# jby1993/SelfReconCode

Measured on NVIDIA H100. Metric: rays_per_sec, higher is better.
Workload: dtype f32

## Files before the change

include/selfrecon_b200.h:

```cpp
#ifndef SELFRECON_B200_H_
#define SELFRECON_B200_H_

#include <stdint.h>

#ifdef __cplusplus
extern "C" {
#endif

#ifndef __DRIVER_TYPES_H__
typedef struct CUstream_st* cudaStream_t;
#endif

enum {
  SR_OK = 0,
  SR_EINVAL = -1,
  SR_EUNSUPPORTED = -2,
  SR_ECAPACITY = -3
};

int sr_abi_version(void);
const char* sr_build_info(void);

int sr_minv3x3_f32(const float* ms, float* invs, uint8_t* checks, int64_t n, cudaStream_t s);
int sr_minv3x3_f64(const double* ms, double* invs, uint8_t* checks, int64_t n, cudaStream_t s);
int sr_minv3x3_bwd_f32(const float* grads, const float* invs, float* outs, int64_t n,
                       cudaStream_t s);
int sr_minv3x3_bwd_f64(const double* grads, const double* invs, double* outs, int64_t n,
                       cudaStream_t s);

int64_t sr_mc_work_bytes(int nx, int ny, int nz);
int sr_mc_count(const float* sdf, int nx, int ny, int nz, float iso, void* work, int32_t* counts,
                cudaStream_t s);
int sr_mc_emit(const float* sdf, int nx, int ny, int nz, float iso, float xstep, float ystep,
               float zstep, float xmin, float ymin, float zmin, int i_offset, const void* work,
               float* vertices, int64_t vcap, int64_t* faces, int64_t fcap, cudaStream_t s);

int sr_interp2x3d_fwd_f32(const float* in, float* out, uint8_t* is_boundary, int bc, int d, int h,
                          int w, float balance, cudaStream_t s);
int sr_interp2x3d_bwd_f32(const float* grad_out, float* grad_in, int bc, int d, int h, int w,
                          cudaStream_t s);
int sr_interp2x2d_fwd_f32(const float* in, float* out, uint8_t* is_boundary, int bc, int h, int w,
                          float balance, cudaStream_t s);
int sr_interp2x2d_bwd_f32(const float* grad_out, float* grad_in, int bc, int h, int w,
                          cudaStream_t s);

int sr_grid_sample3d_fwd_f32(const float* input, const int64_t* istr, const float* grid,
                             float* output, int32_t* corner_idx, int N, int C, int D, int H, int W,
                             int64_t P, cudaStream_t s);
int sr_grid_sample3d_bwd_f32(const float* input, const int64_t* istr, const float* grid,
                             const float* grad_output, float* grad_input, float* grad_grid, int N,
                             int C, int D, int H, int W, int64_t P, cudaStream_t s);
int sr_grid_sample3d_dbwd_f32(const float* gg_input ,
                              const float* gg_grid , const float* input,
                              const int64_t* istr, const float* grid, const float* grad_output,
                              float* grad_input , float* grad_grid,
                              float* grad_grad_output, int N, int C, int D, int H, int W,
                              int64_t P, cudaStream_t s);
int sr_grid_sample3d_fwd_f64(const double* input, const int64_t* istr, const double* grid,
                             double* output, int32_t* corner_idx, int N, int C, int D, int H,
                             int W, int64_t P, cudaStream_t s);
int sr_grid_sample3d_bwd_f64(const double* input, const int64_t* istr, const double* grid,
                             const double* grad_output, double* grad_input, double* grad_grid,
                             int N, int C, int D, int H, int W, int64_t P, cudaStream_t s);
int sr_grid_sample3d_dbwd_f64(const double* gg_input, const double* gg_grid, const double* input,
                              const int64_t* istr, const double* grid, const double* grad_output,
                              double* grad_input, double* grad_grid, double* grad_grad_output,
                              int N, int C, int D, int H, int W, int64_t P, cudaStream_t s);

#define SR_MLP_MAX_LAYERS 12
enum { SR_ACT_NONE = 0, SR_ACT_SOFTPLUS100 = 1, SR_ACT_RELU = 2, SR_ACT_TANH = 3 };

typedef struct sr_mlp_layer {
  const float* wt;
  const float* bias;
  int k;
  int n;
  int kpad;
  int npad;
  int act;
  int skip;
  const float* wb;
} sr_mlp_layer;

typedef struct sr_mlp_desc {
  int n_layers;
  int d_in;
  int multires;
  float pe_w[16];
  sr_mlp_layer layer[SR_MLP_MAX_LAYERS];
} sr_mlp_desc;

int sr_fold_linear(const float* v, const float* g, const float* b, int n, int k, int npad,
                   int kpad, float* wt, float* bias_out, float* wb ,
                   cudaStream_t s);

int sr_sdf_forward(const sr_mlp_desc* net, const float* pts, int64_t P, float* sdf, float* grad,
                   float* feat, int nfeat, cudaStream_t s);

int sr_lbs_bone_transforms(const float* poses, const float* Js, const int32_t* parents,
                           const float* init_pose_inv, int F, float* A, float* posedJ ,
                           cudaStream_t s);

typedef struct sr_lbs_params {
  const float* ws_cl;
  int D, H, W;
  float bmin[3], bmax[3];
  const float* A;
  const float* trans;
  int F;
} sr_lbs_params;

int sr_lbs_weights_to_channels_last(const float* ws_ncdhw, float* ws_cl, int D, int H, int W,
                                    cudaStream_t s);

int sr_deform_forward(const sr_mlp_desc* net, const sr_lbs_params* lbs, const float* pts,
                      const int64_t* batch_inds, int64_t pts_per_frame, const float* conds,
                      int condlen, int64_t P, float* d, float* offset, float* jac,
                      int32_t* corner_idx, cudaStream_t s);

int sr_render_forward(const sr_mlp_desc* net, const float* pts, const float* normals,
                      const float* views, const float* feat, int nfeat, int64_t P, float* rgb,
                      cudaStream_t s);

typedef struct sr_trace_params {
  float cam_pos[3];
  float dthreshold;
  float athreshold;
  float w1, w2;
} sr_trace_params;

int sr_trace_step(const sr_mlp_desc* sdf, const sr_mlp_desc* dnet, const sr_lbs_params* lbs,
                  const sr_trace_params* tp, float* pts, const float* rays,
                  const int64_t* batch_inds, const float* conds, int condlen, int64_t P,
                  const int32_t* active_in, int32_t* active_out, int32_t* counters, int iter,
                  uint8_t* converged, cudaStream_t s);

int64_t sr_trace_scratch_bytes(void);
int sr_trace_step_rev(const sr_mlp_desc* sdf, const sr_mlp_desc* dnet, const sr_lbs_params* lbs,
                      const sr_trace_params* tp, float* pts, const float* rays,
                      const int64_t* batch_inds, const float* conds, int condlen, int64_t P,
                      const int32_t* active_in, int32_t* active_out, int32_t* counters, int iter,
                      uint8_t* converged, float* scratch, cudaStream_t s);

int sr_shade_geometry(const sr_mlp_desc* sdf, const sr_mlp_desc* dnet, const sr_lbs_params* lbs,
                      const float* pts, const float* rays, const int64_t* batch_inds,
                      const float* conds, int condlen, int64_t P, float* normals, float* crays,
                      float* feat, int nfeat, float* dpos, uint8_t* inv_ok, cudaStream_t s);

int sr_tc_embed(const float* pts, int64_t P, int multires, const float* pe_w, int ch,
                const float* conds, const int64_t* batch_inds, int64_t pts_per_frame, int condlen,
                float* out, int ld, const int32_t* index ,
                const int32_t* m_dev , cudaStream_t s);
int sr_tc_embed_backward(const float* pts, int64_t P, int multires, const float* pe_w, int ch, const float* gx, int ld,
                         float* gp, cudaStream_t s);
int64_t sr_tc_act_bytes(int64_t M, int K);
int64_t sr_tc_weight_bytes(int N, int K);
int sr_tc_pack_rows(const float* src, int64_t M, int K, int ld, void* dst, const int32_t* m_dev,
                    cudaStream_t s);
int sr_tc_pack_weights(const float* w, int N, int K, int ld, void* dst, cudaStream_t s);
int sr_tc_linear(const void* A, const void* W, const float* bias, int64_t M, int N, int K,
                 int n_valid, int act, int ch, void* A_next, int K_next, float scale,
                 const float* skip_src, int skip_n, int skip_ld, float* out, int out_ld,
                 int out_col0, int out_n, float* dstash, const void* mul_tiles, int mul_K, int mul_act,
                 float mul_scale, const int32_t* m_dev, cudaStream_t s);

int sr_raster_mesh(const float* verts_screen, const int64_t* faces, int64_t N, int64_t V, int64_t F, int H, int W,
                   uint64_t* keys, int64_t* pix_to_face, float* bary, float* zbuf, cudaStream_t s);

typedef struct sr_phong_params {
  float light_ambient[3], light_diffuse[3], light_specular[3];
  float mat_ambient[3], mat_diffuse[3], mat_specular[3];
  float shininess;
  float background[3];
} sr_phong_params;
int sr_mesh_vertex_normals(const float* verts, const int64_t* faces, const int64_t* vf_offsets, const int64_t* vf_faces,
                           int64_t N, int64_t V, int64_t F, float* normals, cudaStream_t s);
int sr_shade_phong(const float* verts, const float* normals, const float* colors, const int64_t* faces, int64_t N,
                   int64_t V, int64_t F, const int64_t* pix_to_face, const float* bary, int H, int W,
                   const float* cam_pos, const float* light_pos, const sr_phong_params* params, float* out,
                   cudaStream_t s);

int64_t sr_tc_wgrad_partial_bytes(int64_t M, int Kd, int Kx, int* splits_out);
void sr_tc_debug_wgrad_desc_swap(int v);
int sr_tc_wgrad(const void* D, int Kd, const void* X, int Kx, int64_t M, float* part, float* dW, int N, int K,
                int ld, cudaStream_t s);
int sr_tc_colsum(const void* T, int64_t M, int K, int ch, float* partial, int slices, cudaStream_t s);
int sr_tc_unpack_rows(const void* T, int64_t M, int K, int Kpad, float* out, int ld, cudaStream_t s);

typedef struct sr_tc_layer {
  const void* W;
  const void* Wb;
  const float* bias;
  const float* zero_bias;
  int n, k, act, skip;
} sr_tc_layer;
int sr_tc_mlp_forward(const sr_tc_layer* layers, int L, const float* x0, int64_t M, int ld, int d_in, int ch, void* A_in,
                      void* const* acts, float* const* stashes, float* out, const int32_t* m_dev, int n_out,
                      cudaStream_t s);
int sr_tc_mlp_backward(const sr_tc_layer* layers, int L, int64_t M, int ld, int d_in, int ch, const float* gout,
                       const void* A_in, void* const* acts, float* const* stashes, void* D0, void* D1, float* part,
                       float* colsum_ws, int colsum_slices, float* const* dW, float* const* db, float* x0_grad,
                       float* g_skip, int g_skip_ld, cudaStream_t s);

int sr_svals3x3_f32(const float* J, float* S, float* V, int64_t n, cudaStream_t s);
int sr_svals3x3_bwd_f32(const float* J, const float* S, const float* V, const float* gS, float* gJ, int64_t n,
                        cudaStream_t s);

typedef struct sr_wn_layer {
  const float* v;
  const float* g;
  float* w;
  float* inv_norm;
  const float* gw;
  float* gv;
  float* gg;
  int32_t n, k, gw_ld, pad_;
} sr_wn_layer;
int sr_weight_norm_forward(const sr_wn_layer* layers, int L, cudaStream_t s);
int sr_weight_norm_backward(const sr_wn_layer* layers, int L, cudaStream_t s);

int sr_band_select(const float* values, int64_t n, float center, float eps, int32_t* list,
                   int32_t* counter, cudaStream_t s);
int sr_sdf_forward_indexed(const sr_mlp_desc* net, const float* pts, int64_t P, const int32_t* index,
                           const int32_t* m_dev, float* sdf, cudaStream_t s);
int64_t sr_sdf_small_work_bytes(int cap);
int sr_sdf_forward_small(const sr_mlp_desc* net, const float* pts, int64_t P, const int32_t* index,
                         const int32_t* m_dev, float* sdf, void* work, int cap, cudaStream_t s);

int sr_tc_trace_mid(const int32_t* index, const int32_t* m_dev, int64_t P, const float* pts,
                    const float* rays, const int64_t* batch_inds, const float* f, const float* off,
                    const sr_lbs_params* lbs, const sr_trace_params* tp, int do_update,
                    uint8_t* converged, float* dsdf, float* ddef, int ld, float* aux,
                    int32_t* recheck , int32_t* recheck_count, float eps_f, float eps_a,
                    cudaStream_t s);
int sr_tc_trace_update(const int32_t* index, const int32_t* m_dev, int64_t P, float* pts,
                       const float* gs, int gs_ld, const float* gskip, int gk_ld, const float* gd,
                       int gd_ld, const float* aux, int mr_s, const float* pw_s, int mr_d,
                       const float* pw_d, int32_t* active_out, int32_t* counter_out,
                       const uint8_t* converged , cudaStream_t s);

int sr_tc_shade_point(int64_t P, const float* pts, const float* rays, const int64_t* batch_inds,
                      const float* sdf4, int ld_s, const float* off4, const sr_lbs_params* lbs,
                      float* normals, float* crays, float* dpos, uint8_t* inv_ok, cudaStream_t s);
int sr_tc_render_embed(int64_t P, const float* pts, const float* views, const float* normals,
                       const float* feat, int feat_ld, int feat_col0, int nfeat, int feat_row_stride,
                       int multires, const float* pw, float* out, int ld, cudaStream_t s);

int sr_seg3d_candidates(const uint8_t* flag, const uint8_t* calculated, uint8_t* cand, int D,
                        int H, int W, int sz, int sy, int sx, int fD, int fH, int fW,
                        cudaStream_t s);
int sr_seg3d_gather(const int64_t* lin, int64_t n, int H, int W, int sz, int sy, int sx, int fD,
                    int fH, int fW, const float* bmin, const float* bmax, const float* grid,
                    float* points, float* interp, uint8_t* calculated, cudaStream_t s);
int sr_seg3d_scatter(const int64_t* lin, int64_t n, const float* values, const float* interp,
                     float balance, float* grid, uint8_t* conflict, int64_t conflict_bytes,
                     int32_t* n_conflicts, cudaStream_t s);

#ifdef __cplusplus
}
#endif
#endif
```

selfreconcode_b200/_lib.py:

```python
import ctypes as C
import os

_HERE = os.path.dirname(os.path.abspath(__file__))
LIB_PATH = os.environ.get("SELFRECON_B200_LIB") or os.path.join(_HERE, "lib", "libselfrecon_b200.so")

SR_OK = 0
SR_EINVAL, SR_EUNSUPPORTED, SR_ECAPACITY = -1, -2, -3
SR_MLP_MAX_LAYERS = 12
SR_ACT_NONE, SR_ACT_SOFTPLUS100, SR_ACT_RELU, SR_ACT_TANH = 0, 1, 2, 3

c_f = C.c_void_p
i64 = C.c_int64
i32 = C.c_int
f32 = C.c_float
stream_t = C.c_void_p


class MlpLayer(C.Structure):
    _fields_ = [("wt", C.c_void_p), ("bias", C.c_void_p), ("k", C.c_int), ("n", C.c_int),
                ("kpad", C.c_int), ("npad", C.c_int), ("act", C.c_int), ("skip", C.c_int),
                ("wb", C.c_void_p)]


class MlpDesc(C.Structure):
    _fields_ = [("n_layers", C.c_int), ("d_in", C.c_int), ("multires", C.c_int),
                ("pe_w", C.c_float * 16), ("layer", MlpLayer * SR_MLP_MAX_LAYERS)]


class LbsParams(C.Structure):
    _fields_ = [("ws_cl", C.c_void_p), ("D", C.c_int), ("H", C.c_int), ("W", C.c_int),
                ("bmin", C.c_float * 3), ("bmax", C.c_float * 3), ("A", C.c_void_p),
                ("trans", C.c_void_p), ("F", C.c_int)]


class TcLayer(C.Structure):
    _fields_ = [("W", C.c_void_p), ("Wb", C.c_void_p), ("bias", C.c_void_p), ("zero_bias", C.c_void_p),
                ("n", C.c_int), ("k", C.c_int), ("act", C.c_int), ("skip", C.c_int)]


class WnLayer(C.Structure):
    _fields_ = [("v", C.c_void_p), ("g", C.c_void_p), ("w", C.c_void_p), ("inv_norm", C.c_void_p),
                ("gw", C.c_void_p), ("gv", C.c_void_p), ("gg", C.c_void_p),
                ("n", C.c_int32), ("k", C.c_int32), ("gw_ld", C.c_int32), ("pad_", C.c_int32)]


class TraceParams(C.Structure):
    _fields_ = [("cam_pos", C.c_float * 3), ("dthreshold", C.c_float), ("athreshold", C.c_float),
                ("w1", C.c_float), ("w2", C.c_float)]


class PhongParams(C.Structure):
    _fields_ = [("light_ambient", C.c_float * 3), ("light_diffuse", C.c_float * 3), ("light_specular", C.c_float * 3),
                ("mat_ambient", C.c_float * 3), ("mat_diffuse", C.c_float * 3), ("mat_specular", C.c_float * 3),
                ("shininess", C.c_float), ("background", C.c_float * 3)]


SIGNATURES = {
    "sr_abi_version": (C.c_int, []),
    "sr_build_info": (C.c_char_p, []),
    "sr_minv3x3_f32": (C.c_int, [c_f, c_f, c_f, i64, stream_t]),
    "sr_minv3x3_f64": (C.c_int, [c_f, c_f, c_f, i64, stream_t]),
    "sr_minv3x3_bwd_f32": (C.c_int, [c_f, c_f, c_f, i64, stream_t]),
    "sr_minv3x3_bwd_f64": (C.c_int, [c_f, c_f, c_f, i64, stream_t]),
    "sr_mc_work_bytes": (i64, [i32, i32, i32]),
    "sr_mc_count": (C.c_int, [c_f, i32, i32, i32, f32, c_f, c_f, stream_t]),
    "sr_mc_emit": (C.c_int, [c_f, i32, i32, i32, f32, f32, f32, f32, f32, f32, f32, i32, c_f, c_f, i64,
                             c_f, i64, stream_t]),
    "sr_interp2x3d_fwd_f32": (C.c_int, [c_f, c_f, c_f, i32, i32, i32, i32, f32, stream_t]),
    "sr_interp2x3d_bwd_f32": (C.c_int, [c_f, c_f, i32, i32, i32, i32, stream_t]),
    "sr_interp2x2d_fwd_f32": (C.c_int, [c_f, c_f, c_f, i32, i32, i32, f32, stream_t]),
    "sr_interp2x2d_bwd_f32": (C.c_int, [c_f, c_f, i32, i32, i32, stream_t]),
    "sr_grid_sample3d_fwd_f32": (C.c_int, [c_f, C.POINTER(i64), c_f, c_f, c_f, i32, i32, i32, i32,
                                           i32, i64, stream_t]),
    "sr_grid_sample3d_bwd_f32": (C.c_int, [c_f, C.POINTER(i64), c_f, c_f, c_f, c_f, i32, i32, i32,
                                           i32, i32, i64, stream_t]),
    "sr_grid_sample3d_dbwd_f32": (C.c_int, [c_f, c_f, c_f, C.POINTER(i64), c_f, c_f, c_f, c_f, c_f,
                                            i32, i32, i32, i32, i32, i64, stream_t]),
    "sr_grid_sample3d_fwd_f64": (C.c_int, [c_f, C.POINTER(i64), c_f, c_f, c_f, i32, i32, i32, i32,
                                           i32, i64, stream_t]),
    "sr_grid_sample3d_bwd_f64": (C.c_int, [c_f, C.POINTER(i64), c_f, c_f, c_f, c_f, i32, i32, i32,
                                           i32, i32, i64, stream_t]),
    "sr_grid_sample3d_dbwd_f64": (C.c_int, [c_f, c_f, c_f, C.POINTER(i64), c_f, c_f, c_f, c_f, c_f,
                                            i32, i32, i32, i32, i32, i64, stream_t]),
    "sr_fold_linear": (C.c_int, [c_f, c_f, c_f, i32, i32, i32, i32, c_f, c_f, c_f, stream_t]),
    "sr_sdf_forward": (C.c_int, [C.POINTER(MlpDesc), c_f, i64, c_f, c_f, c_f, i32, stream_t]),
    "sr_lbs_bone_transforms": (C.c_int, [c_f, c_f, c_f, c_f, i32, c_f, c_f, stream_t]),
    "sr_lbs_weights_to_channels_last": (C.c_int, [c_f, c_f, i32, i32, i32, stream_t]),
    "sr_deform_forward": (C.c_int, [C.POINTER(MlpDesc), C.POINTER(LbsParams), c_f, c_f, i64, c_f,
                                    i32, i64, c_f, c_f, c_f, c_f, stream_t]),
    "sr_render_forward": (C.c_int, [C.POINTER(MlpDesc), c_f, c_f, c_f, c_f, i32, i64, c_f,
                                    stream_t]),
    "sr_trace_step": (C.c_int, [C.POINTER(MlpDesc), C.POINTER(MlpDesc), C.POINTER(LbsParams),
                                C.POINTER(TraceParams), c_f, c_f, c_f, c_f, i32, i64, c_f, c_f,
                                c_f, i32, c_f, stream_t]),
    "sr_trace_scratch_bytes": (i64, []),
    "sr_trace_step_rev": (C.c_int, [C.POINTER(MlpDesc), C.POINTER(MlpDesc), C.POINTER(LbsParams),
                                    C.POINTER(TraceParams), c_f, c_f, c_f, c_f, i32, i64, c_f, c_f,
                                    c_f, i32, c_f, c_f, stream_t]),
    "sr_shade_geometry": (C.c_int, [C.POINTER(MlpDesc), C.POINTER(MlpDesc), C.POINTER(LbsParams),
                                    c_f, c_f, c_f, c_f, i32, i64, c_f, c_f, c_f, i32, c_f, c_f,
                                    stream_t]),
    "sr_tc_embed": (C.c_int, [c_f, i64, i32, C.POINTER(f32), i32, c_f, c_f, i64, i32, c_f, i32, c_f, c_f,
                              stream_t]),
    "sr_tc_embed_backward": (C.c_int, [c_f, i64, i32, C.POINTER(f32), i32, c_f, i32, c_f, stream_t]),
    "sr_tc_act_bytes": (i64, [i64, i32]),
    "sr_tc_weight_bytes": (i64, [i32, i32]),
    "sr_tc_pack_rows": (C.c_int, [c_f, i64, i32, i32, c_f, c_f, stream_t]),
    "sr_tc_pack_weights": (C.c_int, [c_f, i32, i32, i32, c_f, stream_t]),
    "sr_tc_linear": (C.c_int, [c_f, c_f, c_f, i64, i32, i32, i32, i32, i32, c_f, i32, f32, c_f, i32,
                               i32, c_f, i32, i32, i32, c_f, c_f, i32, i32, f32, c_f, stream_t]),
    "sr_tc_trace_mid": (C.c_int, [c_f, c_f, i64, c_f, c_f, c_f, c_f, c_f, C.POINTER(LbsParams),
                                  C.POINTER(TraceParams), i32, c_f, c_f, c_f, i32, c_f, c_f, c_f, f32, f32,
                                  stream_t]),
    "sr_tc_trace_update": (C.c_int, [c_f, c_f, i64, c_f, c_f, i32, c_f, i32, c_f, i32, c_f, i32,
                                     C.POINTER(f32), i32, C.POINTER(f32), c_f, c_f, c_f, stream_t]),
    "sr_raster_mesh": (C.c_int, [c_f, c_f, i64, i64, i64, i32, i32, c_f, c_f, c_f, c_f, stream_t]),
    "sr_mesh_vertex_normals": (C.c_int, [c_f, c_f, c_f, c_f, i64, i64, i64, c_f, stream_t]),
    "sr_shade_phong": (C.c_int, [c_f, c_f, c_f, c_f, i64, i64, i64, c_f, c_f, i32, i32, c_f, c_f,
                                 C.POINTER(PhongParams), c_f, stream_t]),
    "sr_tc_wgrad_partial_bytes": (i64, [i64, i32, i32, C.POINTER(C.c_int)]),
    "sr_tc_debug_wgrad_desc_swap": (None, [i32]),
    "sr_tc_mlp_forward": (C.c_int, [C.POINTER(TcLayer), i32, c_f, i64, i32, i32, i32, c_f, C.POINTER(C.c_void_p),
                                    C.POINTER(C.c_void_p), c_f, c_f, i32, stream_t]),
    "sr_tc_mlp_backward": (C.c_int, [C.POINTER(TcLayer), i32, i64, i32, i32, i32, c_f, c_f, C.POINTER(C.c_void_p),
                                     C.POINTER(C.c_void_p), c_f, c_f, c_f, c_f, i32, C.POINTER(C.c_void_p),
                                     C.POINTER(C.c_void_p), c_f, c_f, i32, stream_t]),
    "sr_tc_wgrad": (C.c_int, [c_f, i32, c_f, i32, i64, c_f, c_f, i32, i32, i32, stream_t]),
    "sr_tc_colsum": (C.c_int, [c_f, i64, i32, i32, c_f, i32, stream_t]),
    "sr_tc_unpack_rows": (C.c_int, [c_f, i64, i32, i32, c_f, i32, stream_t]),
    "sr_weight_norm_forward": (C.c_int, [C.POINTER(WnLayer), i32, stream_t]),
    "sr_weight_norm_backward": (C.c_int, [C.POINTER(WnLayer), i32, stream_t]),
    "sr_svals3x3_f32": (C.c_int, [c_f, c_f, c_f, i64, stream_t]),
    "sr_svals3x3_bwd_f32": (C.c_int, [c_f, c_f, c_f, c_f, c_f, i64, stream_t]),
    "sr_band_select": (C.c_int, [c_f, i64, f32, f32, c_f, c_f, stream_t]),
    "sr_sdf_small_work_bytes": (i64, [i32]),
    "sr_sdf_forward_small": (C.c_int, [C.POINTER(MlpDesc), c_f, i64, c_f, c_f, c_f, c_f, i32, stream_t]),
    "sr_sdf_forward_indexed": (C.c_int, [C.POINTER(MlpDesc), c_f, i64, c_f, c_f, c_f, stream_t]),
    "sr_tc_shade_point": (C.c_int, [i64, c_f, c_f, c_f, c_f, i32, c_f, C.POINTER(LbsParams), c_f, c_f, c_f,
                                    c_f, stream_t]),
    "sr_tc_render_embed": (C.c_int, [i64, c_f, c_f, c_f, c_f, i32, i32, i32, i32, i32, C.POINTER(f32), c_f,
                                     i32, stream_t]),
    "sr_seg3d_candidates": (C.c_int, [c_f, c_f, c_f, i32, i32, i32, i32, i32, i32, i32, i32, i32,
                                      stream_t]),
    "sr_seg3d_gather": (C.c_int, [c_f, i64, i32, i32, i32, i32, i32, i32, i32, i32, C.POINTER(f32), C.POINTER(f32),
                                  c_f, c_f, c_f, c_f, stream_t]),
    "sr_seg3d_scatter": (C.c_int, [c_f, i64, c_f, c_f, f32, c_f, c_f, i64, c_f, stream_t]),
}

_lib = None


def load():
    global _lib
    if _lib is not None:
        return _lib
    if not os.path.exists(LIB_PATH):
        raise RuntimeError(
            "selfrecon_b200: %s is missing -- run `python -m selfreconcode_b200.build` "
            "(or __graft_entry__.build()).  There is no CPU fallback." % LIB_PATH)
    lib = C.CDLL(LIB_PATH)
    for name, (res, args) in SIGNATURES.items():
        fn = getattr(lib, name)
        fn.restype = res
        fn.argtypes = args
    _lib = lib
    return lib


_ERR = {SR_EINVAL: "invalid argument", SR_EUNSUPPORTED: "unsupported shape",
        SR_ECAPACITY: "output buffer too small"}


def check(code, what):
    if code == SR_OK:
        return
    if code < 0:
        raise RuntimeError("selfrecon_b200.%s: %s (code %d)" % (what, _ERR.get(code, "error"), code))
    raise RuntimeError("selfrecon_b200.%s: CUDA error %d" % (what, code))
```

selfreconcode_b200/csrc/tc_common.cuh:

```cuda
#pragma once
#include <cuda_bf16.h>

#include "common.cuh"

namespace sr_tc {

#ifndef SR_TC_PLANES
#define SR_TC_PLANES 2
#endif
constexpr int kPlanes = SR_TC_PLANES;
constexpr int BM = 128, BN = 256, BK = 32, STAGES = kPlanes == 2 ? 3 : 2;
constexpr int A_PLANE = BM * BK;
constexpr int W_PLANE = BN * BK;
constexpr int A_STAGE = kPlanes * A_PLANE;
constexpr int W_STAGE = kPlanes * W_PLANE;
constexpr uint32_t A_STAGE_BYTES = A_STAGE * 2, W_STAGE_BYTES = W_STAGE * 2;

__host__ __device__ inline size_t a_tile_off(long long mt, int kc, int KC, int p) {
  return (((size_t)mt * KC + kc) * kPlanes + p) * A_PLANE;
}
__host__ __device__ inline size_t w_tile_off(int nt, int kc, int KC, int p) {
  return (((size_t)nt * KC + kc) * kPlanes + p) * W_PLANE;
}
__device__ __forceinline__ int in_tile_off(int rows_per_tile, int r, int k) {
  return (k >> 3) * (rows_per_tile * 8) + (r >> 3) * 64 + (r & 7) * 8 + (k & 7);
}

__device__ __forceinline__ void split3(float x, __nv_bfloat16& b1, __nv_bfloat16& b2, __nv_bfloat16& b3) {
  b1 = __float2bfloat16_rn(x);
  const float r1 = x - __bfloat162float(b1);
  b2 = __float2bfloat16_rn(r1);
  const float r2 = r1 - __bfloat162float(b2);
  b3 = __float2bfloat16_rn(r2);
}

__device__ __forceinline__ uint64_t make_desc(uint32_t smem_addr, uint32_t lbo_bytes, uint32_t sbo_bytes) {
  uint64_t d = (uint64_t)((smem_addr & 0x3FFFFu) >> 4);
  d |= (uint64_t)((lbo_bytes >> 4) & 0x3FFFu) << 16;
  d |= (uint64_t)((sbo_bytes >> 4) & 0x3FFFu) << 32;
  return d;
}
__device__ __forceinline__ void wgmma_fence() { asm volatile("wgmma.fence.sync.aligned;" ::: "memory"); }
__device__ __forceinline__ void wgmma_commit() { asm volatile("wgmma.commit_group.sync.aligned;" ::: "memory"); }
template <int N>
__device__ __forceinline__ void wgmma_wait() {
  asm volatile("wgmma.wait_group.sync.aligned %0;" ::"n"(N) : "memory");
}
__device__ __forceinline__ void warpgroup_sync(int id) { asm volatile("bar.sync %0, 128;" ::"r"(id) : "memory"); }

#define SR_ACC8(c, d, i)                                                                                \
  c(d[i]), c(d[i + 1]), c(d[i + 2]), c(d[i + 3]), c(d[i + 4]), c(d[i + 5]), c(d[i + 6]), c(d[i + 7])
#define SR_ACC32(c, d, i) SR_ACC8(c, d, i), SR_ACC8(c, d, i + 8), SR_ACC8(c, d, i + 16), SR_ACC8(c, d, i + 24)
#define SR_ACC128(c, d) SR_ACC32(c, d, 0), SR_ACC32(c, d, 32), SR_ACC32(c, d, 64), SR_ACC32(c, d, 96)
#define SR_WGMMA_M64N256K16_BF16                                                                                   \
  "{\n\t.reg .pred p;\n\tsetp.ne.b32 p, %130, 0;\n\t"                                                            \
  "wgmma.mma_async.sync.aligned.m64n256k16.f32.bf16.bf16 "                                                         \
  "{%0, %1, %2, %3, %4, %5, %6, %7, %8, %9, %10, %11, %12, %13, %14, %15, %16, %17, %18, %19, %20, %21, %22, "     \
  "%23, %24, %25, %26, %27, %28, %29, %30, %31, %32, %33, %34, %35, %36, %37, %38, %39, %40, %41, %42, %43, "      \
  "%44, %45, %46, %47, %48, %49, %50, %51, %52, %53, %54, %55, %56, %57, %58, %59, %60, %61, %62, %63, %64, "      \
  "%65, %66, %67, %68, %69, %70, %71, %72, %73, %74, %75, %76, %77, %78, %79, %80, %81, %82, %83, %84, %85, "      \
  "%86, %87, %88, %89, %90, %91, %92, %93, %94, %95, %96, %97, %98, %99, %100, %101, %102, %103, %104, %105, "     \
  "%106, %107, %108, %109, %110, %111, %112, %113, %114, %115, %116, %117, %118, %119, %120, %121, %122, %123, "   \
  "%124, %125, %126, %127}, %128, %129, p, 1, 1, %131, %132;\n\t}\n"

#define SR_OUT(x) "=f"(x)
#define SR_INOUT(x) "+f"(x)
template <int TA, int TB, bool FIRST>
__device__ __forceinline__ void wgmma_m64n256k16(float (&d)[128], uint64_t adesc, uint64_t bdesc) {
  if constexpr (FIRST)
    asm volatile(SR_WGMMA_M64N256K16_BF16
                 : SR_ACC128(SR_OUT, d)
                 : "l"(adesc), "l"(bdesc), "r"(0), "n"(TA), "n"(TB));
  else
    asm volatile(SR_WGMMA_M64N256K16_BF16
                 : SR_ACC128(SR_INOUT, d)
                 : "l"(adesc), "l"(bdesc), "r"(1), "n"(TA), "n"(TB));
}
#undef SR_OUT
#undef SR_INOUT
#undef SR_WGMMA_M64N256K16_BF16
#undef SR_ACC128
#undef SR_ACC32
#undef SR_ACC8

}
```

selfreconcode_b200/csrc/tc_gemm.cu:

```cuda
#include <cstdlib>

#include "tc_common.cuh"

namespace sr_tc {

struct LayerArgs {
  const __nv_bfloat16* A;
  const __nv_bfloat16* W;
  const float* bias;
  long long M;
  int MT, NT, KC;
  int n_gemm;
  int n;
  int ch;
  __nv_bfloat16* A_next;
  int KCn;
  float scale;
  const float* skip_src;
  int skip_n, skip_ld;
  float* out;
  int out_ld;
  float* dstash;
  const __nv_bfloat16* mul_tiles;
  int mul_KC;
  float mul_inv_scale;
  int out_col0;
  int out_n;
  const int* m_dev;
};

template <int ACT>
__device__ __forceinline__ float act_fn(float z, float& d) {
  if constexpr (ACT == SR_ACT_SOFTPLUS100) {
    const float bz = z * 100.0f;
    const float e = __expf(fminf(bz, 20.0f));
    const float sp = __logf(1.0f + e) * 0.01f;
    const float dd = __fdividef(e, e + 1.0f);
    d = bz > 20.0f ? 1.0f : dd;
    return bz > 20.0f ? z : sp;
  } else if constexpr (ACT == SR_ACT_RELU) {
    d = z > 0.f ? 1.f : 0.f;
    return fmaxf(z, 0.f);
  } else if constexpr (ACT == SR_ACT_TANH) {
    const float t = tanhf(z);
    d = 1.f - t * t;
    return t;
  } else {
    d = 1.f;
    return z;
  }
}

__device__ __forceinline__ float fast_ex2(float x) {
  float y;
  asm("ex2.approx.ftz.f32 %0, %1;" : "=f"(y) : "f"(x));
  return y;
}
__device__ __forceinline__ float fast_lg2(float x) {
  float y;
  asm("lg2.approx.ftz.f32 %0, %1;" : "=f"(y) : "f"(x));
  return y;
}
template <int ACT>
__device__ __forceinline__ float act_val(float z) {
  if constexpr (ACT == SR_ACT_SOFTPLUS100) {
    const float t = z * 144.26950408889634f;
    const float e = fast_ex2(fminf(t, 28.853900817779268f));
    const float sp = fast_lg2(1.0f + e) * 0.006931471805599453f;
    return t > 28.853900817779268f ? z : sp;
  } else if constexpr (ACT == SR_ACT_RELU) {
    return fmaxf(z, 0.f);
  } else if constexpr (ACT == SR_ACT_TANH) {
    return tanhf(z);
  } else {
    return z;
  }
}
template <int ACT>
__device__ __forceinline__ float dact_from_val(float a) {
  if constexpr (ACT == SR_ACT_SOFTPLUS100) return 1.0f - fast_ex2(a * -144.26950408889634f);
  else if constexpr (ACT == SR_ACT_RELU) return a > 0.f ? 1.f : 0.f;
  else if constexpr (ACT == SR_ACT_TANH) return 1.f - a * a;
  else return 1.f;
}

__device__ __forceinline__ void split3x2(float x0, float x1, uint32_t& p1, uint32_t& p2, uint32_t& p3) {
  __nv_bfloat162 h = __floats2bfloat162_rn(x0, x1);
  p1 = *reinterpret_cast<uint32_t*>(&h);
  const float r0 = x0 - __uint_as_float(p1 << 16), r1 = x1 - __uint_as_float(p1 & 0xffff0000u);
  h = __floats2bfloat162_rn(r0, r1);
  p2 = *reinterpret_cast<uint32_t*>(&h);
  if constexpr (kPlanes == 3) {
    const float s0 = r0 - __uint_as_float(p2 << 16), s1 = r1 - __uint_as_float(p2 & 0xffff0000u);
    h = __floats2bfloat162_rn(s0, s1);
    p3 = *reinterpret_cast<uint32_t*>(&h);
  } else {
    p3 = 0u;
  }
}

struct EpiRow {
  long long mt, row;
  int nt, row_in_tile, lane;
  bool row_ok, is_val;
  size_t ds_ld;
};

template <int ACT, int CH, bool MUL, bool PF = true>
__device__ __forceinline__ void epi_chunk(const LayerArgs& a, const EpiRow& r, uint32_t (&v)[32], int chunk,
                                          bool live) {
  const int c0 = r.nt * BN + chunk * 32;
  float o[32];
  if (live) {
    if constexpr (MUL) {
      const __nv_bfloat16* mt = a.mul_tiles + a_tile_off(r.mt, c0 >> 5, a.mul_KC, 0) +
                                (size_t)(r.row_in_tile >> 3) * 64 + (r.row_in_tile & 7) * 8;
      const float kk = -144.26950408889634f * a.mul_inv_scale;
      const long long srow = r.row_ok ? (CH == 4 ? (r.row & ~3LL) : r.row) : 0;
      const float* stash = a.dstash == nullptr || c0 >= a.n ? nullptr : a.dstash + (size_t)srow * r.ds_ld + c0;
      const bool use_stash = (ACT == SR_ACT_SOFTPLUS100) && stash != nullptr;
      uint4 q0[PF ? 4 : 1], q1[PF ? 4 : 1];
      float st[PF ? 32 : 1];
      if constexpr (PF) {
#pragma unroll
        for (int g = 0; g < 4; ++g) {
          q0[g] = __ldg(reinterpret_cast<const uint4*>(mt + (size_t)g * (BM * 8)));
          q1[g] = __ldg(reinterpret_cast<const uint4*>(mt + (size_t)g * (BM * 8) + A_PLANE));
        }
        if (use_stash) {
#pragma unroll
          for (int j4 = 0; j4 < 8; ++j4) {
            const float4 t = __ldg(reinterpret_cast<const float4*>(stash) + j4);
            st[4 * j4] = t.x; st[4 * j4 + 1] = t.y; st[4 * j4 + 2] = t.z; st[4 * j4 + 3] = t.w;
          }
        }
      }
#pragma unroll
      for (int g = 0; g < 4; ++g) {
        uint4 a0, a1;
        float sg[8];
        if constexpr (PF) {
          a0 = q0[g]; a1 = q1[g];
        } else {
          a0 = __ldg(reinterpret_cast<const uint4*>(mt + (size_t)g * (BM * 8)));
          a1 = __ldg(reinterpret_cast<const uint4*>(mt + (size_t)g * (BM * 8) + A_PLANE));
          if (use_stash) {
            const float4 t0 = __ldg(reinterpret_cast<const float4*>(stash) + 2 * g);
            const float4 t1 = __ldg(reinterpret_cast<const float4*>(stash) + 2 * g + 1);
            sg[0] = t0.x; sg[1] = t0.y; sg[2] = t0.z; sg[3] = t0.w; sg[4] = t1.x; sg[5] = t1.y; sg[6] = t1.z; sg[7] = t1.w;
          }
        }
        const uint32_t w0[4] = {a0.x, a0.y, a0.z, a0.w}, w1[4] = {a1.x, a1.y, a1.z, a1.w};
#pragma unroll
        for (int e = 0; e < 8; ++e) {
          const int j = g * 8 + e;
          const uint32_t h0 = w0[e >> 1], h1 = w1[e >> 1];
          const float as = (e & 1) ? __uint_as_float(h0 & 0xffff0000u) + __uint_as_float(h1 & 0xffff0000u)
                                   : __uint_as_float(h0 << 16) + __uint_as_float(h1 << 16);
          float val = __uint_as_float(v[j]);
          if constexpr (CH == 1) {
            float d;
            if constexpr (ACT == SR_ACT_SOFTPLUS100) {
              d = use_stash ? (PF ? st[PF ? j : 0] : sg[e]) : 1.0f - fast_ex2(kk * as);
            } else if constexpr (ACT == SR_ACT_RELU) d = as > 0.f ? 1.f : 0.f;
            else d = 1.f;
            if (c0 + j < a.n) val = r.row_ok ? val * d : 0.f;
          } else {
            float d;
            if constexpr (ACT == SR_ACT_SOFTPLUS100) {
              if (use_stash) d = PF ? st[PF ? j : 0] : sg[e];
              else d = 1.0f - fast_ex2(kk * __shfl_sync(0xffffffffu, as, r.lane & ~3));
            } else if constexpr (ACT == SR_ACT_RELU) {
              d = __shfl_sync(0xffffffffu, as, r.lane & ~3) > 0.f ? 1.f : 0.f;
            } else d = 1.f;
            float cross = 0.f;
            if constexpr (ACT == SR_ACT_SOFTPLUS100) {
              float prod = r.is_val ? 0.f : val * (as * a.mul_inv_scale);
              prod += __shfl_xor_sync(0xffffffffu, prod, 1);
              prod += __shfl_xor_sync(0xffffffffu, prod, 2);
              cross = prod;
            }
            if (c0 + j < a.n) {
              float o4 = val * d;
              if constexpr (ACT == SR_ACT_SOFTPLUS100) { if (r.is_val) o4 += 100.0f * (1.0f - d) * cross; }
              val = r.row_ok ? o4 : 0.f;
            }
          }
          o[j] = val * a.scale;
        }
      }
    } else {
#pragma unroll
      for (int j4 = 0; j4 < 8; ++j4) {
        const float4 b4 = __ldg(reinterpret_cast<const float4*>(a.bias + c0) + j4);
        const float bb[4] = {b4.x, b4.y, b4.z, b4.w};
#pragma unroll
        for (int jj = 0; jj < 4; ++jj) {
          const int j = j4 * 4 + jj;
          const float acc = __uint_as_float(v[j]);
          float val;
          if constexpr (CH == 1) {
            val = act_val<ACT>(acc + bb[jj]);
          } else {
            float d = 1.f;
            val = act_fn<ACT>(acc + bb[jj], d);
            const float dv = __shfl_sync(0xffffffffu, d, r.lane & ~3);
            if (!r.is_val) { val = dv * acc; }
            v[j] = __float_as_uint(d);
          }
          o[j] = val * a.scale;
        }
      }
      if (a.dstash != nullptr && r.is_val && r.row_ok) {
        if constexpr (CH == 1) {
          const float inv = 1.0f / a.scale;
#pragma unroll
          for (int j = 0; j < 32; ++j) v[j] = __float_as_uint(dact_from_val<ACT>(o[j] * inv));
        }
        float4* dd = reinterpret_cast<float4*>(a.dstash + (size_t)r.row * r.ds_ld + c0);
#pragma unroll
        for (int j4 = 0; j4 < 8; ++j4)
          dd[j4] = make_float4(__uint_as_float(v[4 * j4]), __uint_as_float(v[4 * j4 + 1]),
                               __uint_as_float(v[4 * j4 + 2]), __uint_as_float(v[4 * j4 + 3]));
      }
    }
    if (a.out != nullptr && r.row_ok && c0 < a.out_col0 + a.out_n && c0 + 32 > a.out_col0) {
#pragma unroll
      for (int j = 0; j < 32; ++j) {
        const int c = c0 + j - a.out_col0;
        if (c >= 0 && c < a.out_n) a.out[(size_t)r.row * a.out_ld + c] = o[j];
      }
    }
  }
  if (a.A_next == nullptr) return;
  const int kcn = c0 >> 5;
  if (kcn >= a.KCn) return;
  if (!live || c0 + 32 > a.n) {
#pragma unroll
    for (int j = 0; j < 32; ++j) {
      const int c = c0 + j;
      if (!live || c >= a.n) {
        float val = 0.f;
        if (a.skip_src != nullptr && c >= a.n && c < a.n + a.skip_n && r.row_ok)
          val = a.skip_src[(size_t)r.row * a.skip_ld + (c - a.n)] * a.scale;
        o[j] = val;
      }
    }
  }
  __nv_bfloat16* base = a.A_next + a_tile_off(r.mt, kcn, a.KCn, 0) + (size_t)(r.row_in_tile >> 3) * 64 +
                        (r.row_in_tile & 7) * 8;
#pragma unroll
  for (int g = 0; g < 4; ++g) {
    uint4 q1, q2, q3;
    split3x2(o[g * 8 + 0], o[g * 8 + 1], q1.x, q2.x, q3.x);
    split3x2(o[g * 8 + 2], o[g * 8 + 3], q1.y, q2.y, q3.y);
    split3x2(o[g * 8 + 4], o[g * 8 + 5], q1.z, q2.z, q3.z);
    split3x2(o[g * 8 + 6], o[g * 8 + 7], q1.w, q2.w, q3.w);
    __nv_bfloat16* dst = base + (size_t)g * (BM * 8);
    *reinterpret_cast<uint4*>(dst) = q1;
    *reinterpret_cast<uint4*>(dst + A_PLANE) = q2;
    if constexpr (kPlanes == 3) *reinterpret_cast<uint4*>(dst + 2 * A_PLANE) = q3;
  }
}


constexpr int kConsumerWGs = 2;
constexpr int kThreads = 128 * (1 + kConsumerWGs);
constexpr int kEpiWarps = 4 * kConsumerWGs;
constexpr int STG_LD = 132;
constexpr int STG_FLOATS = 64 * STG_LD;
constexpr size_t kSmem = (size_t)STAGES * (A_STAGE_BYTES + W_STAGE_BYTES) + (size_t)kConsumerWGs * STG_FLOATS * 4 + 256;
static_assert(kSmem <= 227 * 1024, "shared memory of one H100 block");

template <bool FIRST>
__device__ __forceinline__ void mma_chunk(float (&acc)[128], uint32_t abase, uint32_t wbase) {
  constexpr int kTerms = kPlanes == 2 ? 3 : 6;
  const int pa[6] = {0, 1, 0, 2, 1, 0}, pw[6] = {1, 0, 0, 0, 1, 0};
  const int pa3[6] = {0, 2, 1, 0, 1, 0}, pw3[6] = {2, 0, 1, 1, 0, 0};
#pragma unroll
  for (int q = 0; q < kTerms; ++q) {
#pragma unroll
    for (int jj = 0; jj < BK / 16; ++jj) {
      const int qa = kPlanes == 2 ? pa[q] : pa3[q], qw = kPlanes == 2 ? pw[q] : pw3[q];
      const uint64_t ad = make_desc(abase + qa * (A_PLANE * 2) + jj * 2 * (BM * 16), BM * 16, 128);
      const uint64_t bd = make_desc(wbase + qw * (W_PLANE * 2) + jj * 2 * (BN * 16), BN * 16, 128);
      if (FIRST && q == 0 && jj == 0) wgmma_m64n256k16<0, 0, true>(acc, ad, bd);
      else wgmma_m64n256k16<0, 0, false>(acc, ad, bd);
    }
  }
}

template <int ACT, int CH, bool MUL>
__global__ void __launch_bounds__(kThreads, 1) tc_sweep_kernel(const __grid_constant__ LayerArgs a) {
  extern __shared__ __align__(1024) unsigned char smem[];
  __nv_bfloat16* sA = reinterpret_cast<__nv_bfloat16*>(smem);
  __nv_bfloat16* sW = reinterpret_cast<__nv_bfloat16*>(smem + (size_t)STAGES * A_STAGE_BYTES);
  float* stg = reinterpret_cast<float*>(smem + (size_t)STAGES * (A_STAGE_BYTES + W_STAGE_BYTES));
  uint64_t* bars = reinterpret_cast<uint64_t*>(stg + kConsumerWGs * STG_FLOATS);
  uint64_t* full = bars;
  uint64_t* empty = bars + STAGES;

  const int warp = threadIdx.x >> 5, lane = threadIdx.x & 31, wg = threadIdx.x >> 7;
  if (threadIdx.x == 0) {
    for (int i = 0; i < STAGES; ++i) { sr_mbar_init(&full[i], 1); sr_mbar_init(&empty[i], kEpiWarps); }
    sr_fence_barrier_init();
  }
  __syncthreads();
  long long Mrows = a.M;
  int MTe = a.MT;
  if (a.m_dev != nullptr) {
    const long long md = (long long)(*a.m_dev);
    Mrows = md < a.M ? md : a.M;
    MTe = (int)((Mrows + BM - 1) / BM);
  }
  const int cta = blockIdx.x, ncta = gridDim.x;
  const int J = cta < MTe ? (MTe - cta + ncta - 1) / ncta : 0;

  if (wg == 0) {
    asm volatile("setmaxnreg.dec.sync.aligned.u32 40;");
    if (threadIdx.x == 0) {
      int slot = 0;
      uint32_t phase = 0;
      for (int j = 0; j < J; ++j) {
        const long long mt = (long long)cta + (long long)j * ncta;
        for (int nt = 0; nt < a.NT; ++nt) {
          for (int kc = 0; kc < a.KC; ++kc) {
            sr_mbar_wait(&empty[slot], phase ^ 1u);
            sr_mbar_arrive_expect_tx(&full[slot], A_STAGE_BYTES + W_STAGE_BYTES);
            sr_bulk_g2s(sW + (size_t)slot * W_STAGE, a.W + w_tile_off(nt, kc, a.KC, 0), W_STAGE_BYTES, &full[slot]);
            sr_bulk_g2s(sA + (size_t)slot * A_STAGE, a.A + a_tile_off(mt, kc, a.KC, 0), A_STAGE_BYTES, &full[slot]);
            if (++slot == STAGES) { slot = 0; phase ^= 1u; }
          }
        }
      }
    }
  } else {
    asm volatile("setmaxnreg.inc.sync.aligned.u32 232;");
    const int cw = wg - 1;
    const int wq = warp & 3;
    float* st = stg + cw * STG_FLOATS;
    float acc[128];
    EpiRow r;
    r.row_in_tile = cw * 64 + (wq & 1) * 32 + lane;
    r.lane = lane;
    r.is_val = (CH == 1) || ((lane & 3) == 0);
    r.ds_ld = MUL ? (size_t)((a.n + BN - 1) / BN) * BN : (size_t)a.NT * BN;
    int slot = 0;
    uint32_t phase = 0;
    for (int j = 0; j < J; ++j) {
      r.mt = (long long)cta + (long long)j * ncta;
      r.row = r.mt * BM + r.row_in_tile;
      r.row_ok = r.row < Mrows;
      for (int nt = 0; nt < a.NT; ++nt) {
        r.nt = nt;
        sr_mbar_wait(&full[slot], phase);
        wgmma_fence();
        mma_chunk<true>(acc, sr_smem_u32(sA + (size_t)slot * A_STAGE) + cw * 8 * 128,
                        sr_smem_u32(sW + (size_t)slot * W_STAGE));
        wgmma_commit();
        int prev = slot;
        if (++slot == STAGES) { slot = 0; phase ^= 1u; }
        for (int kc = 1; kc < a.KC; ++kc) {
          sr_mbar_wait(&full[slot], phase);
          wgmma_fence();
          mma_chunk<false>(acc, sr_smem_u32(sA + (size_t)slot * A_STAGE) + cw * 8 * 128,
                           sr_smem_u32(sW + (size_t)slot * W_STAGE));
          wgmma_commit();
          wgmma_wait<1>();
          if (lane == 0) sr_mbar_arrive(&empty[prev]);
          prev = slot;
          if (++slot == STAGES) { slot = 0; phase ^= 1u; }
        }
        wgmma_wait<0>();
        if (lane == 0) sr_mbar_arrive(&empty[prev]);
#pragma unroll
        for (int h = 0; h < 2; ++h) {
          const int fr = 16 * wq + (lane >> 2), fc = 2 * (lane & 3);
#pragma unroll
          for (int i = 0; i < 16; ++i) {
            *reinterpret_cast<float2*>(st + fr * STG_LD + 8 * i + fc) =
                make_float2(acc[4 * (16 * h + i)], acc[4 * (16 * h + i) + 1]);
            *reinterpret_cast<float2*>(st + (fr + 8) * STG_LD + 8 * i + fc) =
                make_float2(acc[4 * (16 * h + i) + 2], acc[4 * (16 * h + i) + 3]);
          }
          warpgroup_sync(1 + cw);
          const float* srow = st + ((wq & 1) * 32 + lane) * STG_LD + (wq >> 1) * 64;
          for (int i = 0; i < 2; ++i) {
            const int chunk = 4 * h + 2 * (wq >> 1) + i;
            uint32_t v[32];
#pragma unroll
            for (int j4 = 0; j4 < 8; ++j4) {
              const float4 t = reinterpret_cast<const float4*>(srow + 32 * i)[j4];
              v[4 * j4] = __float_as_uint(t.x); v[4 * j4 + 1] = __float_as_uint(t.y);
              v[4 * j4 + 2] = __float_as_uint(t.z); v[4 * j4 + 3] = __float_as_uint(t.w);
            }
            epi_chunk<ACT, CH, MUL>(a, r, v, chunk, nt * BN + chunk * 32 < a.n_gemm);
          }
          warpgroup_sync(1 + cw);
        }
      }
    }
  }
}

__global__ void pack_rows_kernel(const float* __restrict__ src, long long M, int K, int ld,
                                 __nv_bfloat16* __restrict__ dst, int KC, long long MT,
                                 const int* __restrict__ m_dev) {
  if (m_dev != nullptr) {
    const long long md = *m_dev;
    M = md < M ? md : M;
    MT = (M + BM - 1) / BM;
  }
  const long long total = MT * BM * (long long)KC * 4;
  for (long long idx = (long long)blockIdx.x * blockDim.x + threadIdx.x; idx < total;
       idx += (long long)gridDim.x * blockDim.x) {
    const int r = (int)(idx % BM);
    const long long rest = idx / BM;
    const int g = (int)(rest % (KC * 4));
    const long long mt = rest / (KC * 4);
    const long long row = mt * BM + r;
    const int kc = g >> 2, k8 = g & 3;
    __align__(16) __nv_bfloat16 p1[8], p2[8], p3[8];
#pragma unroll
    for (int e = 0; e < 8; ++e) {
      const int k = kc * 32 + k8 * 8 + e;
      const float x = (row < M && k < K) ? src[(size_t)row * ld + k] : 0.f;
      split3(x, p1[e], p2[e], p3[e]);
    }
    const size_t off = (size_t)k8 * (BM * 8) + (size_t)(r >> 3) * 64 + (r & 7) * 8;
    *reinterpret_cast<uint4*>(dst + a_tile_off(mt, kc, KC, 0) + off) = *reinterpret_cast<uint4*>(p1);
    *reinterpret_cast<uint4*>(dst + a_tile_off(mt, kc, KC, 1) + off) = *reinterpret_cast<uint4*>(p2);
    if constexpr (kPlanes == 3)
      *reinterpret_cast<uint4*>(dst + a_tile_off(mt, kc, KC, kPlanes - 1) + off) = *reinterpret_cast<uint4*>(p3);
  }
}

__global__ void pack_skip_tail_kernel(const float* __restrict__ skip_src, int skip_ld, int n, int skip_n, float scale,
                                      long long M, int kc0, int KCn, __nv_bfloat16* __restrict__ dst,
                                      const int* __restrict__ m_dev) {
  if (m_dev != nullptr) {
    const long long md = *m_dev;
    M = md < M ? md : M;
  }
  const long long MT = (M + BM - 1) / BM;
  const int nkc = KCn - kc0;
  const long long total = MT * BM * (long long)nkc * 4;
  for (long long idx = (long long)blockIdx.x * blockDim.x + threadIdx.x; idx < total;
       idx += (long long)gridDim.x * blockDim.x) {
    const int r = (int)(idx % BM);
    const long long rest = idx / BM;
    const int g = (int)(rest % (nkc * 4));
    const long long mt = rest / (nkc * 4);
    const long long row = mt * BM + r;
    const int kc = kc0 + (g >> 2), k8 = g & 3;
    __align__(16) __nv_bfloat16 p1[8], p2[8], p3[8];
#pragma unroll
    for (int e = 0; e < 8; ++e) {
      const int c = kc * 32 + k8 * 8 + e;
      const float x = (skip_src != nullptr && row < M && c >= n && c < n + skip_n)
                          ? skip_src[(size_t)row * skip_ld + (c - n)] * scale : 0.f;
      split3(x, p1[e], p2[e], p3[e]);
    }
    const size_t off = (size_t)k8 * (BM * 8) + (size_t)(r >> 3) * 64 + (r & 7) * 8;
    *reinterpret_cast<uint4*>(dst + a_tile_off(mt, kc, KCn, 0) + off) = *reinterpret_cast<uint4*>(p1);
    *reinterpret_cast<uint4*>(dst + a_tile_off(mt, kc, KCn, 1) + off) = *reinterpret_cast<uint4*>(p2);
    if constexpr (kPlanes == 3)
      *reinterpret_cast<uint4*>(dst + a_tile_off(mt, kc, KCn, kPlanes - 1) + off) = *reinterpret_cast<uint4*>(p3);
  }
}

__global__ void pack_weights_kernel(const float* __restrict__ w, int N, int K, int ld,
                                    __nv_bfloat16* __restrict__ dst, int NT, int KC) {
  const long long total = (long long)NT * BN * KC * 4;
  for (long long idx = (long long)blockIdx.x * blockDim.x + threadIdx.x; idx < total;
       idx += (long long)gridDim.x * blockDim.x) {
    const int r = (int)(idx % BN);
    const long long rest = idx / BN;
    const int g = (int)(rest % (KC * 4));
    const int nt = (int)(rest / (KC * 4));
    const int n = nt * BN + r;
    const int kc = g >> 2, k8 = g & 3;
    __align__(16) __nv_bfloat16 p1[8], p2[8], p3[8];
#pragma unroll
    for (int e = 0; e < 8; ++e) {
      const int k = kc * 32 + k8 * 8 + e;
      const float x = (n < N && k < K) ? w[(size_t)n * ld + k] : 0.f;
      split3(x, p1[e], p2[e], p3[e]);
    }
    const size_t off = (size_t)k8 * (BN * 8) + (size_t)(r >> 3) * 64 + (r & 7) * 8;
    *reinterpret_cast<uint4*>(dst + w_tile_off(nt, kc, KC, 0) + off) = *reinterpret_cast<uint4*>(p1);
    *reinterpret_cast<uint4*>(dst + w_tile_off(nt, kc, KC, 1) + off) = *reinterpret_cast<uint4*>(p2);
    if constexpr (kPlanes == 3)
      *reinterpret_cast<uint4*>(dst + w_tile_off(nt, kc, KC, kPlanes - 1) + off) = *reinterpret_cast<uint4*>(p3);
  }
}

struct EmbedArgs {
  const float* pts;
  long long P;
  int multires;
  float pe_w[16];
  int ch;
  const float* conds;
  const long long* batch_inds;
  long long pts_per_frame;
  int condlen;
  float* out;
  int ld;
  const int* index;
  const int* m_dev;
};
__global__ void embed_kernel(const __grid_constant__ EmbedArgs a) {
  long long np = a.P;
  if (a.m_dev != nullptr) { const long long md = *a.m_dev; np = md < np ? md : np; }
  const long long total = np * a.ch * (long long)a.ld;
  const int pe_dim = 3 + 6 * a.multires;
  for (long long idx = (long long)blockIdx.x * blockDim.x + threadIdx.x; idx < total;
       idx += (long long)gridDim.x * blockDim.x) {
    const int k = (int)(idx % a.ld);
    const long long row = idx / a.ld;
    const long long pi = row / a.ch;
    const long long p = a.index ? (long long)a.index[pi] : pi;
    const int t = (int)(row % a.ch);
    float v = 0.f;
    if (k < 3) {
      v = t == 0 ? a.pts[p * 3 + k] : (t - 1 == k ? 1.f : 0.f);
    } else if (k < pe_dim) {
      const int b = (k - 3) / 6, w6 = (k - 3) % 6, j = w6 % 3;
      const bool is_cos = w6 >= 3;
      if (t == 0 || t - 1 == j) {
        const float freq = (float)(1 << b);
        float sn, cs;
        sincosf(a.pts[p * 3 + j] * freq, &sn, &cs);
        const float w = a.pe_w[b];
        if (t == 0) v = w * (is_cos ? cs : sn);
        else v = is_cos ? -(w * freq) * sn : (w * freq) * cs;
      }
    } else if (k < pe_dim + a.condlen) {
      if (t == 0) {
        const long long bi = a.batch_inds ? a.batch_inds[p] : (a.pts_per_frame > 0 ? p / a.pts_per_frame : 0);
        v = a.conds[bi * a.condlen + (k - pe_dim)];
      }
    }
    a.out[idx] = v;
  }
}

__global__ void embed_bwd_kernel(const float* __restrict__ pts, long long P, int multires, const float* __restrict__ gx,
                                 int ld, int ch, float* __restrict__ gp, float pw0, float pw1, float pw2, float pw3,
                                 float pw4, float pw5, float pw6, float pw7) {
  const float pw[8] = {pw0, pw1, pw2, pw3, pw4, pw5, pw6, pw7};
  for (long long p = (long long)blockIdx.x * blockDim.x + threadIdx.x; p < P; p += (long long)gridDim.x * blockDim.x) {
    const float* gv = gx + (size_t)p * ch * ld;
    float out[3];
#pragma unroll
    for (int j = 0; j < 3; ++j) {
      const float x = pts[p * 3 + j];
      float acc = gv[j];
      const float* gt = ch == 4 ? gv + (size_t)(1 + j) * ld : nullptr;
      float freq = 1.0f;
      for (int b = 0; b < multires; ++b, freq *= 2.0f) {
        float sn, cs;
        sincosf(x * freq, &sn, &cs);
        const float w = pw[b] * freq;
        const int ks = 3 + 6 * b + j, kc = ks + 3;
        acc += w * (cs * gv[ks] - sn * gv[kc]);
        if (gt) acc -= w * freq * (sn * gt[ks] + cs * gt[kc]);
      }
      out[j] = acc;
    }
    gp[p * 3] = out[0]; gp[p * 3 + 1] = out[1]; gp[p * 3 + 2] = out[2];
  }
}

}

extern "C" {

int sr_tc_embed_backward(const float* pts, int64_t P, int multires, const float* pe_w, int ch, const float* gx, int ld,
                         float* gp, cudaStream_t s) {
  if (!pts || !gx || !gp || !pe_w || P <= 0 || (ch != 1 && ch != 4) || multires < 0 || multires > 8 ||
      ld < 3 + 6 * multires)
    return SR_EINVAL;
  float w[8];
  for (int i = 0; i < 8; ++i) w[i] = i < multires ? pe_w[i] : 0.f;
  sr_tc::embed_bwd_kernel<<<sr_grid_for(P, 256, 8), 256, 0, s>>>(pts, P, multires, gx, ld, ch, gp, w[0], w[1], w[2], w[3],
                                                                  w[4], w[5], w[6], w[7]);
  return sr_launch_status();
}

int sr_tc_embed(const float* pts, int64_t P, int multires, const float* pe_w, int ch,
                const float* conds, const int64_t* batch_inds, int64_t pts_per_frame, int condlen,
                float* out, int ld, const int32_t* index, const int32_t* m_dev, cudaStream_t s) {
  if (!pts || !out || !pe_w || P <= 0 || (ch != 1 && ch != 4) || multires < 0 || multires > 16) return SR_EINVAL;
  if (ld < 3 + 6 * multires + condlen || (condlen > 0 && !conds)) return SR_EINVAL;
  sr_tc::EmbedArgs a;
  a.pts = pts; a.P = P; a.multires = multires; a.ch = ch; a.conds = conds;
  a.batch_inds = (const long long*)batch_inds; a.pts_per_frame = pts_per_frame; a.condlen = condlen;
  a.out = out; a.ld = ld; a.index = index; a.m_dev = m_dev;
  for (int i = 0; i < 16; ++i) a.pe_w[i] = i < multires ? pe_w[i] : 0.f;
  const long long total = P * ch * (long long)ld;
  sr_tc::embed_kernel<<<sr_grid_for(total, 256, 8), 256, 0, s>>>(a);
  return sr_launch_status();
}

int64_t sr_tc_act_bytes(int64_t M, int K) {
  const int64_t MT = (M + sr_tc::BM - 1) / sr_tc::BM, KC = (K + 31) / 32;
  return MT * KC * sr_tc::kPlanes * sr_tc::A_PLANE * 2;
}
int64_t sr_tc_weight_bytes(int N, int K) {
  const int64_t NT = (N + sr_tc::BN - 1) / sr_tc::BN, KC = (K + 31) / 32;
  return NT * KC * sr_tc::kPlanes * sr_tc::W_PLANE * 2;
}

int sr_tc_pack_rows(const float* src, int64_t M, int K, int ld, void* dst, const int32_t* m_dev,
                    cudaStream_t s) {
  if (!src || !dst || M <= 0 || K <= 0 || ld < K) return SR_EINVAL;
  const long long MT = (M + sr_tc::BM - 1) / sr_tc::BM;
  const int KC = (K + 31) / 32;
  const long long total = MT * sr_tc::BM * KC * 4;
  sr_tc::pack_rows_kernel<<<sr_grid_for(total, 256, 8), 256, 0, s>>>(src, M, K, ld, (__nv_bfloat16*)dst, KC, MT, m_dev);
  return sr_launch_status();
}

int sr_tc_pack_weights(const float* w, int N, int K, int ld, void* dst, cudaStream_t s) {
  if (!w || !dst || N <= 0 || K <= 0 || ld < K) return SR_EINVAL;
  const int NT = (N + sr_tc::BN - 1) / sr_tc::BN, KC = (K + 31) / 32;
  const long long total = (long long)NT * sr_tc::BN * KC * 4;
  sr_tc::pack_weights_kernel<<<sr_grid_for(total, 256, 8), 256, 0, s>>>(w, N, K, ld, (__nv_bfloat16*)dst, NT, KC);
  return sr_launch_status();
}

int sr_tc_linear(const void* A, const void* W, const float* bias, int64_t M, int N, int K, int n_valid,
                 int act, int ch, void* A_next, int K_next, float scale, const float* skip_src,
                 int skip_n, int skip_ld, float* out, int out_ld, int out_col0, int out_n,
                 float* dstash, const void* mul_tiles, int mul_K, int mul_act, float mul_scale,
                 const int32_t* m_dev, cudaStream_t s) {
  using namespace sr_tc;
  if (M <= 0 || (ch != 1 && ch != 4)) return SR_EINVAL;
  if (!A || !W || !bias || N <= 0 || K <= 0 || (!A_next && !out)) return SR_EINVAL;
  if (mul_tiles ? (mul_K < n_valid || (mul_act != SR_ACT_NONE && mul_act != SR_ACT_SOFTPLUS100 && mul_act != SR_ACT_RELU))
                : (act < SR_ACT_NONE || act > SR_ACT_TANH))
    return SR_EINVAL;
  LayerArgs a;
  a.A = (const __nv_bfloat16*)A; a.W = (const __nv_bfloat16*)W; a.bias = bias; a.M = M;
  a.MT = (int)((M + BM - 1) / BM); a.NT = (N + BN - 1) / BN; a.KC = (K + 31) / 32;
  a.n_gemm = N; a.n = n_valid; a.ch = ch;
  a.A_next = (__nv_bfloat16*)A_next; a.KCn = A_next ? (K_next + 31) / 32 : 0;
  a.scale = scale; a.skip_src = skip_src; a.skip_n = skip_n; a.skip_ld = skip_ld;
  a.out = out; a.out_ld = out_ld; a.dstash = dstash; a.out_col0 = out_col0; a.out_n = out_n;
  a.mul_tiles = (const __nv_bfloat16*)mul_tiles; a.mul_KC = (mul_K + 31) / 32;
  a.mul_inv_scale = mul_scale != 0.f ? 1.0f / mul_scale : 1.0f; a.m_dev = m_dev;

  using Kern = void (*)(const LayerArgs);
  Kern kern = nullptr;
#define SR_SW(ACT_, CH_, MUL_) kern = (Kern)tc_sweep_kernel<ACT_, CH_, MUL_>
  const int key = (ch == 4 ? 10 : 0) + (mul_tiles ? 5 + mul_act : act);
  switch (key) {
    case 0: SR_SW(SR_ACT_NONE, 1, false); break;
    case 1: SR_SW(SR_ACT_SOFTPLUS100, 1, false); break;
    case 2: SR_SW(SR_ACT_RELU, 1, false); break;
    case 3: SR_SW(SR_ACT_TANH, 1, false); break;
    case 5: SR_SW(SR_ACT_NONE, 1, true); break;
    case 6: SR_SW(SR_ACT_SOFTPLUS100, 1, true); break;
    case 7: SR_SW(SR_ACT_RELU, 1, true); break;
    case 10: SR_SW(SR_ACT_NONE, 4, false); break;
    case 11: SR_SW(SR_ACT_SOFTPLUS100, 4, false); break;
    case 12: SR_SW(SR_ACT_RELU, 4, false); break;
    case 13: SR_SW(SR_ACT_TANH, 4, false); break;
    case 15: SR_SW(SR_ACT_NONE, 4, true); break;
    case 16: SR_SW(SR_ACT_SOFTPLUS100, 4, true); break;
    case 17: SR_SW(SR_ACT_RELU, 4, true); break;
  }
#undef SR_SW
  if (!kern) return SR_EINVAL;
  static bool attr_set_dev[64][20] = {};
  int cur_dev = 0;
  cudaGetDevice(&cur_dev);
  bool& attr_set = attr_set_dev[cur_dev & 63][key];
  if (!attr_set) {
    cudaError_t e = cudaFuncSetAttribute(kern, cudaFuncAttributeMaxDynamicSharedMemorySize, (int)kSmem);
    if (e != cudaSuccess) return (int)e;
    attr_set = true;
  }
  const int grid = a.MT < SR_NUM_SMS ? a.MT : SR_NUM_SMS;
  kern<<<grid, kThreads, kSmem, s>>>(a);
  const int kc0 = a.NT * (BN / 32);
  if (a.A_next != nullptr && a.KCn > kc0) {
    const int rc = sr_launch_status();
    if (rc) return rc;
    const long long total = (long long)a.MT * BM * (a.KCn - kc0) * 4;
    pack_skip_tail_kernel<<<sr_grid_for(total, 256, 8), 256, 0, s>>>(a.skip_src, a.skip_ld, a.n, a.skip_n, a.scale, M,
                                                                     kc0, a.KCn, a.A_next, m_dev);
  }
  return sr_launch_status();
}
}
```

selfreconcode_b200/csrc/trace_tc.cu:

```cuda
#include "common.cuh"
#include "lbs.cuh"

namespace {

struct MidArgs {
  const int* index;
  const int* m_dev;
  long long P;
  const float* pts;
  const float* rays;
  const long long* batch_inds;
  const float* f;
  const float* off;
  sr_lbs_params lbs;
  int has_lbs;
  sr_trace_params tp;
  int do_update;
  unsigned char* converged;
  float* dsdf;
  float* ddef;
  int ld;
  float* aux;
  int* recheck;
  int* recheck_count;
  float eps_f, eps_a;
};

__global__ void __launch_bounds__(256) trace_mid_kernel(const __grid_constant__ MidArgs a) {
  long long M = a.P;
  if (a.m_dev) { const long long md = *a.m_dev; M = md < M ? md : M; }
  const int lane = threadIdx.x & 31;
  const long long warp0 = ((long long)blockIdx.x * blockDim.x + threadIdx.x) >> 5;
  const long long nwarps = ((long long)gridDim.x * blockDim.x) >> 5;
  for (long long i = warp0; i < M; i += nwarps) {
    const long long gp = a.index ? (long long)a.index[i] : i;
    float p[3], pp[3], off[3] = {0.f, 0.f, 0.f};
#pragma unroll
    for (int j = 0; j < 3; ++j) {
      p[j] = a.pts[gp * 3 + j];
      if (a.off) off[j] = a.off[i * 3 + j];
      pp[j] = __fadd_rn(p[j], off[j]);
    }
    float d[3], Mm[9];
    int ci[3];
    if (a.has_lbs) {
      lbs_point(a.lbs, pp, a.batch_inds ? (int)a.batch_inds[gp] : 0, d, Mm, ci);
    } else {
#pragma unroll
      for (int j = 0; j < 3; ++j) d[j] = pp[j];
#pragma unroll
      for (int q = 0; q < 9; ++q) Mm[q] = (q % 4 == 0) ? 1.f : 0.f;
    }
    if (lane == 0) {
      const float f = a.f[i];
      const float vx = a.rays[gp * 3], vy = a.rays[gp * 3 + 1], vz = a.rays[gp * 3 + 2];
      const float ux = d[0] - a.tp.cam_pos[0], uy = d[1] - a.tp.cam_pos[1], uz = d[2] - a.tp.cam_pos[2];
      const float cx = uy * vz - uz * vy, cy = uz * vx - ux * vz, cz = ux * vy - uy * vx;
      const float n_up = sqrtf(cx * cx + cy * cy + cz * cz);
      const float n_u = sqrtf(ux * ux + uy * uy + uz * uz);
      const float sang = n_up / n_u;
      const float ang = asinf(sang) * 180.0f / 3.14159265358979323846f;
      bool done = (fabsf(f) < a.tp.dthreshold) && (ang < a.tp.athreshold);
      if (a.recheck != nullptr) {
        const bool maybe = (fabsf(f) < a.tp.dthreshold + a.eps_f) && (ang < a.tp.athreshold + a.eps_a);
        const bool sure = (fabsf(f) < a.tp.dthreshold - a.eps_f) && (ang < a.tp.athreshold - a.eps_a);
        if (maybe && !sure) a.recheck[atomicAdd(a.recheck_count, 1)] = (int)gp;
        done = sure;
      }
      float u[3] = {0.f, 0.f, 0.f}, loss = 0.f;
      int state = 0;
      if (done) {
        a.converged[gp] = 1;
      } else if (a.do_update) {
        state = 1;
        loss = a.tp.w1 * fabsf(f) + a.tp.w2 * fabsf(sang);
        float q[3] = {0.f, 0.f, 0.f};
        if (n_up > 0.f) {
          const float wx = vy * cz - vz * cy, wy = vz * cx - vx * cz, wz = vx * cy - vy * cx;
          const float i1 = 1.0f / (n_up * n_u), i2 = n_up / (n_u * n_u * n_u);
          q[0] = wx * i1 - ux * i2; q[1] = wy * i1 - uy * i2; q[2] = wz * i1 - uz * i2;
        }
#pragma unroll
        for (int j = 0; j < 3; ++j) u[j] = a.tp.w2 * (Mm[j] * q[0] + Mm[3 + j] * q[1] + Mm[6 + j] * q[2]);
      }
      float* ax = a.aux + i * 8;
      ax[0] = loss; ax[1] = __int_as_float(state); ax[2] = u[0]; ax[3] = u[1]; ax[4] = u[2];
    }
    __syncwarp();
    const float* ax = a.aux + i * 8;
    for (int k = lane; k < a.ld; k += 32) {
      float vs = 0.f, vd = 0.f;
      if (k == 0) {
        const float f = a.f[i];
        vs = (__float_as_int(ax[1]) == 1) ? a.tp.w1 * (f > 0.f ? 1.f : (f < 0.f ? -1.f : 0.f)) : 0.f;
      }
      if (k < 3) vd = ax[2 + k];
      a.dsdf[i * a.ld + k] = vs;
      if (a.ddef) a.ddef[i * a.ld + k] = vd;
    }
  }
}

struct UpdArgs {
  const int* index;
  const int* m_dev;
  long long P;
  float* pts;
  const float* gs;
  int gs_ld;
  const float* gskip;
  int gk_ld;
  const float* gd;
  int gd_ld;
  const float* aux;
  int mr_s;
  float pw_s[16];
  int mr_d;
  float pw_d[16];
  int* active_out;
  int* counter_out;
  const unsigned char* converged;
};

__device__ __forceinline__ void pe_chain(const float* g, const float* gk, const float x[3], int multires,
                                         const float* pw, float out[3]) {
#pragma unroll
  for (int j = 0; j < 3; ++j) out[j] += g[j] + (gk ? gk[j] : 0.f);
  float freq = 1.0f;
  for (int b = 0; b < multires; ++b, freq *= 2.0f) {
    const float w = pw[b] * freq;
    const int ks = 3 + 6 * b, kc = ks + 3;
#pragma unroll
    for (int j = 0; j < 3; ++j) {
      float sn, cs;
      sincosf(x[j] * freq, &sn, &cs);
      const float gsn = g[ks + j] + (gk ? gk[ks + j] : 0.f), gcs = g[kc + j] + (gk ? gk[kc + j] : 0.f);
      out[j] += w * (cs * gsn - sn * gcs);
    }
  }
}

__global__ void __launch_bounds__(256) trace_update_kernel(const __grid_constant__ UpdArgs a) {
  long long M = a.P;
  if (a.m_dev) { const long long md = *a.m_dev; M = md < M ? md : M; }
  for (long long i = (long long)blockIdx.x * blockDim.x + threadIdx.x; i < M;
       i += (long long)gridDim.x * blockDim.x) {
    const float* ax = a.aux + i * 8;
    if (__float_as_int(ax[1]) != 1) continue;
    const long long gp = a.index ? (long long)a.index[i] : i;
    if (a.converged != nullptr && a.converged[gp]) continue;
    const float x[3] = {a.pts[gp * 3], a.pts[gp * 3 + 1], a.pts[gp * 3 + 2]};
    float g[3] = {ax[2], ax[3], ax[4]};
    pe_chain(a.gs + i * a.gs_ld, a.gskip ? a.gskip + i * a.gk_ld : nullptr, x, a.mr_s, a.pw_s, g);
    if (a.gd) pe_chain(a.gd + i * a.gd_ld, nullptr, x, a.mr_d, a.pw_d, g);
    const float t = -ax[0] / (g[0] * g[0] + g[1] * g[1] + g[2] * g[2]);
#pragma unroll
    for (int j = 0; j < 3; ++j) a.pts[gp * 3 + j] = x[j] + t * g[j];
    const int slot = atomicAdd(a.counter_out, 1);
    a.active_out[slot] = (int)gp;
  }
}

struct ShadePtArgs {
  long long P;
  const float* pts;
  const float* rays;
  const long long* batch_inds;
  const float* sdf4;
  int ld_s;
  const float* off4;
  sr_lbs_params lbs;
  int has_lbs;
  float* normals;
  float* crays;
  float* dpos;
  unsigned char* inv_ok;
};

__global__ void __launch_bounds__(256) shade_point_kernel(const __grid_constant__ ShadePtArgs a) {
  const int lane = threadIdx.x & 31;
  const long long warp0 = ((long long)blockIdx.x * blockDim.x + threadIdx.x) >> 5;
  const long long nwarps = ((long long)gridDim.x * blockDim.x) >> 5;
  for (long long i = warp0; i < a.P; i += nwarps) {
    float p[3], pp[3], off[3] = {0.f, 0.f, 0.f};
#pragma unroll
    for (int j = 0; j < 3; ++j) {
      p[j] = a.pts[i * 3 + j];
      if (a.off4) off[j] = a.off4[(i * 4) * 3 + j];
      pp[j] = __fadd_rn(p[j], off[j]);
    }
    float d[3], Mm[9];
    int ci[3];
    if (a.has_lbs) lbs_point(a.lbs, pp, a.batch_inds ? (int)a.batch_inds[i] : 0, d, Mm, ci);
    else {
#pragma unroll
      for (int j = 0; j < 3; ++j) d[j] = pp[j];
#pragma unroll
      for (int q = 0; q < 9; ++q) Mm[q] = (q % 4 == 0) ? 1.f : 0.f;
    }
    if (lane == 0) {
      float Q[9], m[9];
#pragma unroll
      for (int r = 0; r < 3; ++r)
#pragma unroll
        for (int c = 0; c < 3; ++c) Q[3 * r + c] = (r == c ? 1.f : 0.f) + (a.off4 ? a.off4[(i * 4 + 1 + c) * 3 + r] : 0.f);
#pragma unroll
      for (int r = 0; r < 3; ++r)
#pragma unroll
        for (int c = 0; c < 3; ++c) m[3 * r + c] = Mm[3 * r] * Q[c] + Mm[3 * r + 1] * Q[3 + c] + Mm[3 * r + 2] * Q[6 + c];
      const float gx = a.sdf4[(i * 4 + 1) * a.ld_s], gy = a.sdf4[(i * 4 + 2) * a.ld_s], gz = a.sdf4[(i * 4 + 3) * a.ld_s];
      const float gn = sqrtf(gx * gx + gy * gy + gz * gz);
      a.normals[i * 3] = gx / gn; a.normals[i * 3 + 1] = gy / gn; a.normals[i * 3 + 2] = gz / gn;
      const float c00 = m[4] * m[8] - m[5] * m[7], c01 = -m[3] * m[8] + m[5] * m[6], c02 = m[3] * m[7] - m[4] * m[6];
      const float c10 = -m[1] * m[8] + m[2] * m[7], c11 = m[0] * m[8] - m[2] * m[6], c12 = -m[0] * m[7] + m[1] * m[6];
      const float c20 = m[1] * m[5] - m[2] * m[4], c21 = -m[0] * m[5] + m[2] * m[3], c22 = m[0] * m[4] - m[1] * m[3];
      const float det = m[0] * c00 + m[1] * c01 + m[2] * c02;
      const bool ok = !(fabs((double)det) < 0.0001);
      const float vx = a.rays[i * 3], vy = a.rays[i * 3 + 1], vz = a.rays[i * 3 + 2];
      float rx = vx, ry = vy, rz = vz;
      if (ok) {
        rx = (c00 / det) * vx + (c10 / det) * vy + (c20 / det) * vz;
        ry = (c01 / det) * vx + (c11 / det) * vy + (c21 / det) * vz;
        rz = (c02 / det) * vx + (c12 / det) * vy + (c22 / det) * vz;
      }
      const float rn = sqrtf(rx * rx + ry * ry + rz * rz);
      a.crays[i * 3] = rx / rn; a.crays[i * 3 + 1] = ry / rn; a.crays[i * 3 + 2] = rz / rn;
      if (a.dpos) { a.dpos[i * 3] = d[0]; a.dpos[i * 3 + 1] = d[1]; a.dpos[i * 3 + 2] = d[2]; }
      if (a.inv_ok) a.inv_ok[i] = ok ? 1 : 0;
    }
  }
}

struct RenderEmbedArgs {
  long long P;
  const float* pts;
  const float* views;
  const float* normals;
  const float* feat;
  int feat_ld, feat_col0, nfeat, feat_row_stride;
  int multires;
  float pw[16];
  float* out;
  int ld;
};
__global__ void render_embed_kernel(const __grid_constant__ RenderEmbedArgs a) {
  const long long total = a.P * (long long)a.ld;
  const int pe = 3 + 6 * a.multires;
  for (long long idx = (long long)blockIdx.x * blockDim.x + threadIdx.x; idx < total;
       idx += (long long)gridDim.x * blockDim.x) {
    const int k = (int)(idx % a.ld);
    const long long p = idx / a.ld;
    float v = 0.f;
    if (k < 3) v = a.pts[p * 3 + k];
    else if (k < 3 + pe) {
      const int q = k - 3;
      if (q < 3) v = a.views[p * 3 + q];
      else {
        const int b = (q - 3) / 6, w6 = (q - 3) % 6, j = w6 % 3;
        float sn, cs;
        sincosf(a.views[p * 3 + j] * (float)(1 << b), &sn, &cs);
        v = a.pw[b] * (w6 >= 3 ? cs : sn);
      }
    } else if (k < 3 + pe + 3) v = a.normals[p * 3 + (k - 3 - pe)];
    else if (k < 3 + pe + 3 + a.nfeat)
      v = a.feat[(size_t)p * a.feat_row_stride * a.feat_ld + a.feat_col0 + (k - 3 - pe - 3)];
    a.out[idx] = v;
  }
}

}

extern "C" {

int sr_tc_shade_point(int64_t P, const float* pts, const float* rays, const int64_t* batch_inds,
                      const float* sdf4, int ld_s, const float* off4, const sr_lbs_params* lbs,
                      float* normals, float* crays, float* dpos, uint8_t* inv_ok, cudaStream_t s) {
  if (P <= 0 || !pts || !rays || !sdf4 || !normals || !crays) return SR_EINVAL;
  ShadePtArgs a;
  a.P = P; a.pts = pts; a.rays = rays; a.batch_inds = (const long long*)batch_inds; a.sdf4 = sdf4;
  a.ld_s = ld_s; a.off4 = off4; a.has_lbs = lbs ? 1 : 0;
  if (lbs) a.lbs = *lbs;
  a.normals = normals; a.crays = crays; a.dpos = dpos; a.inv_ok = inv_ok;
  shade_point_kernel<<<sr_grid_for(P * 32, 256, 8), 256, 0, s>>>(a);
  return sr_launch_status();
}

int sr_tc_render_embed(int64_t P, const float* pts, const float* views, const float* normals,
                       const float* feat, int feat_ld, int feat_col0, int nfeat, int feat_row_stride,
                       int multires, const float* pw, float* out, int ld, cudaStream_t s) {
  if (P <= 0 || !pts || !views || !normals || !out || !pw || (nfeat > 0 && !feat)) return SR_EINVAL;
  if (ld < 3 + 3 + 6 * multires + 3 + nfeat) return SR_EINVAL;
  RenderEmbedArgs a;
  a.P = P; a.pts = pts; a.views = views; a.normals = normals; a.feat = feat; a.feat_ld = feat_ld;
  a.feat_col0 = feat_col0; a.nfeat = nfeat; a.feat_row_stride = feat_row_stride; a.multires = multires;
  for (int i = 0; i < 16; ++i) a.pw[i] = i < multires ? pw[i] : 0.f;
  a.out = out; a.ld = ld;
  render_embed_kernel<<<sr_grid_for(P * (long long)ld, 256, 8), 256, 0, s>>>(a);
  return sr_launch_status();
}

int sr_tc_trace_mid(const int32_t* index, const int32_t* m_dev, int64_t P, const float* pts,
                    const float* rays, const int64_t* batch_inds, const float* f, const float* off,
                    const sr_lbs_params* lbs, const sr_trace_params* tp, int do_update,
                    uint8_t* converged, float* dsdf, float* ddef, int ld, float* aux,
                    int32_t* recheck, int32_t* recheck_count, float eps_f, float eps_a, cudaStream_t s) {
  if (!pts || !rays || !f || !tp || !converged || !dsdf || !aux || P <= 0 || ld < 8) return SR_EINVAL;
  if ((recheck != nullptr) != (recheck_count != nullptr) || eps_f < 0.f || eps_a < 0.f) return SR_EINVAL;
  MidArgs a;
  a.index = index; a.m_dev = m_dev; a.P = P; a.pts = pts; a.rays = rays;
  a.batch_inds = (const long long*)batch_inds; a.f = f; a.off = off;
  a.has_lbs = lbs ? 1 : 0;
  if (lbs) a.lbs = *lbs;
  a.tp = *tp; a.do_update = do_update; a.converged = converged; a.dsdf = dsdf; a.ddef = ddef; a.ld = ld;
  a.aux = aux; a.recheck = recheck; a.recheck_count = recheck_count; a.eps_f = eps_f; a.eps_a = eps_a;
  trace_mid_kernel<<<sr_grid_for(P * 32, 256, 8), 256, 0, s>>>(a);
  return sr_launch_status();
}

int sr_tc_trace_update(const int32_t* index, const int32_t* m_dev, int64_t P, float* pts,
                       const float* gs, int gs_ld, const float* gskip, int gk_ld, const float* gd,
                       int gd_ld, const float* aux, int mr_s, const float* pw_s, int mr_d,
                       const float* pw_d, int32_t* active_out, int32_t* counter_out,
                       const uint8_t* converged, cudaStream_t s) {
  if (!pts || !gs || !aux || !active_out || !counter_out || !pw_s || P <= 0) return SR_EINVAL;
  UpdArgs a;
  a.index = index; a.m_dev = m_dev; a.P = P; a.pts = pts; a.gs = gs; a.gs_ld = gs_ld; a.gskip = gskip;
  a.gk_ld = gk_ld; a.gd = gd; a.gd_ld = gd_ld; a.aux = aux; a.mr_s = mr_s; a.mr_d = mr_d;
  for (int i = 0; i < 16; ++i) { a.pw_s[i] = i < mr_s ? pw_s[i] : 0.f; a.pw_d[i] = (pw_d && i < mr_d) ? pw_d[i] : 0.f; }
  a.active_out = active_out; a.counter_out = counter_out; a.converged = converged;
  trace_update_kernel<<<sr_grid_for(P, 256, 8), 256, 0, s>>>(a);
  return sr_launch_status();
}
}
```

selfreconcode_b200/ops.py:

```python
import ctypes as C
import math

import torch

from . import _lib
from ._lib import MlpDesc, LbsParams, TraceParams
from ._lib import check as _check


import os as _os

TC_ENABLED = _os.environ.get("SELFRECON_B200_TC", "1") != "0"
TC_MIN_POINTS = int(_os.environ.get("SELFRECON_B200_TC_MIN_POINTS", "2048"))

TC_EPS_F = float(_os.environ.get("SELFRECON_B200_TC_EPS_F", "4e-5"))
TC_EPS_A = float(_os.environ.get("SELFRECON_B200_TC_EPS_A", "1e-3"))
TC_REFINE = _os.environ.get("SELFRECON_B200_TC_REFINE", "1") != "0"
TC_REFINE_TRACE = _os.environ.get("SELFRECON_B200_TC_REFINE_TRACE", "0") != "0"
TC_DUAL_STREAM = _os.environ.get("SELFRECON_B200_TC_DUAL_STREAM", "1") != "0"

import itertools as _it
_uid_counter = _it.count()
LAUNCHES = 0

_KERNELS_PER_CALL = {"mc_count": 3}


def _stream():
    return C.c_void_p(torch.cuda.current_stream().cuda_stream)


def check(code, what):
    global LAUNCHES
    _check(code, what)
    LAUNCHES += _KERNELS_PER_CALL.get(what, 1)


def _p(t):
    return C.c_void_p(t.data_ptr()) if t is not None else C.c_void_p(0)


def _need_cuda(*ts):
    for t in ts:
        if t is not None and not t.is_cuda:
            raise RuntimeError("selfrecon_b200: expected a CUDA tensor (no CPU fallback)")


def minv3x3(ms):
    _need_cuda(ms)
    n = ms.shape[0]
    invs = torch.empty((n, 3, 3), dtype=ms.dtype, device=ms.device)
    checks = torch.empty((n,), dtype=torch.bool, device=ms.device)
    lib = _lib.load()
    with torch.cuda.device(ms.device):
        fn = lib.sr_minv3x3_f32 if ms.dtype == torch.float32 else lib.sr_minv3x3_f64
        check(fn(_p(ms), _p(invs), _p(checks), n, _stream()), "minv3x3")
    return invs, checks


def minv3x3_backward(grads, invs):
    _need_cuda(grads, invs)
    n = invs.shape[0]
    outs = torch.empty((n, 3, 3), dtype=invs.dtype, device=invs.device)
    lib = _lib.load()
    with torch.cuda.device(invs.device):
        fn = lib.sr_minv3x3_bwd_f32 if invs.dtype == torch.float32 else lib.sr_minv3x3_bwd_f64
        check(fn(_p(grads), _p(invs), _p(outs), n, _stream()), "minv3x3_bwd")
    return outs


def raster_mesh(verts_screen, faces, H, W):
    _need_cuda(verts_screen, faces)
    vs = verts_screen.detach().contiguous().float()
    fc = faces.contiguous().to(torch.int64)
    N, V, _ = vs.shape
    F = fc.shape[0]
    dev = vs.device
    keys = torch.empty((N, H, W), dtype=torch.int64, device=dev)
    p2f = torch.empty((N, H, W, 1), dtype=torch.int64, device=dev)
    bary = torch.empty((N, H, W, 1, 3), dtype=torch.float32, device=dev)
    zbuf = torch.empty((N, H, W, 1), dtype=torch.float32, device=dev)
    with torch.cuda.device(dev):
        check(_lib.load().sr_raster_mesh(_p(vs), _p(fc), N, V, F, int(H), int(W), _p(keys), _p(p2f), _p(bary),
                                         _p(zbuf), _stream()), "raster_mesh")
    return p2f, bary, zbuf


_KERNELS_PER_CALL["raster_mesh"] = 2


def mesh_vertex_normals(verts, faces, csr):
    _need_cuda(verts, faces, csr[0], csr[1])
    vs = verts.detach().contiguous().float()
    fc = faces.contiguous().to(torch.int64)
    off, fid = csr[0].contiguous().to(torch.int64), csr[1].contiguous().to(torch.int64)
    N, V, _ = vs.shape
    if off.numel() != V + 1:
        raise ValueError("mesh_vertex_normals: csr offsets must have V + 1 entries")
    out = torch.empty_like(vs)
    with torch.cuda.device(vs.device):
        check(_lib.load().sr_mesh_vertex_normals(_p(vs), _p(fc), _p(off), _p(fid), N, V, fc.shape[0], _p(out),
                                                 _stream()), "mesh_vertex_normals")
    return out


def shade_phong(verts, normals, faces, pix_to_face, bary, cam_pos, light_pos, params, colors=None):
    _need_cuda(verts, normals, faces, pix_to_face, bary, cam_pos, light_pos, colors)
    vs = verts.detach().contiguous().float()
    N, V, _ = vs.shape
    H, W = pix_to_face.shape[1], pix_to_face.shape[2]
    nr = normals.detach().contiguous().float()
    col = colors.detach().contiguous().float() if colors is not None else None
    fc = faces.contiguous().to(torch.int64)
    p2f = pix_to_face.contiguous().to(torch.int64)
    br = bary.detach().contiguous().float()
    cp = cam_pos.detach().float().reshape(-1, 3).expand(N, 3).contiguous()
    lp = light_pos.detach().float().reshape(-1, 3).expand(N, 3).contiguous()
    if nr.shape != vs.shape or (col is not None and col.shape != vs.shape) or p2f.numel() != N * H * W \
            or br.numel() != 3 * N * H * W:
        raise ValueError("shade_phong: inconsistent shapes")
    out = torch.empty((N, H, W, 4), dtype=torch.float32, device=vs.device)
    with torch.cuda.device(vs.device):
        check(_lib.load().sr_shade_phong(_p(vs), _p(nr), _p(col), _p(fc), N, V, fc.shape[0], _p(p2f), _p(br),
                                         int(H), int(W), _p(cp), _p(lp), C.byref(params), _p(out), _stream()),
              "shade_phong")
    return out


_KERNELS_PER_CALL.update({"mesh_vertex_normals": 1, "shade_phong": 1})


def svals3x3(J, want_v=True):
    _need_cuda(J)
    J = J.contiguous().float()
    n = J.shape[0]
    S = torch.empty((n, 3), dtype=torch.float32, device=J.device)
    V = torch.empty((n, 3, 3), dtype=torch.float32, device=J.device) if want_v else None
    with torch.cuda.device(J.device):
        check(_lib.load().sr_svals3x3_f32(_p(J), _p(S), _p(V), n, _stream()), "svals3x3")
    return S, V


def svals3x3_backward(J, S, V, gS):
    _need_cuda(J, S, V, gS)
    n = J.shape[0]
    gJ = torch.empty((n, 3, 3), dtype=torch.float32, device=J.device)
    with torch.cuda.device(J.device):
        check(_lib.load().sr_svals3x3_bwd_f32(_p(J.contiguous()), _p(S.contiguous()), _p(V.contiguous()),
                                              _p(gS.contiguous().float()), _p(gJ), n, _stream()), "svals3x3_bwd")
    return gJ


_mc_work = {}


def marching_cubes(sdfs, xstep=1.0, ystep=1.0, zstep=1.0, xmin=0.0, ymin=0.0, zmin=0.0, iso=0.0,
                   i_offset=0):
    _need_cuda(sdfs)
    nx, ny, nz = sdfs.shape
    lib = _lib.load()
    dev = sdfs.device
    with torch.cuda.device(dev):
        wb = lib.sr_mc_work_bytes(nx, ny, nz)
        key = (dev.index, torch.cuda.current_stream().cuda_stream)
        work = _mc_work.get(key)
        if work is None or work.numel() < wb:
            work = torch.empty((wb,), dtype=torch.uint8, device=dev)
            _mc_work[key] = work
        counts = torch.empty((2,), dtype=torch.int32, device=dev)
        check(lib.sr_mc_count(_p(sdfs), nx, ny, nz, float(iso), _p(work), _p(counts), _stream()),
              "mc_count")
        nv, nf = counts.tolist()
        verts = torch.empty((nv, 3), dtype=torch.float32, device=dev)
        faces = torch.empty((nf, 3), dtype=torch.int64, device=dev)
        if nv or nf:
            check(lib.sr_mc_emit(_p(sdfs), nx, ny, nz, float(iso), float(xstep), float(ystep),
                                 float(zstep), float(xmin), float(ymin), float(zmin), int(i_offset),
                                 _p(work),
                                 _p(verts), nv, _p(faces), nf, _stream()), "mc_emit")
    return verts, faces


def marching_cubes_count(sdfs, iso=0.0):
    _need_cuda(sdfs)
    nx, ny, nz = sdfs.shape
    lib = _lib.load()
    dev = sdfs.device
    with torch.cuda.device(dev):
        wb = lib.sr_mc_work_bytes(nx, ny, nz)
        key = (dev.index, torch.cuda.current_stream().cuda_stream, "count")
        work = _mc_work.get(key)
        if work is None or work.numel() < wb:
            work = torch.empty((wb,), dtype=torch.uint8, device=dev)
            _mc_work[key] = work
        counts = torch.empty((2,), dtype=torch.int32, device=dev)
        check(lib.sr_mc_count(_p(sdfs), nx, ny, nz, float(iso), _p(work), _p(counts), _stream()), "mc_count")
        nv, nf = counts.tolist()
    return nv, nf


def interp2x3d_forward(inp, balance):
    _need_cuda(inp)
    b, c, d, h, w = inp.shape
    out = torch.empty((b, c, 2 * d - 1, 2 * h - 1, 2 * w - 1), dtype=inp.dtype, device=inp.device)
    bnd = torch.empty(out.shape, dtype=torch.bool, device=inp.device)
    lib = _lib.load()
    with torch.cuda.device(inp.device):
        check(lib.sr_interp2x3d_fwd_f32(_p(inp), _p(out), _p(bnd), b * c, d, h, w, float(balance),
                                        _stream()), "interp2x3d_fwd")
    return out, bnd


def interp2x3d_backward(grad_out):
    _need_cuda(grad_out)
    b, c, od, oh, ow = grad_out.shape
    d, h, w = (od + 1) // 2, (oh + 1) // 2, (ow + 1) // 2
    gin = torch.empty((b, c, d, h, w), dtype=grad_out.dtype, device=grad_out.device)
    lib = _lib.load()
    with torch.cuda.device(grad_out.device):
        check(lib.sr_interp2x3d_bwd_f32(_p(grad_out), _p(gin), b * c, d, h, w, _stream()),
              "interp2x3d_bwd")
    return gin


def interp2x2d_forward(inp, balance):
    _need_cuda(inp)
    b, c, h, w = inp.shape
    out = torch.empty((b, c, 2 * h - 1, 2 * w - 1), dtype=inp.dtype, device=inp.device)
    bnd = torch.empty(out.shape, dtype=torch.bool, device=inp.device)
    lib = _lib.load()
    with torch.cuda.device(inp.device):
        check(lib.sr_interp2x2d_fwd_f32(_p(inp), _p(out), _p(bnd), b * c, h, w, float(balance),
                                        _stream()), "interp2x2d_fwd")
    return out, bnd


def interp2x2d_backward(grad_out):
    _need_cuda(grad_out)
    b, c, oh, ow = grad_out.shape
    h, w = (oh + 1) // 2, (ow + 1) // 2
    gin = torch.empty((b, c, h, w), dtype=grad_out.dtype, device=grad_out.device)
    lib = _lib.load()
    with torch.cuda.device(grad_out.device):
        check(lib.sr_interp2x2d_bwd_f32(_p(grad_out), _p(gin), b * c, h, w, _stream()),
              "interp2x2d_bwd")
    return gin


def _istr(t):
    return (C.c_int64 * 5)(*t.stride())


def _gs_suffix(t):
    if t.dtype == torch.float32:
        return "f32"
    if t.dtype == torch.float64:
        return "f64"
    raise RuntimeError("grid_sampler_3d: only float32/float64 are supported")


def grid_sample3d_forward(inp, grid, want_corner_idx=False):
    _need_cuda(inp, grid)
    N, Cc, D, H, W = inp.shape
    Do, Ho, Wo = grid.shape[1:4]
    P = Do * Ho * Wo
    g = grid.reshape(N, P, 3).contiguous()
    out = torch.empty((N, Cc, Do, Ho, Wo), dtype=inp.dtype, device=inp.device)
    cidx = torch.empty((N, P, 3), dtype=torch.int32, device=inp.device) if want_corner_idx else None
    lib = _lib.load()
    with torch.cuda.device(inp.device):
        fn = getattr(lib, "sr_grid_sample3d_fwd_" + _gs_suffix(inp))
        check(fn(_p(inp), _istr(inp), _p(g), _p(out), _p(cidx), N, Cc, D, H, W, P, _stream()),
              "grid_sample3d_fwd")
    return (out, cidx) if want_corner_idx else out


def grid_sample3d_backward(inp, grid, grad_output):
    _need_cuda(inp, grid, grad_output)
    N, Cc, D, H, W = inp.shape
    Do, Ho, Wo = grid.shape[1:4]
    P = Do * Ho * Wo
    g = grid.reshape(N, P, 3).contiguous()
    go = grad_output.reshape(N, Cc, P).contiguous()
    ginp = torch.zeros((N, Cc, D, H, W), dtype=inp.dtype, device=inp.device)
    ggrid = torch.empty((N, P, 3), dtype=inp.dtype, device=inp.device)
    lib = _lib.load()
    with torch.cuda.device(inp.device):
        fn = getattr(lib, "sr_grid_sample3d_bwd_" + _gs_suffix(inp))
        check(fn(_p(inp), _istr(inp), _p(g), _p(go), _p(ginp), _p(ggrid), N, Cc, D, H, W, P,
                 _stream()), "grid_sample3d_bwd")
    return ginp, ggrid.reshape(grid.shape)


def grid_sample3d_dbackward(gg_input, gg_grid, inp, grid, grad_output):
    _need_cuda(gg_input, gg_grid, inp, grid, grad_output)
    N, Cc, D, H, W = inp.shape
    Do, Ho, Wo = grid.shape[1:4]
    P = Do * Ho * Wo
    g = grid.reshape(N, P, 3).contiguous()
    go = grad_output.reshape(N, Cc, P).contiguous()
    ggi = gg_input.contiguous()
    ggg = gg_grid.reshape(N, P, 3).contiguous()
    ginp = torch.zeros((N, Cc, D, H, W), dtype=inp.dtype, device=inp.device)
    ggrid = torch.empty((N, P, 3), dtype=inp.dtype, device=inp.device)
    ggout = torch.empty((N, Cc, P), dtype=inp.dtype, device=inp.device)
    lib = _lib.load()
    with torch.cuda.device(inp.device):
        fn = getattr(lib, "sr_grid_sample3d_dbwd_" + _gs_suffix(inp))
        check(fn(_p(ggi), _p(ggg), _p(inp), _istr(inp), _p(g), _p(go), _p(ginp), _p(ggrid),
                 _p(ggout), N, Cc, D, H, W, P, _stream()), "grid_sample3d_dbwd")
    return ginp, ggrid.reshape(grid.shape), ggout.reshape(grad_output.shape)


def _pad(x, m):
    return (x + m - 1) // m * m


class FusedMLP:

    def __init__(self, d_in, multires, device):
        self.d_in = int(d_in)
        self.multires = int(multires)
        self.device = torch.device(device)
        self.bufs = []
        self.desc = MlpDesc()
        self._sig = None
        self.uid = next(_uid_counter)

    def fold(self, linears, pe_w=None):
        d = self.desc
        d.n_layers = len(linears)
        d.d_in = self.d_in
        d.multires = self.multires
        pw = pe_w if pe_w is not None else [1.0] * self.multires
        for i in range(16):
            d.pe_w[i] = float(pw[i]) if i < len(pw) else 0.0
        if len(linears) > _lib.SR_MLP_MAX_LAYERS:
            raise RuntimeError("FusedMLP: too many layers")
        self._linears = linears
        self._lay = []
        with torch.cuda.device(self.device):
            for i, L in enumerate(linears):
                n, k = L["v"].shape
                _need_cuda(L["v"])
                npad, kpad = _pad(n, 128), _pad(k, 8)
                if npad > 512 or kpad > 512:
                    raise RuntimeError("FusedMLP: layer %dx%d exceeds the 512-wide engine" % (n, k))
                wt = torch.empty((kpad, npad), dtype=torch.float32, device=self.device)
                bias = torch.empty((npad,), dtype=torch.float32, device=self.device)
                wb = torch.empty((_pad(n, 8), _pad(k, 128)), dtype=torch.float32, device=self.device)
                self._lay.append(dict(wt=wt, bias=bias, wb=wb, n=n, k=k, npad=npad, kpad=kpad))
                ly = d.layer[i]
                ly.wt, ly.bias, ly.wb = wt.data_ptr(), bias.data_ptr(), wb.data_ptr()
                ly.k, ly.n, ly.kpad, ly.npad = k, n, kpad, npad
                ly.act = int(L["act"])
                ly.skip = 1 if L.get("skip") else 0
        self.bufs = [t for e in self._lay for t in (e["wt"], e["bias"], e["wb"])]
        self._children = []
        self.version = 0
        self.refold()
        return self

    def refold(self):
        lib = _lib.load()
        with torch.cuda.device(self.device):
            for e, L in zip(self._lay, self._linears):
                v = L["v"].detach().contiguous().float()
                g, b = L.get("g"), L.get("b")
                g = g.detach().contiguous().float().view(-1) if g is not None else None
                b = b.detach().contiguous().float() if b is not None else None
                check(lib.sr_fold_linear(_p(v), _p(g), _p(b), e["n"], e["k"], e["npad"], e["kpad"], _p(e["wt"]),
                                         _p(e["bias"]), _p(e["wb"]), _stream()), "fold_linear")
        self.version += 1
        for c in self._children:
            c._refresh_from_parent()
        tc = getattr(self, "_tc", None)
        if tc is not None:
            tc.repack()
        return self

    def set_pe_weights(self, pe_w):
        for i in range(16):
            self.desc.pe_w[i] = float(pe_w[i]) if i < len(pe_w) else 0.0

    def truncated_last(self, n_out):
        t = FusedMLP(self.d_in, self.multires, self.device)
        C.memmove(C.byref(t.desc), C.byref(self.desc), C.sizeof(MlpDesc))
        last = t.desc.layer[t.desc.n_layers - 1]
        e = self._lay[-1]
        npad = _pad(n_out, 128)
        t._own = None
        if npad != e["npad"]:
            t._own = (e["wt"][:, :npad].contiguous(), e["bias"][:npad].contiguous(), npad)
            last.wt = t._own[0].data_ptr()
            last.bias = t._own[1].data_ptr()
            last.npad = npad
        last.n = n_out
        t._parent = self
        t._lay = self._lay[:-1] + [dict(e, n=n_out, npad=npad, wt=t._own[0] if t._own else e["wt"],
                                        bias=t._own[1] if t._own else e["bias"])]
        t.bufs = [x for x in (t._own[:2] if t._own else [])]
        t._children = []
        t.version = self.version
        self._children.append(t)
        return t

    def _refresh_from_parent(self):
        if self._own is not None:
            e = self._parent._lay[-1]
            self._own[0].copy_(e["wt"][:, :self._own[2]])
            self._own[1].copy_(e["bias"][:self._own[2]])
        self.version = self._parent.version
        tc = getattr(self, "_tc", None)
        if tc is not None:
            tc.repack()


def annealing_weights(multires, ratio):
    if ratio is None:
        return [1.0] * multires
    if ratio <= 0:
        return [0.0] * multires
    alpha = ratio * multires
    return [(1.0 - math.cos(math.pi * min(max(alpha - float(i), 0.0), 1.0))) / 2.0
            for i in range(multires)]


def sdf_forward(net, pts, want_grad=False, nfeat=0):
    _need_cuda(pts)
    pts = pts.contiguous().float()
    P = pts.shape[0]
    dev = pts.device
    sdf = torch.empty((P,), dtype=torch.float32, device=dev)
    grad = torch.empty((P, 3), dtype=torch.float32, device=dev) if want_grad else None
    feat = torch.empty((P, nfeat), dtype=torch.float32, device=dev) if nfeat else None
    lib = _lib.load()
    with torch.cuda.device(dev):
        check(lib.sr_sdf_forward(C.byref(net.desc), _p(pts), P, _p(sdf), _p(grad), _p(feat),
                                 int(nfeat), _stream()), "sdf_forward")
    return sdf, grad, feat


_band_scratch = {}
SMALL_REFINE = _os.environ.get("SELFRECON_B200_SMALL_REFINE", "1") != "0"
SMALL_CAP = 4096
_KERNELS_PER_CALL["sdf_forward_small"] = 10


def sdf_refine_band(net, pts, sdf, center=0.0, eps=None):
    _need_cuda(pts, sdf)
    eps = TC_EPS_F if eps is None else float(eps)
    P = sdf.numel()
    if P == 0:
        return sdf
    dev = sdf.device
    lib = _lib.load()
    with torch.cuda.device(dev):
        key = (dev.index, torch.cuda.current_stream().cuda_stream)
        buf = _band_scratch.get(key)
        if buf is None or buf.numel() < P + 1:
            buf = torch.empty((max(P + 1, 1 << 16),), dtype=torch.int32, device=dev)
            _band_scratch[key] = buf
        cnt, lst = buf[0:1], buf[1:]
        cnt.zero_()
        check(lib.sr_band_select(_p(sdf), P, float(center), eps, _p(lst), _p(cnt), _stream()), "band_select")
        if SMALL_REFINE:
            wkey = key + ("small",)
            work = _band_scratch.get(wkey)
            if work is None:
                work = torch.empty((lib.sr_sdf_small_work_bytes(SMALL_CAP),), dtype=torch.uint8, device=dev)
                _band_scratch[wkey] = work
            check(lib.sr_sdf_forward_small(C.byref(net.desc), _p(pts), P, _p(lst), _p(cnt), _p(sdf), _p(work),
                                           SMALL_CAP, _stream()), "sdf_forward_small")
            over = _band_scratch.get(key + ("over",))
            if over is None:
                over = torch.empty((1,), dtype=torch.int32, device=dev)
                _band_scratch[key + ("over",)] = over
            torch.clamp(cnt - SMALL_CAP, min=0, out=over)
            if P > SMALL_CAP:
                check(lib.sr_sdf_forward_indexed(C.byref(net.desc), _p(pts), P, _p(lst[SMALL_CAP:]), _p(over), _p(sdf),
                                                 _stream()), "sdf_forward_indexed")
        else:
            check(lib.sr_sdf_forward_indexed(C.byref(net.desc), _p(pts), P, _p(lst), _p(cnt), _p(sdf), _stream()),
                  "sdf_forward_indexed")
    return sdf


class LbsState:

    def __init__(self, ws_ncdhw, bmin, bmax, Js, parents, init_pose_inv):
        _need_cuda(ws_ncdhw)
        dev = ws_ncdhw.device
        _, c, D, H, W = ws_ncdhw.shape
        assert c == 24
        self.D, self.H, self.W = D, H, W
        self.device = dev
        self.ws_cl = torch.empty((D, H, W, 24), dtype=torch.float32, device=dev)
        lib = _lib.load()
        with torch.cuda.device(dev):
            check(lib.sr_lbs_weights_to_channels_last(_p(ws_ncdhw.contiguous().float()),
                                                      _p(self.ws_cl), D, H, W, _stream()),
                  "lbs_weights_to_channels_last")
        self.bmin = [float(x) for x in bmin.view(-1).tolist()]
        self.bmax = [float(x) for x in bmax.view(-1).tolist()]
        self.Js = Js.detach().contiguous().float().view(24, 3)
        self.parents = torch.as_tensor(parents, dtype=torch.int32, device=dev).contiguous()
        self.ipi = init_pose_inv.detach().contiguous().float() if init_pose_inv is not None else None
        self.A = None
        self.trans = None
        self.params = LbsParams()

    def set_pose(self, poses, trans, want_posed_joints=False):
        F = poses.shape[0]
        poses = poses.detach().contiguous().float().view(F, 24, 3)
        self.trans = trans.detach().contiguous().float().view(F, 3)
        self.A = torch.empty((F, 24, 4, 4), dtype=torch.float32, device=self.device)
        pj = torch.empty((F, 24, 3), dtype=torch.float32, device=self.device) if want_posed_joints else None
        lib = _lib.load()
        with torch.cuda.device(self.device):
            check(lib.sr_lbs_bone_transforms(_p(poses), _p(self.Js), _p(self.parents), _p(self.ipi),
                                             F, _p(self.A), _p(pj), _stream()), "lbs_bone_transforms")
        p = self.params
        p.ws_cl = self.ws_cl.data_ptr()
        p.D, p.H, p.W = self.D, self.H, self.W
        for i in range(3):
            p.bmin[i] = self.bmin[i]
            p.bmax[i] = self.bmax[i]
        p.A = self.A.data_ptr()
        p.trans = self.trans.data_ptr()
        p.F = F
        return pj


def _lbs_ref(lbs):
    return C.byref(lbs.params) if lbs is not None else None


def deform_forward(net, lbs, pts, batch_inds, conds, want_jac=False, want_offset=False,
                   want_corner_idx=False, pts_per_frame=0):
    _need_cuda(pts)
    pts = pts.contiguous().float().view(-1, 3)
    P = pts.shape[0]
    dev = pts.device
    conds = conds.detach().contiguous().float() if conds is not None else None
    condlen = conds.shape[-1] if conds is not None else 0
    bi = batch_inds.contiguous().to(torch.int64) if batch_inds is not None else None
    d = torch.empty((P, 3), dtype=torch.float32, device=dev)
    off = torch.empty((P, 3), dtype=torch.float32, device=dev) if want_offset else None
    jac = torch.empty((P, 3, 3), dtype=torch.float32, device=dev) if want_jac else None
    ci = torch.empty((P, 3), dtype=torch.int32, device=dev) if want_corner_idx else None
    lib = _lib.load()
    with torch.cuda.device(dev):
        check(lib.sr_deform_forward(C.byref(net.desc), _lbs_ref(lbs), _p(pts), _p(bi),
                                    int(pts_per_frame), _p(conds), condlen, P, _p(d), _p(off),
                                    _p(jac), _p(ci), _stream()), "deform_forward")
    return d, off, jac, ci


def render_forward(net, pts, normals, views, feat):
    _need_cuda(pts, normals, views)
    P = pts.shape[0]
    dev = pts.device
    nfeat = feat.shape[1] if feat is not None else 0
    rgb = torch.empty((P, 3), dtype=torch.float32, device=dev)
    lib = _lib.load()
    with torch.cuda.device(dev):
        check(lib.sr_render_forward(C.byref(net.desc), _p(pts.contiguous().float()),
                                    _p(normals.contiguous().float()), _p(views.contiguous().float()),
                                    _p(feat.contiguous().float() if feat is not None else None),
                                    nfeat, P, _p(rgb), _stream()), "render_forward")
    return rgb


_scratch = {}


_host_cache = {}


def _host_floats(t):
    if not t.is_cuda:
        return tuple(float(x) for x in t.detach().reshape(-1).tolist())
    key = (t.device.index, t.data_ptr(), t._version, t.numel())
    v = _host_cache.get(key)
    if v is None:
        if len(_host_cache) > 64:
            _host_cache.clear()
        v = tuple(float(x) for x in t.detach().reshape(-1).tolist())
        _host_cache[key] = v
    return v


def _trace_scratch(dev):
    key = (dev.index, torch.cuda.current_stream(dev).cuda_stream)
    if key not in _scratch:
        n = _lib.load().sr_trace_scratch_bytes()
        _scratch[key] = torch.empty((n // 4,), dtype=torch.float32, device=dev)
    return _scratch[key]


def trace_surface_points(sdf_net, def_net, lbs, cam_pos, rays, init_pts, batch_inds, conds,
                         dthreshold=5e-5, athreshold=0.02, w1=3.05, w2=1.0, times=5,
                         return_counters=False, mode="auto"):
    if mode == "auto":
        mode = "tc" if (TC_ENABLED and init_pts.shape[0] >= TC_MIN_POINTS) else "reverse"
    if mode == "tc":
        return trace_surface_points_tc(sdf_net, def_net, lbs, cam_pos, rays, init_pts, batch_inds, conds,
                                       dthreshold, athreshold, w1, w2, times, return_counters)
    _need_cuda(rays, init_pts)
    dev = init_pts.device
    P = init_pts.shape[0]
    pts = init_pts.detach().contiguous().float().clone()
    rays = rays.detach().contiguous().float()
    bi = batch_inds.contiguous().to(torch.int64) if batch_inds is not None else None
    conds = conds.detach().contiguous().float() if conds is not None else None
    condlen = conds.shape[-1] if conds is not None else 0
    conv = torch.zeros((P,), dtype=torch.bool, device=dev)
    if P == 0:
        return (pts, conv, torch.zeros((times + 3,), dtype=torch.int32, device=dev)) if return_counters \
            else (pts, conv)
    lists = [torch.empty((P,), dtype=torch.int32, device=dev) for _ in range(2)]
    counters = torch.zeros((times + 3,), dtype=torch.int32, device=dev)
    tp = TraceParams()
    cp = _host_floats(cam_pos)
    for i in range(3):
        tp.cam_pos[i] = cp[i]
    tp.dthreshold, tp.athreshold, tp.w1, tp.w2 = float(dthreshold), float(athreshold), float(w1), float(w2)
    lib = _lib.load()
    dref = C.byref(def_net.desc) if def_net is not None else None
    with torch.cuda.device(dev):
        scratch = _trace_scratch(dev) if mode == "reverse" else None
        for it in range(times + 1):
            a_in = lists[(it + 1) & 1] if it > 0 else None
            a_out = lists[it & 1] if it < times else None
            if mode == "reverse":
                check(lib.sr_trace_step_rev(C.byref(sdf_net.desc), dref, _lbs_ref(lbs), C.byref(tp),
                                            _p(pts), _p(rays), _p(bi), _p(conds), condlen, P, _p(a_in),
                                            _p(a_out), _p(counters), it, _p(conv), _p(scratch),
                                            _stream()), "trace_step_rev")
            else:
                check(lib.sr_trace_step(C.byref(sdf_net.desc), dref, _lbs_ref(lbs), C.byref(tp),
                                        _p(pts), _p(rays), _p(bi), _p(conds), condlen, P, _p(a_in),
                                        _p(a_out), _p(counters), it, _p(conv), _stream()),
                      "trace_step")
    if return_counters:
        return pts, conv, counters
    return pts, conv


def shade_geometry(sdf_net, def_net, lbs, pts, rays, batch_inds, conds, nfeat=0, want_dpos=False):
    _need_cuda(pts, rays)
    dev = pts.device
    P = pts.shape[0]
    pts = pts.detach().contiguous().float()
    rays = rays.detach().contiguous().float()
    bi = batch_inds.contiguous().to(torch.int64) if batch_inds is not None else None
    conds = conds.detach().contiguous().float() if conds is not None else None
    condlen = conds.shape[-1] if conds is not None else 0
    normals = torch.empty((P, 3), dtype=torch.float32, device=dev)
    crays = torch.empty((P, 3), dtype=torch.float32, device=dev)
    feat = torch.empty((P, nfeat), dtype=torch.float32, device=dev) if nfeat else None
    dpos = torch.empty((P, 3), dtype=torch.float32, device=dev) if want_dpos else None
    ok = torch.empty((P,), dtype=torch.bool, device=dev)
    lib = _lib.load()
    with torch.cuda.device(dev):
        check(lib.sr_shade_geometry(C.byref(sdf_net.desc),
                                    C.byref(def_net.desc) if def_net is not None else None, _lbs_ref(lbs),
                                    _p(pts), _p(rays), _p(bi), _p(conds), condlen, P, _p(normals),
                                    _p(crays), _p(feat), int(nfeat), _p(dpos), _p(ok), _stream()),
              "shade_geometry")
    return normals, crays, feat, dpos, ok


def seg3d_candidates(flag, calculated, stride_zyx):
    _need_cuda(flag, calculated)
    D, H, W = flag.shape
    fD, fH, fW = calculated.shape
    cand = torch.empty((D, H, W), dtype=torch.bool, device=flag.device)
    lib = _lib.load()
    with torch.cuda.device(flag.device):
        check(lib.sr_seg3d_candidates(_p(flag.contiguous()), _p(calculated), _p(cand), D, H, W,
                                      int(stride_zyx[0]), int(stride_zyx[1]), int(stride_zyx[2]),
                                      fD, fH, fW, _stream()), "seg3d_candidates")
    return cand


_KERNELS_PER_CALL.update({"seg3d_candidates": 2, "seg3d_scatter": 3})


def seg3d_gather(lin, level_hw, stride_zyx, calculated, bmin, bmax, grid_flat):
    _need_cuda(lin, calculated, grid_flat)
    n = lin.numel()
    dev = lin.device
    fD, fH, fW = calculated.shape
    pts = torch.empty((n, 3), dtype=torch.float32, device=dev)
    interp = torch.empty((n,), dtype=torch.float32, device=dev)
    lib = _lib.load()
    lo = (C.c_float * 3)(*[float(v) for v in bmin])
    hi = (C.c_float * 3)(*[float(v) for v in bmax])
    with torch.cuda.device(dev):
        check(lib.sr_seg3d_gather(_p(lin), n, int(level_hw[0]), int(level_hw[1]), int(stride_zyx[0]),
                                  int(stride_zyx[1]), int(stride_zyx[2]), fD, fH, fW, lo, hi, _p(grid_flat),
                                  _p(pts), _p(interp), _p(calculated), _stream()), "seg3d_gather")
    return pts, interp


def seg3d_scatter(lin, values, interp, balance, grid_flat):
    _need_cuda(lin, values, interp, grid_flat)
    dev = lin.device
    conflict = torch.empty((grid_flat.numel(),), dtype=torch.bool, device=dev)
    ncf = torch.empty((1,), dtype=torch.int32, device=dev)
    lib = _lib.load()
    with torch.cuda.device(dev):
        check(lib.sr_seg3d_scatter(_p(lin), lin.numel(), _p(values), _p(interp), float(balance), _p(grid_flat),
                                   _p(conflict), conflict.numel(), _p(ncf), _stream()), "seg3d_scatter")
    return conflict, ncf


def tc_pack_rows(x):
    _need_cuda(x)
    x = x.contiguous().float()
    M, K = x.shape
    lib = _lib.load()
    buf = torch.empty((lib.sr_tc_act_bytes(M, K),), dtype=torch.uint8, device=x.device)
    with torch.cuda.device(x.device):
        check(lib.sr_tc_pack_rows(_p(x), M, K, K, _p(buf), None, _stream()), "tc_pack_rows")
    return buf


def tc_pack_weights(w):
    _need_cuda(w)
    w = w.contiguous().float()
    N, K = w.shape
    lib = _lib.load()
    buf = torch.empty((lib.sr_tc_weight_bytes(N, K),), dtype=torch.uint8, device=w.device)
    with torch.cuda.device(w.device):
        check(lib.sr_tc_pack_weights(_p(w), N, K, K, _p(buf), _stream()), "tc_pack_weights")
    return buf


def tc_linear(A, W, bias, M, N, K, n_valid, act, ch=1, K_next=0, scale=1.0, skip_src=None, skip_n=0,
              want_out=False):
    lib = _lib.load()
    dev = A.device
    A_next = torch.empty((lib.sr_tc_act_bytes(M, K_next),), dtype=torch.uint8, device=dev) if K_next else None
    out = torch.empty((M, n_valid), dtype=torch.float32, device=dev) if want_out else None
    npad = (N + 255) // 256 * 256
    b = torch.zeros((npad,), dtype=torch.float32, device=dev)
    b[:bias.numel()] = bias.reshape(-1)
    with torch.cuda.device(dev):
        check(lib.sr_tc_linear(_p(A), _p(W), _p(b), M, N, K, n_valid, int(act), int(ch), _p(A_next),
                               int(K_next), float(scale), _p(skip_src), int(skip_n),
                               skip_src.shape[1] if skip_src is not None else 0, _p(out),
                               n_valid if want_out else 0, 0, n_valid, None, None, 0, 0, 1.0, None, _stream()),
              "tc_linear")
    return A_next, out, None


class TcNet:

    def __init__(self, fused):
        self.fused = fused
        d = fused.desc
        self.layers = []
        lib = _lib.load()
        dev = fused.device
        for i in range(d.n_layers):
            ly = d.layer[i]
            e = fused._lay[i]
            n, k = ly.n, ly.k
            W = torch.empty((lib.sr_tc_weight_bytes(n, k),), dtype=torch.uint8, device=dev)
            Wb = torch.empty((lib.sr_tc_weight_bytes(k, n),), dtype=torch.uint8, device=dev)
            self.layers.append(dict(W=W, Wb=Wb, bias=torch.zeros((_pad(n, 256),), dtype=torch.float32, device=dev),
                                    n=n, k=k, act=ly.act, skip=bool(ly.skip), _e=e,
                                    zero_bias=torch.zeros((_pad(k, 256),), dtype=torch.float32, device=dev)))
        self.c_layers = (_lib.TcLayer * len(self.layers))()
        for c, L in zip(self.c_layers, self.layers):
            c.W, c.Wb, c.bias, c.zero_bias = (L[t].data_ptr() for t in ("W", "Wb", "bias", "zero_bias"))
            c.n, c.k, c.act, c.skip = L["n"], L["k"], L["act"], int(L["skip"])
        self.repack()

    def repack(self):
        lib = _lib.load()
        with torch.cuda.device(self.fused.device):
            for L in self.layers:
                e, n, k = L["_e"], L["n"], L["k"]
                check(lib.sr_tc_pack_weights(_p(e["wb"]), n, k, e["wb"].shape[1], _p(L["W"]), _stream()),
                      "tc_pack_weights")
                check(lib.sr_tc_pack_weights(_p(e["wt"]), k, n, e["wt"].shape[1], _p(L["Wb"]), _stream()),
                      "tc_pack_weights")
                L["bias"][:n].copy_(e["bias"][:n])


def tc_net(fused):
    t = getattr(fused, "_tc", None)
    if t is None:
        t = TcNet(fused)
        fused._tc = t
    return t


def _tc_mlp(lib, tcn, x0, ch, out, A_in=None, acts=None, m_dev=None):
    global LAUNCHES
    M, ld = x0.shape
    L = len(tcn.layers)
    if A_in is None:
        A_in = torch.empty((lib.sr_tc_act_bytes(M, ld),), dtype=torch.uint8, device=x0.device)
        acts = [torch.empty((lib.sr_tc_act_bytes(M, _pad(ly["k"], 32)),), dtype=torch.uint8, device=x0.device)
                for ly in tcn.layers[1:]]
    acts_c = (C.c_void_p * max(L - 1, 1))(*[a.data_ptr() for a in acts])
    check(lib.sr_tc_mlp_forward(tcn.c_layers, L, _p(x0), M, ld, tcn.fused.desc.d_in, ch, _p(A_in), acts_c, None,
                                _p(out), _p(m_dev), out.shape[1], _stream()), "tc_mlp_forward")
    LAUNCHES += L


def tc_mlp_forward(fused, pts, ch=1, conds=None, batch_inds=None, pts_per_frame=0, n_out=None):
    _need_cuda(pts)
    net = tc_net(fused)
    d = fused.desc
    dev = pts.device
    pts = pts.contiguous().float().view(-1, 3)
    P = pts.shape[0]
    M = P * ch
    condlen = conds.shape[-1] if conds is not None else 0
    ld = _pad(d.d_in, 32)
    lib = _lib.load()
    emb = torch.empty((M, ld), dtype=torch.float32, device=dev)
    out = torch.empty((M, n_out or net.layers[-1]["n"]), dtype=torch.float32, device=dev)
    pw = (C.c_float * 16)(*[d.pe_w[i] for i in range(16)])
    bi = batch_inds.contiguous().to(torch.int64) if batch_inds is not None else None
    cd = conds.detach().contiguous().float() if conds is not None else None
    with torch.cuda.device(dev):
        check(lib.sr_tc_embed(_p(pts), P, d.multires, pw, ch, _p(cd), _p(bi), int(pts_per_frame), condlen,
                              _p(emb), ld, None, None, _stream()), "tc_embed")
        _tc_mlp(lib, net, emb, ch, out)
    return out


class _TcTraceBuffers:

    def __init__(self, dev, P, sdf_net, def_net):
        lib = _lib.load()
        self.P = P
        f32 = lambda *shape: torch.empty(shape, dtype=torch.float32, device=dev)
        u8 = lambda n: torch.empty((n,), dtype=torch.uint8, device=dev)
        self.ld_s = _pad(sdf_net.desc.d_in, 32)
        self.emb_s = f32(P, self.ld_s)
        widest = max([32] + [_pad(net.desc.layer[l].n, 32) for net in (sdf_net, def_net) if net is not None
                             for l in range(net.desc.n_layers - 1)])
        self.A = [u8(lib.sr_tc_act_bytes(P, widest)) for _ in range(2)]
        self.f = f32(P, 1)
        self.A_in = u8(lib.sr_tc_act_bytes(P, 256))
        self.acts_s = [u8(lib.sr_tc_act_bytes(P, _pad(sdf_net.desc.layer[i + 1].k, 32)))
                       for i in range(sdf_net.desc.n_layers - 1)]
        self.cot_s = f32(P, 32)
        self.cot_d = f32(P, 32)
        self.aux = f32(P, 8)
        self.gs = f32(P, 64)
        self.gskip = f32(P, 64)
        if def_net is not None:
            self.ld_d = _pad(def_net.desc.d_in, 32)
            self.emb_d = f32(P, self.ld_d)
            self.off = f32(P, 3)
            self.acts_d = [u8(lib.sr_tc_act_bytes(P, _pad(def_net.desc.layer[i + 1].k, 32)))
                           for i in range(def_net.desc.n_layers - 1)]
            self.gd = f32(P, 64)
            self.A_in_d = u8(lib.sr_tc_act_bytes(P, 256))
            self.A_d = [u8(lib.sr_tc_act_bytes(P, widest)) for _ in range(2)]
            self.gskip_d = f32(P, 64)


def _tc_backward_sweep(lib, tcn, cot, bufs, acts, P, m_dev, g_out, g_skip, n_keep):
    d_in = tcn.fused.desc.d_in
    cur, nxt = bufs
    check(lib.sr_tc_pack_rows(_p(cot), P, 32, 32, _p(cur), _p(m_dev), _stream()), "tc_pack_rows")
    K = 32
    for l in range(len(tcn.layers) - 1, -1, -1):
        ly = tcn.layers[l]
        scale = 0.7071067811865476 if ly["skip"] else 1.0
        if l > 0:
            n_prev = tcn.layers[l - 1]["n"]
            Kn = _pad(n_prev, 32)
            gk = g_skip if ly["skip"] else None
            check(lib.sr_tc_linear(_p(cur), _p(ly["Wb"]), _p(ly["zero_bias"]), P, ly["k"], K, n_prev, 0, 1, _p(nxt),
                                   Kn, scale, None, 0, 0, _p(gk), gk.shape[1] if gk is not None else 0, n_prev,
                                   d_in if gk is not None else 0, None, _p(acts[l - 1]), _pad(ly["k"], 32),
                                   tcn.layers[l - 1]["act"], scale, _p(m_dev), _stream()), "tc_linear")
            cur, nxt, K = nxt, cur, Kn
        else:
            check(lib.sr_tc_linear(_p(cur), _p(ly["Wb"]), _p(ly["zero_bias"]), P, ly["k"], K, ly["k"], 0, 1, None, 0,
                                   scale, None, 0, 0, _p(g_out), g_out.shape[1], 0, n_keep, None, None, 0, 0, 1.0,
                                   _p(m_dev), _stream()), "tc_linear")


class _TcTraceCtx:

    def __init__(self, dev, P, sdf_net, def_net, n_frames, condlen, times):
        self.B = _TcTraceBuffers(dev, P, sdf_net, def_net)
        self.pts = torch.empty((P, 3), dtype=torch.float32, device=dev)
        self.rays = torch.empty((P, 3), dtype=torch.float32, device=dev)
        self.bi = torch.empty((P,), dtype=torch.int64, device=dev)
        self.conds = torch.empty((n_frames, condlen), dtype=torch.float32, device=dev) if condlen else None
        self.conv = torch.empty((P,), dtype=torch.bool, device=dev)
        self.counters = torch.empty((times + 3,), dtype=torch.int32, device=dev)
        self.lists = [torch.empty((P,), dtype=torch.int32, device=dev) for _ in range(2)]
        self.lbsA = torch.empty((n_frames, 24, 4, 4), dtype=torch.float32, device=dev)
        self.lbsT = torch.empty((n_frames, 3), dtype=torch.float32, device=dev)
        self.lbs_params = LbsParams()
        self.side_stream = torch.cuda.Stream(device=dev)
        self.recheck = torch.empty((P,), dtype=torch.int32, device=dev)
        self.recheck_counts = torch.empty((times + 1,), dtype=torch.int32, device=dev)
        self.rev_scratch = _trace_scratch(dev)
        self.graph = None
        self.sig = None
        self.calls = 0
        self.n_launches = 0


_tc_trace_ctx = {}
GRAPHS_ENABLED = _os.environ.get("SELFRECON_B200_GRAPHS", "1") != "0"


def _tc_trace_body(lib, G, sdf_net, def_net, ts, td, tp, P, times, condlen, has_lbs):
    B = G.B
    ds, dd = sdf_net.desc, (def_net.desc if def_net is not None else None)
    pw_s = (C.c_float * 16)(*[ds.pe_w[i] for i in range(16)])
    pw_d = (C.c_float * 16)(*[dd.pe_w[i] for i in range(16)]) if dd is not None else None
    pts, rays, bi, conds, conv, counters, lists = G.pts, G.rays, G.bi, G.conds, G.conv, G.counters, G.lists
    lbs_ref = C.byref(G.lbs_params) if has_lbs else None
    conv.zero_()
    counters.zero_()
    counters[0:1].fill_(P)
    refine = TC_REFINE_TRACE
    if refine:
        G.recheck_counts.zero_()
    dref = C.byref(def_net.desc) if def_net is not None else None
    for it in range(times + 1):
        idx = lists[(it + 1) & 1] if it > 0 else None
        a_out = lists[it & 1] if it < times else None
        m_dev = counters[it:it + 1]
        check(lib.sr_tc_embed(_p(pts), P, ds.multires, pw_s, 1, None, None, 0, 0, _p(B.emb_s), B.ld_s,
                              _p(idx), _p(m_dev), _stream()), "tc_embed")
        dual = TC_DUAL_STREAM and def_net is not None
        if dual:
            main = torch.cuda.current_stream()
            side = G.side_stream
            side.wait_stream(main)
            with torch.cuda.stream(side):
                check(lib.sr_tc_embed(_p(pts), P, dd.multires, pw_d, 1, _p(conds), _p(bi), 0, condlen,
                                      _p(B.emb_d), B.ld_d, _p(idx), _p(m_dev), _stream()), "tc_embed")
                _tc_mlp(lib, td, B.emb_d, 1, B.off, B.A_in_d, B.acts_d, m_dev)
        _tc_mlp(lib, ts, B.emb_s, 1, B.f, B.A_in, B.acts_s, m_dev)
        if dual:
            main.wait_stream(side)
        elif def_net is not None:
            check(lib.sr_tc_embed(_p(pts), P, dd.multires, pw_d, 1, _p(conds), _p(bi), 0, condlen,
                                  _p(B.emb_d), B.ld_d, _p(idx), _p(m_dev), _stream()), "tc_embed")
            _tc_mlp(lib, td, B.emb_d, 1, B.off, B.A_in, B.acts_d, m_dev)
        check(lib.sr_tc_trace_mid(_p(idx), _p(m_dev), P, _p(pts), _p(rays), _p(bi), _p(B.f),
                                  _p(B.off) if def_net is not None else None, lbs_ref, C.byref(tp),
                                  1 if a_out is not None else 0, _p(conv), _p(B.cot_s),
                                  _p(B.cot_d) if def_net is not None else None, 32, _p(B.aux),
                                  _p(G.recheck) if refine else None,
                                  _p(G.recheck_counts[it:it + 1]) if refine else None,
                                  TC_EPS_F if refine else 0.0, TC_EPS_A if refine else 0.0, _stream()),
              "tc_trace_mid")
        if refine:
            check(lib.sr_trace_step_rev(C.byref(sdf_net.desc), dref, lbs_ref, C.byref(tp), _p(pts), _p(rays),
                                        _p(bi), _p(conds), condlen, P, _p(G.recheck), None,
                                        _p(G.recheck_counts), it, _p(conv), _p(G.rev_scratch), _stream()),
                  "trace_step_rev")
        if a_out is None:
            break
        if dual:
            side.wait_stream(main)
            with torch.cuda.stream(side):
                _tc_backward_sweep(lib, td, B.cot_d, B.A_d, B.acts_d, P, m_dev, B.gd, B.gskip_d, 3 + 6 * dd.multires)
        _tc_backward_sweep(lib, ts, B.cot_s, B.A, B.acts_s, P, m_dev, B.gs, B.gskip, ds.d_in)
        if dual:
            main.wait_stream(side)
        elif def_net is not None:
            _tc_backward_sweep(lib, td, B.cot_d, B.A, B.acts_d, P, m_dev, B.gd, B.gskip, 3 + 6 * dd.multires)
        has_skip = any(l["skip"] for l in ts.layers)
        check(lib.sr_tc_trace_update(_p(idx), _p(m_dev), P, _p(pts), _p(B.gs), B.gs.shape[1],
                                     _p(B.gskip) if has_skip else None, B.gskip.shape[1],
                                     _p(B.gd) if def_net is not None else None,
                                     B.gd.shape[1] if def_net is not None else 0, _p(B.aux), ds.multires,
                                     pw_s, dd.multires if dd is not None else 0, pw_d, _p(a_out),
                                     _p(counters[it + 1:it + 2]), _p(conv) if refine else None, _stream()),
              "tc_trace_update")


def trace_surface_points_tc(sdf_net, def_net, lbs, cam_pos, rays, init_pts, batch_inds, conds,
                            dthreshold=5e-5, athreshold=0.02, w1=3.05, w2=1.0, times=5,
                            return_counters=False):
    global LAUNCHES
    _need_cuda(rays, init_pts)
    dev = init_pts.device
    P = init_pts.shape[0]
    if P == 0:
        pts = init_pts.detach().float().clone()
        conv = torch.zeros((0,), dtype=torch.bool, device=dev)
        return (pts, conv, torch.zeros((times + 3,), dtype=torch.int32, device=dev)) if return_counters \
            else (pts, conv)
    lib = _lib.load()
    condlen = conds.shape[-1] if conds is not None else 0
    n_frames = lbs.A.shape[0] if lbs is not None else (conds.shape[0] if conds is not None else 1)
    cp = _host_floats(cam_pos)
    ds, dd = sdf_net.desc, (def_net.desc if def_net is not None else None)
    key = (dev.index, P, tuple(ds.layer[i].n for i in range(ds.n_layers)),
           tuple(dd.layer[i].n for i in range(dd.n_layers)) if dd is not None else (), n_frames, condlen,
           conds.shape[0] if conds is not None else 0, times)
    sig = (sdf_net.uid, def_net.uid if def_net is not None else -1,
           lbs.ws_cl.data_ptr() if lbs is not None else 0, cp, float(dthreshold), float(athreshold),
           float(w1), float(w2), tuple(ds.pe_w[i] for i in range(ds.multires)),
           tuple(dd.pe_w[i] for i in range(dd.multires)) if dd is not None else (),
           TC_REFINE_TRACE, TC_EPS_F, TC_EPS_A, TC_DUAL_STREAM)
    G = _tc_trace_ctx.get(key)
    if G is None:
        if len(_tc_trace_ctx) >= 4:
            _tc_trace_ctx.pop(next(iter(_tc_trace_ctx)))
        G = _TcTraceCtx(dev, P, sdf_net, def_net, n_frames, condlen, times)
        _tc_trace_ctx[key] = G
    if G.sig != sig:
        G.sig, G.graph, G.calls = sig, None, 0
    ts, td = tc_net(sdf_net), (tc_net(def_net) if def_net is not None else None)
    tp = TraceParams()
    for i in range(3):
        tp.cam_pos[i] = cp[i]
    tp.dthreshold, tp.athreshold, tp.w1, tp.w2 = float(dthreshold), float(athreshold), float(w1), float(w2)
    with torch.cuda.device(dev):
        G.pts.copy_(init_pts.detach().reshape(P, 3))
        G.rays.copy_(rays.detach().reshape(P, 3))
        if batch_inds is not None:
            G.bi.copy_(batch_inds.reshape(P))
        else:
            G.bi.zero_()
        if conds is not None:
            G.conds.copy_(conds.detach())
        if lbs is not None:
            G.lbsA.copy_(lbs.A)
            G.lbsT.copy_(lbs.trans)
            C.memmove(C.byref(G.lbs_params), C.byref(lbs.params), C.sizeof(LbsParams))
            G.lbs_params.A = G.lbsA.data_ptr()
            G.lbs_params.trans = G.lbsT.data_ptr()
        args = (lib, G, sdf_net, def_net, ts, td, tp, P, times, condlen, lbs is not None)
        if G.graph is not None:
            G.graph.replay()
            LAUNCHES += G.n_launches
        elif GRAPHS_ENABLED and G.calls >= 1:
            before = LAUNCHES
            g = torch.cuda.CUDAGraph()
            with torch.cuda.graph(g):
                _tc_trace_body(*args)
            G.n_launches = LAUNCHES - before
            G.graph = g
            g.replay()
        else:
            _tc_trace_body(*args)
        G.calls += 1
        out = (G.pts.clone(), G.conv.clone())
        if return_counters:
            out = out + (G.counters.clone(),)
    return out


_side_streams = {}


def _side_stream(dev):
    st = _side_streams.get(dev.index)
    if st is None:
        st = torch.cuda.Stream(device=dev)
        _side_streams[dev.index] = st
    return st


def shade_and_render_tc(sdf_full, def_net, lbs, render_net, pts, rays, batch_inds, conds, nfeat=256):
    _need_cuda(pts, rays)
    dev = pts.device
    P = pts.shape[0]
    pts = pts.detach().contiguous().float()
    rays = rays.detach().contiguous().float()
    bi = batch_inds.contiguous().to(torch.int64) if batch_inds is not None else None
    lib = _lib.load()
    with torch.cuda.device(dev):
        if TC_DUAL_STREAM and def_net is not None:
            main = torch.cuda.current_stream()
            side = _side_stream(dev)
            side.wait_stream(main)
            with torch.cuda.stream(side):
                o4 = tc_mlp_forward(def_net, pts, ch=4, conds=conds, batch_inds=bi)
            s4 = tc_mlp_forward(sdf_full, pts, ch=4)
            main.wait_stream(side)
            o4.record_stream(main)
        else:
            s4 = tc_mlp_forward(sdf_full, pts, ch=4)
            o4 = tc_mlp_forward(def_net, pts, ch=4, conds=conds, batch_inds=bi) if def_net is not None else None
        normals = torch.empty((P, 3), dtype=torch.float32, device=dev)
        crays = torch.empty((P, 3), dtype=torch.float32, device=dev)
        dpos = torch.empty((P, 3), dtype=torch.float32, device=dev)
        ok = torch.empty((P,), dtype=torch.bool, device=dev)
        check(lib.sr_tc_shade_point(P, _p(pts), _p(rays), _p(bi), _p(s4), s4.shape[1], _p(o4), _lbs_ref(lbs),
                                    _p(normals), _p(crays), _p(dpos), _p(ok), _stream()), "tc_shade_point")
        rd = render_net.desc
        ld = _pad(rd.d_in, 32)
        emb = torch.empty((P, ld), dtype=torch.float32, device=dev)
        pw = (C.c_float * 16)(*[rd.pe_w[i] for i in range(16)])
        check(lib.sr_tc_render_embed(P, _p(pts), _p(crays), _p(normals), _p(s4), s4.shape[1], 1, nfeat, 4,
                                     rd.multires, pw, _p(emb), ld, _stream()), "tc_render_embed")
        rn = tc_net(render_net)
        rgb = torch.empty((P, rn.layers[-1]["n"]), dtype=torch.float32, device=dev)
        _tc_mlp(lib, rn, emb, 1, rgb)
    return normals, crays, rgb, dpos, ok
```

selfreconcode_b200/train_ops.py:

```python
import ctypes as C

import torch

from . import _lib
from ._lib import SR_ACT_NONE
from . import ops
from .ops import _p, _pad, _stream, check

INV_SQRT2 = 0.7071067811865476


class MlpConfig:

    def __init__(self, acts, skips, d_in, ch, packs=None):
        self.acts = [int(a) for a in acts]
        self.skips = [bool(s) for s in skips]
        self.d_in = int(d_in)
        self.ch = int(ch)
        self.packs = packs


def _pack_weights(lib, w):
    w = w.contiguous()
    n, k = w.shape
    buf = torch.empty((lib.sr_tc_weight_bytes(n, k),), dtype=torch.uint8, device=w.device)
    check(lib.sr_tc_pack_weights(_p(w), n, k, w.shape[1], _p(buf), _stream()), "tc_pack_weights")
    return buf


class _Workspace:
    _pool = {}

    @classmethod
    def get(cls, dev, nbytes):
        key = (dev.index, torch.cuda.current_stream(dev).cuda_stream)
        buf = cls._pool.get(key)
        if buf is None or buf.numel() < nbytes:
            buf = torch.empty((int(nbytes),), dtype=torch.uint8, device=dev)
            cls._pool[key] = buf
        return buf


COLSUM_SLICES = 64
DEBUG_LAST = None


def _align(n, a=256):
    return (n + a - 1) // a * a


class _Arena:

    def __init__(self, dev):
        self.dev = dev
        self.sizes = []

    def add(self, nbytes):
        off = sum(self.sizes)
        self.sizes.append(_align(int(nbytes)))
        return len(self.sizes) - 1, off

    def alloc(self):
        self.buf = torch.empty((max(sum(self.sizes), 1),), dtype=torch.uint8, device=self.dev)
        self.base = self.buf.data_ptr()
        return self

    def ptr(self, off):
        return self.base + off


def _layer_array(lib, cfg, Ws, bs, dev):
    L = len(Ws)
    arr = (_lib.TcLayer * L)()
    keep = []
    for i in range(L):
        n, k = Ws[i].shape
        pk = cfg.packs[i] if cfg.packs is not None else None
        if pk is not None and (pk["n"], pk["k"]) == (n, k):
            W, Wb, bias, zb = pk["W"], pk["Wb"], pk["bias"], pk["zero_bias"]
        else:
            W = _pack_weights(lib, Ws[i])
            Wb = _pack_weights(lib, Ws[i].t().contiguous())
            bias = torch.zeros((_pad(n, 256),), dtype=torch.float32, device=dev)
            if bs[i] is not None:
                bias[:n] = bs[i].detach().float()
            zb = torch.zeros((_pad(k, 256),), dtype=torch.float32, device=dev)
        keep += [W, Wb, bias, zb]
        a = arr[i]
        a.W, a.Wb, a.bias, a.zero_bias = W.data_ptr(), Wb.data_ptr(), bias.data_ptr(), zb.data_ptr()
        a.n, a.k, a.act, a.skip = n, k, cfg.acts[i], 1 if cfg.skips[i] else 0
    return arr, keep


class TcMlpFunction(torch.autograd.Function):
    @staticmethod
    def forward(ctx, x0, cfg, *wb):
        lib = _lib.load()
        dev = x0.device
        if not x0.is_cuda:
            raise RuntimeError("TcMlpFunction: CUDA tensors required (no CPU path)")
        x0 = x0.detach().contiguous().float()
        M, ld = x0.shape
        L = len(wb) // 2
        Ws = [wb[2 * i].detach().contiguous().float() for i in range(L)]
        bs = [wb[2 * i + 1] for i in range(L)]
        ch = cfg.ch
        with torch.cuda.device(dev):
            layers, keep = _layer_array(lib, cfg, Ws, bs, dev)
            ar = _Arena(dev)
            _, o_in = ar.add(lib.sr_tc_act_bytes(M, ld))
            o_act, o_st = [], []
            for i in range(L - 1):
                o_act.append(ar.add(lib.sr_tc_act_bytes(M, _pad(Ws[i + 1].shape[1], 32)))[1])
                o_st.append(ar.add(M * _pad(Ws[i].shape[0], 256) * 4)[1] if cfg.acts[i] == _lib.SR_ACT_SOFTPLUS100 else None)
            ar.alloc()
            acts = (C.c_void_p * max(L - 1, 1))(*[ar.ptr(o) for o in o_act])
            stashes = (C.c_void_p * max(L - 1, 1))(*[ar.ptr(o) if o is not None else None for o in o_st])
            out = torch.empty((M, Ws[-1].shape[0]), dtype=torch.float32, device=dev)
            check(lib.sr_tc_mlp_forward(layers, L, _p(x0), M, ld, cfg.d_in, ch, C.c_void_p(ar.ptr(o_in)), acts, stashes,
                                        _p(out), None, 0, _stream()), "tc_mlp_forward")
            ops.LAUNCHES += L
        ctx.cfg, ctx.M, ctx.ld, ctx.L = cfg, M, ld, L
        ctx.arena, ctx.o_in, ctx.acts_c, ctx.stashes_c, ctx.o_act = ar, o_in, acts, stashes, o_act
        ctx.layers, ctx.keep, ctx.shapes = layers, keep, [tuple(w.shape) for w in Ws]
        ctx.has_bias = [b is not None for b in bs]
        if DEBUG_LAST is not None:
            views = [ar.buf[o:o + lib.sr_tc_act_bytes(M, _pad(Ws[i + 1].shape[1], 32))] for i, o in enumerate(o_act)]
            DEBUG_LAST.update(acts=views, M=M, widths=[w.shape[0] for w in Ws], kpads=[_pad(w.shape[1], 32) for w in Ws])
        return out

    @staticmethod
    @torch.autograd.function.once_differentiable
    def backward(ctx, gout):
        lib = _lib.load()
        cfg, M, ld, L, shapes = ctx.cfg, ctx.M, ctx.ld, ctx.L, ctx.shapes
        ch = cfg.ch
        dev = gout.device
        need_x0 = ctx.needs_input_grad[0]
        with torch.cuda.device(dev):
            g = gout.detach().contiguous().float()
            wmax = max(_pad(n, 32) for n, _ in shapes)
            ar = _Arena(dev)
            o_d0 = ar.add(lib.sr_tc_act_bytes(M, wmax))[1]
            o_d1 = ar.add(lib.sr_tc_act_bytes(M, wmax))[1]
            kxs = [ld] + [_pad(k, 32) for _, k in shapes[1:]]
            o_part = ar.add(max(lib.sr_tc_wgrad_partial_bytes(M, _pad(n, 32), kx, None)
                                for (n, _), kx in zip(shapes, kxs)))[1]
            o_cs = ar.add(COLSUM_SLICES * wmax * 4)[1]
            gs_ld = _pad(cfg.d_in, 4)
            o_gs = ar.add(M * gs_ld * 4)[1] if any(cfg.skips) else None
            ar.alloc()
            sizes = [n * k for n, k in shapes] + [n for n, _ in shapes]
            flat = torch.empty((sum(sizes),), dtype=torch.float32, device=dev)
            dWs, dbs, o = [], [], 0
            for n, k in shapes:
                dWs.append(flat[o:o + n * k].view(n, k))
                o += n * k
            for n, _ in shapes:
                dbs.append(flat[o:o + n])
                o += n
            want_w = [ctx.needs_input_grad[2 + 2 * l] for l in range(L)]
            want_b = [ctx.has_bias[l] and ctx.needs_input_grad[3 + 2 * l] for l in range(L)]
            dW_c = (C.c_void_p * L)(*[dWs[l].data_ptr() if want_w[l] else None for l in range(L)])
            db_c = (C.c_void_p * L)(*[dbs[l].data_ptr() if want_b[l] else None for l in range(L)])
            x0_grad = torch.empty((M, ld), dtype=torch.float32, device=dev) if need_x0 else None
            fa = ctx.arena
            check(lib.sr_tc_mlp_backward(ctx.layers, L, M, ld, cfg.d_in, ch, _p(g), C.c_void_p(fa.ptr(ctx.o_in)), ctx.acts_c,
                                         ctx.stashes_c, C.c_void_p(ar.ptr(o_d0)), C.c_void_p(ar.ptr(o_d1)),
                                         C.c_void_p(ar.ptr(o_part)), C.c_void_p(ar.ptr(o_cs)), COLSUM_SLICES, dW_c, db_c,
                                         _p(x0_grad), C.c_void_p(ar.ptr(o_gs)) if o_gs is not None else None, gs_ld,
                                         _stream()), "tc_mlp_backward")
            ops.LAUNCHES += 5 * L
        grads = []
        for l in range(L):
            grads += [dWs[l] if want_w[l] else None, dbs[l] if want_b[l] else None]
        ctx.arena = ctx.keep = None
        return (x0_grad, None) + tuple(grads)


def unpack_tiles(tiles, M, K):
    lib = _lib.load()
    out = torch.empty((M, K), dtype=torch.float32, device=tiles.device)
    with torch.cuda.device(tiles.device):
        check(lib.sr_tc_unpack_rows(_p(tiles), M, K, _pad(K, 32), _p(out), K, _stream()), "tc_unpack_rows")
    return out


def tc_mlp(x0, cfg, weights, biases):
    flat = []
    for w, b in zip(weights, biases):
        flat += [w, b]
    return TcMlpFunction.apply(x0, cfg, *flat)


class EmbedRowsFunction(torch.autograd.Function):

    @staticmethod
    def forward(ctx, p, extra, multires, pe_w, ch, width):
        lib = _lib.load()
        pts = p.detach().contiguous().float()
        P = pts.shape[0]
        E = extra.shape[1] if extra is not None else 0
        out = torch.empty((P * ch, width), dtype=torch.float32, device=pts.device)
        pw = (C.c_float * 16)(*[float(pe_w[i]) if i < multires else 0.0 for i in range(16)])
        ex = extra.detach().contiguous().float() if extra is not None else None
        with torch.cuda.device(pts.device):
            check(lib.sr_tc_embed(_p(pts), P, multires, pw, ch, _p(ex), None, 1 if ex is not None else 0, E, _p(out), width,
                                  None, None, _stream()), "tc_embed")
        ctx.save_for_backward(pts)
        ctx.meta = (multires, [float(pe_w[i]) for i in range(multires)], ch, width, E)
        return out

    @staticmethod
    @torch.autograd.function.once_differentiable
    def backward(ctx, gx):
        (pts,) = ctx.saved_tensors
        multires, pe_w, ch, width, E = ctx.meta
        lib = _lib.load()
        P = pts.shape[0]
        gx = gx.contiguous().float()
        gp = ge = None
        if ctx.needs_input_grad[0]:
            gp = torch.empty((P, 3), dtype=torch.float32, device=pts.device)
            pw = (C.c_float * 16)(*[pe_w[i] if i < multires else 0.0 for i in range(16)])
            with torch.cuda.device(pts.device):
                check(lib.sr_tc_embed_backward(_p(pts), P, multires, pw, ch, _p(gx), width, _p(gp), _stream()),
                      "tc_embed_backward")
        if E and ctx.needs_input_grad[1]:
            pe = 3 + 6 * multires
            ge = gx.view(P, ch, width)[:, 0, pe:pe + E]
        return gp, ge, None, None, None, None


EMBED_KERNELS = True


def embed_rows(p, multires, pe_w, ch, extra=None, ld=None):
    P = p.shape[0]
    if EMBED_KERNELS and p.is_cuda and p.dtype == torch.float32 and multires <= 8:
        E0 = extra.shape[1] if extra is not None else 0
        width0 = ld if ld is not None else _pad(3 + 6 * multires + E0, 32)
        return EmbedRowsFunction.apply(p, extra, multires, list(pe_w), ch, width0)
    freqs = [float(2 ** k) for k in range(multires)]
    vals = [p]
    for k, fr in enumerate(freqs):
        w = float(pe_w[k])
        vals += [w * torch.sin(p * fr), w * torch.cos(p * fr)]
    val = torch.cat(vals, dim=1)
    pe = val.shape[1]
    E = extra.shape[1] if extra is not None else 0
    width = ld if ld is not None else _pad(pe + E, 32)
    if ch == 1:
        parts = [val] + ([extra] if extra is not None else [])
        row = torch.cat(parts, dim=1)
        return torch.nn.functional.pad(row, (0, width - row.shape[1]))
    eye = torch.eye(3, dtype=p.dtype, device=p.device)
    tans = [eye.unsqueeze(0).expand(P, 3, 3)]
    for k, fr in enumerate(freqs):
        w = float(pe_w[k]) * fr
        tans += [torch.diag_embed(w * torch.cos(p * fr)), torch.diag_embed(-w * torch.sin(p * fr))]
    tan = torch.cat(tans, dim=2)
    rows = torch.cat([val.unsqueeze(1), tan], dim=1)
    if extra is not None:
        ex = torch.cat([extra.unsqueeze(1), torch.zeros(P, 3, E, dtype=p.dtype, device=p.device)], dim=1)
        rows = torch.cat([rows, ex], dim=2)
    rows = torch.nn.functional.pad(rows, (0, width - rows.shape[2]))
    return rows.reshape(P * 4, width)


def weight_norm_eff(v, g):
    if g is None:
        return v
    return v * (g.view(-1, 1) / v.norm(dim=1, keepdim=True))


class WeightNormAllFunction(torch.autograd.Function):

    @staticmethod
    def forward(ctx, *vg):
        lib = _lib.load()
        L = len(vg) // 2
        vs = [vg[2 * i].detach().contiguous().float() for i in range(L)]
        gs = [vg[2 * i + 1].detach().reshape(-1).contiguous().float() for i in range(L)]
        dev = vs[0].device
        nk = [tuple(v.shape) for v in vs]
        wbuf = torch.empty((sum(n * k for n, k in nk),), dtype=torch.float32, device=dev)
        inv = torch.empty((sum(n for n, _ in nk),), dtype=torch.float32, device=dev)
        arr = (_lib.WnLayer * L)()
        outs, o, r = [], 0, 0
        for i, (n, k) in enumerate(nk):
            w = wbuf[o:o + n * k].view(n, k)
            c = arr[i]
            c.v, c.g, c.w, c.inv_norm = vs[i].data_ptr(), gs[i].data_ptr(), w.data_ptr(), inv[r:r + n].data_ptr()
            c.gw, c.gv, c.gg, c.n, c.k, c.gw_ld = None, None, None, n, k, k
            outs.append(w)
            o += n * k
            r += n
        with torch.cuda.device(dev):
            check(lib.sr_weight_norm_forward(arr, L, torch.cuda.current_stream().cuda_stream), "weight_norm_forward")
        ctx.save_for_backward(inv, *vs, *gs)
        ctx.nk = nk
        ctx.g_shapes = [vg[2 * i + 1].shape for i in range(L)]
        return tuple(outs)

    @staticmethod
    @torch.autograd.function.once_differentiable
    def backward(ctx, *gws):
        lib = _lib.load()
        saved = ctx.saved_tensors
        inv = saved[0]
        L = len(ctx.nk)
        vs, gs = saved[1:1 + L], saved[1 + L:1 + 2 * L]
        dev = inv.device
        gvbuf = torch.empty((sum(n * k for n, k in ctx.nk),), dtype=torch.float32, device=dev)
        ggbuf = torch.empty((sum(n for n, _ in ctx.nk),), dtype=torch.float32, device=dev)
        arr = (_lib.WnLayer * L)()
        keep, res, o, r = [], [], 0, 0
        for i, (n, k) in enumerate(ctx.nk):
            gw = gws[i]
            if gw is not None and (gw.dtype != torch.float32 or gw.stride(1) != 1):
                gw = gw.float().contiguous()
            keep.append(gw)
            gv, gg = gvbuf[o:o + n * k].view(n, k), ggbuf[r:r + n]
            c = arr[i]
            c.v, c.g, c.w, c.inv_norm = vs[i].data_ptr(), gs[i].data_ptr(), None, inv[r:r + n].data_ptr()
            c.gw = gw.data_ptr() if gw is not None else None
            c.gv, c.gg, c.n, c.k, c.gw_ld = gv.data_ptr(), gg.data_ptr(), n, k, (gw.stride(0) if gw is not None else k)
            res += [gv, gg.view(ctx.g_shapes[i])]
            o += n * k
            r += n
        with torch.cuda.device(dev):
            check(lib.sr_weight_norm_backward(arr, L, torch.cuda.current_stream().cuda_stream), "weight_norm_backward")
        return tuple(res)


import os as _os

FUSED_WEIGHT_NORM = _os.environ.get("SELFRECON_B200_FUSED_WN", "0") != "0"


def weight_norm_all(lins, fused=None):
    if lins and (FUSED_WEIGHT_NORM if fused is None else fused) and lins[0].weight_v.is_cuda and len(lins) <= 12:
        vg = []
        for lin in lins:
            vg += [lin.weight_v, lin.weight_g]
        return list(WeightNormAllFunction.apply(*vg))
    return [weight_norm_eff(lin.weight_v, lin.weight_g) for lin in lins]


TC_TRAIN_ENABLED = _os.environ.get("SELFRECON_B200_TC_TRAIN", "1") != "0"


def small_matmul(a, b):
    return (a.unsqueeze(-1) * b.unsqueeze(-3)).sum(-2)


def small_matvec(m, v):
    return (m * v.unsqueeze(-2)).sum(-1)


def small_mattvec(m, v):
    return (m * v.unsqueeze(-1)).sum(-2)
```

Measured before the change: 1.017 million.

## Compute SDF normals via reverse-mode backward sweep instead of 4-channel forward

Shading previously ran the SDF MLP with four channels (value plus three tangents) to obtain gradients. It now runs a one-channel forward pass and a reverse-mode backward sweep through a truncated net, then folds the embedding backward, including the skip-connection gradient, into the point gradient. This cuts GEMM width roughly fourfold for the forward pass. To support it, the GEMM gains a narrow 64-column tile path using m64n64k16 wgmma, the head weights are cached in packed form, and the shade buffers persist across calls. It adds a backward pass and more code paths that could hide bugs.

```diff
diff --git a/include/selfrecon_b200.h b/include/selfrecon_b200.h
--- a/include/selfrecon_b200.h
+++ b/include/selfrecon_b200.h
@@ -152,7 +152,7 @@
                 float* out, int ld, const int32_t* index ,
                 const int32_t* m_dev , cudaStream_t s);
 int sr_tc_embed_backward(const float* pts, int64_t P, int multires, const float* pe_w, int ch, const float* gx, int ld,
-                         float* gp, cudaStream_t s);
+                         const float* gk, int gk_ld, float* gp, cudaStream_t s);
 int64_t sr_tc_act_bytes(int64_t M, int K);
 int64_t sr_tc_weight_bytes(int N, int K);
 int sr_tc_pack_rows(const float* src, int64_t M, int K, int ld, void* dst, const int32_t* m_dev,
@@ -240,7 +240,7 @@
                        const uint8_t* converged , cudaStream_t s);
 
 int sr_tc_shade_point(int64_t P, const float* pts, const float* rays, const int64_t* batch_inds,
-                      const float* sdf4, int ld_s, const float* off4, const sr_lbs_params* lbs,
+                      const float* grad, const float* off4, const sr_lbs_params* lbs,
                       float* normals, float* crays, float* dpos, uint8_t* inv_ok, cudaStream_t s);
 int sr_tc_render_embed(int64_t P, const float* pts, const float* views, const float* normals,
                        const float* feat, int feat_ld, int feat_col0, int nfeat, int feat_row_stride,
diff --git a/selfreconcode_b200/_lib.py b/selfreconcode_b200/_lib.py
--- a/selfreconcode_b200/_lib.py
+++ b/selfreconcode_b200/_lib.py
@@ -102,7 +102,7 @@
                                     stream_t]),
     "sr_tc_embed": (C.c_int, [c_f, i64, i32, C.POINTER(f32), i32, c_f, c_f, i64, i32, c_f, i32, c_f, c_f,
                               stream_t]),
-    "sr_tc_embed_backward": (C.c_int, [c_f, i64, i32, C.POINTER(f32), i32, c_f, i32, c_f, stream_t]),
+    "sr_tc_embed_backward": (C.c_int, [c_f, i64, i32, C.POINTER(f32), i32, c_f, i32, c_f, i32, c_f, stream_t]),
     "sr_tc_act_bytes": (i64, [i64, i32]),
     "sr_tc_weight_bytes": (i64, [i32, i32]),
     "sr_tc_pack_rows": (C.c_int, [c_f, i64, i32, i32, c_f, c_f, stream_t]),
@@ -136,8 +136,8 @@
     "sr_sdf_small_work_bytes": (i64, [i32]),
     "sr_sdf_forward_small": (C.c_int, [C.POINTER(MlpDesc), c_f, i64, c_f, c_f, c_f, c_f, i32, stream_t]),
     "sr_sdf_forward_indexed": (C.c_int, [C.POINTER(MlpDesc), c_f, i64, c_f, c_f, c_f, stream_t]),
-    "sr_tc_shade_point": (C.c_int, [i64, c_f, c_f, c_f, c_f, i32, c_f, C.POINTER(LbsParams), c_f, c_f, c_f,
-                                    c_f, stream_t]),
+    "sr_tc_shade_point": (C.c_int, [i64, c_f, c_f, c_f, c_f, c_f, C.POINTER(LbsParams), c_f, c_f, c_f, c_f,
+                                    stream_t]),
     "sr_tc_render_embed": (C.c_int, [i64, c_f, c_f, c_f, c_f, i32, i32, i32, i32, i32, C.POINTER(f32), c_f,
                                      i32, stream_t]),
     "sr_seg3d_candidates": (C.c_int, [c_f, c_f, c_f, i32, i32, i32, i32, i32, i32, i32, i32, i32,
diff --git a/selfreconcode_b200/csrc/tc_common.cuh b/selfreconcode_b200/csrc/tc_common.cuh
--- a/selfreconcode_b200/csrc/tc_common.cuh
+++ b/selfreconcode_b200/csrc/tc_common.cuh
@@ -9,18 +9,17 @@
 #define SR_TC_PLANES 2
 #endif
 constexpr int kPlanes = SR_TC_PLANES;
-constexpr int BM = 128, BN = 256, BK = 32, STAGES = kPlanes == 2 ? 3 : 2;
+constexpr int BM = 128, BN = 256, BN_NARROW = 64, BK = 32, STAGES = kPlanes == 2 ? 3 : 2;
 constexpr int A_PLANE = BM * BK;
-constexpr int W_PLANE = BN * BK;
 constexpr int A_STAGE = kPlanes * A_PLANE;
-constexpr int W_STAGE = kPlanes * W_PLANE;
-constexpr uint32_t A_STAGE_BYTES = A_STAGE * 2, W_STAGE_BYTES = W_STAGE * 2;
+constexpr uint32_t A_STAGE_BYTES = A_STAGE * 2;
+__host__ __device__ constexpr int tile_n(int N) { return N <= BN_NARROW ? BN_NARROW : BN; }
 
 __host__ __device__ inline size_t a_tile_off(long long mt, int kc, int KC, int p) {
   return (((size_t)mt * KC + kc) * kPlanes + p) * A_PLANE;
 }
-__host__ __device__ inline size_t w_tile_off(int nt, int kc, int KC, int p) {
-  return (((size_t)nt * KC + kc) * kPlanes + p) * W_PLANE;
+__host__ __device__ inline size_t w_tile_off(int bn, int nt, int kc, int KC, int p) {
+  return (((size_t)nt * KC + kc) * kPlanes + p) * (size_t)(bn * BK);
 }
 __device__ __forceinline__ int in_tile_off(int rows_per_tile, int r, int k) {
   return (k >> 3) * (rows_per_tile * 8) + (r >> 3) * 64 + (r & 7) * 8 + (k & 7);
@@ -76,8 +75,25 @@
                  : SR_ACC128(SR_INOUT, d)
                  : "l"(adesc), "l"(bdesc), "r"(1), "n"(TA), "n"(TB));
 }
+#define SR_WGMMA_M64N64K16_BF16                                                                                    \
+  "{\n\t.reg .pred p;\n\tsetp.ne.b32 p, %34, 0;\n\t"                                                             \
+  "wgmma.mma_async.sync.aligned.m64n64k16.f32.bf16.bf16 "                                                          \
+  "{%0, %1, %2, %3, %4, %5, %6, %7, %8, %9, %10, %11, %12, %13, %14, %15, %16, %17, %18, %19, %20, %21, %22, "     \
+  "%23, %24, %25, %26, %27, %28, %29, %30, %31}, %32, %33, p, 1, 1, %35, %36;\n\t}\n"
+template <int TA, int TB, bool FIRST>
+__device__ __forceinline__ void wgmma_m64n64k16(float (&d)[32], uint64_t adesc, uint64_t bdesc) {
+  if constexpr (FIRST)
+    asm volatile(SR_WGMMA_M64N64K16_BF16
+                 : SR_ACC32(SR_OUT, d, 0)
+                 : "l"(adesc), "l"(bdesc), "r"(0), "n"(TA), "n"(TB));
+  else
+    asm volatile(SR_WGMMA_M64N64K16_BF16
+                 : SR_ACC32(SR_INOUT, d, 0)
+                 : "l"(adesc), "l"(bdesc), "r"(1), "n"(TA), "n"(TB));
+}
 #undef SR_OUT
 #undef SR_INOUT
+#undef SR_WGMMA_M64N64K16_BF16
 #undef SR_WGMMA_M64N256K16_BF16
 #undef SR_ACC128
 #undef SR_ACC32
diff --git a/selfreconcode_b200/csrc/tc_gemm.cu b/selfreconcode_b200/csrc/tc_gemm.cu
--- a/selfreconcode_b200/csrc/tc_gemm.cu
+++ b/selfreconcode_b200/csrc/tc_gemm.cu
@@ -101,15 +101,13 @@
 
 struct EpiRow {
   long long mt, row;
-  int nt, row_in_tile, lane;
+  int row_in_tile, lane;
   bool row_ok, is_val;
   size_t ds_ld;
 };
 
 template <int ACT, int CH, bool MUL, bool PF = true>
-__device__ __forceinline__ void epi_chunk(const LayerArgs& a, const EpiRow& r, uint32_t (&v)[32], int chunk,
-                                          bool live) {
-  const int c0 = r.nt * BN + chunk * 32;
+__device__ __forceinline__ void epi_chunk(const LayerArgs& a, const EpiRow& r, uint32_t (&v)[32], int c0, bool live) {
   float o[32];
   if (live) {
     if constexpr (MUL) {
@@ -269,11 +267,16 @@
 constexpr int kEpiWarps = 4 * kConsumerWGs;
 constexpr int STG_LD = 132;
 constexpr int STG_FLOATS = 64 * STG_LD;
-constexpr size_t kSmem = (size_t)STAGES * (A_STAGE_BYTES + W_STAGE_BYTES) + (size_t)kConsumerWGs * STG_FLOATS * 4 + 256;
-static_assert(kSmem <= 227 * 1024, "shared memory of one H100 block");
-
-template <bool FIRST>
-__device__ __forceinline__ void mma_chunk(float (&acc)[128], uint32_t abase, uint32_t wbase) {
+template <int TBN>
+constexpr uint32_t w_stage_bytes() { return (uint32_t)kPlanes * TBN * BK * 2; }
+template <int TBN>
+constexpr size_t smem_bytes() {
+  return (size_t)STAGES * (A_STAGE_BYTES + w_stage_bytes<TBN>()) + (size_t)kConsumerWGs * STG_FLOATS * 4 + 256;
+}
+static_assert(smem_bytes<BN>() <= 227 * 1024, "shared memory of one H100 block");
+
+template <int TBN, bool FIRST>
+__device__ __forceinline__ void mma_chunk(float (&acc)[TBN / 2], uint32_t abase, uint32_t wbase) {
   constexpr int kTerms = kPlanes == 2 ? 3 : 6;
   const int pa[6] = {0, 1, 0, 2, 1, 0}, pw[6] = {1, 0, 0, 0, 1, 0};
   const int pa3[6] = {0, 2, 1, 0, 1, 0}, pw3[6] = {2, 0, 1, 1, 0, 0};
@@ -283,15 +286,24 @@
     for (int jj = 0; jj < BK / 16; ++jj) {
       const int qa = kPlanes == 2 ? pa[q] : pa3[q], qw = kPlanes == 2 ? pw[q] : pw3[q];
       const uint64_t ad = make_desc(abase + qa * (A_PLANE * 2) + jj * 2 * (BM * 16), BM * 16, 128);
-      const uint64_t bd = make_desc(wbase + qw * (W_PLANE * 2) + jj * 2 * (BN * 16), BN * 16, 128);
-      if (FIRST && q == 0 && jj == 0) wgmma_m64n256k16<0, 0, true>(acc, ad, bd);
-      else wgmma_m64n256k16<0, 0, false>(acc, ad, bd);
-    }
-  }
-}
-
-template <int ACT, int CH, bool MUL>
+      const uint64_t bd = make_desc(wbase + qw * (TBN * BK * 2) + jj * 2 * (TBN * 16), TBN * 16, 128);
+      const bool first = FIRST && q == 0 && jj == 0;
+      if constexpr (TBN == BN) {
+        if (first) wgmma_m64n256k16<0, 0, true>(acc, ad, bd);
+        else wgmma_m64n256k16<0, 0, false>(acc, ad, bd);
+      } else {
+        static_assert(TBN == BN_NARROW, "column tile");
+        if (first) wgmma_m64n64k16<0, 0, true>(acc, ad, bd);
+        else wgmma_m64n64k16<0, 0, false>(acc, ad, bd);
+      }
+    }
+  }
+}
+
+template <int ACT, int CH, bool MUL, int TBN>
 __global__ void __launch_bounds__(kThreads, 1) tc_sweep_kernel(const __grid_constant__ LayerArgs a) {
+  constexpr uint32_t W_STAGE_BYTES = w_stage_bytes<TBN>();
+  constexpr int W_STAGE = W_STAGE_BYTES / 2;
   extern __shared__ __align__(1024) unsigned char smem[];
   __nv_bfloat16* sA = reinterpret_cast<__nv_bfloat16*>(smem);
   __nv_bfloat16* sW = reinterpret_cast<__nv_bfloat16*>(smem + (size_t)STAGES * A_STAGE_BYTES);
@@ -327,7 +339,7 @@
           for (int kc = 0; kc < a.KC; ++kc) {
             sr_mbar_wait(&empty[slot], phase ^ 1u);
             sr_mbar_arrive_expect_tx(&full[slot], A_STAGE_BYTES + W_STAGE_BYTES);
-            sr_bulk_g2s(sW + (size_t)slot * W_STAGE, a.W + w_tile_off(nt, kc, a.KC, 0), W_STAGE_BYTES, &full[slot]);
+            sr_bulk_g2s(sW + (size_t)slot * W_STAGE, a.W + w_tile_off(TBN, nt, kc, a.KC, 0), W_STAGE_BYTES, &full[slot]);
             sr_bulk_g2s(sA + (size_t)slot * A_STAGE, a.A + a_tile_off(mt, kc, a.KC, 0), A_STAGE_BYTES, &full[slot]);
             if (++slot == STAGES) { slot = 0; phase ^= 1u; }
           }
@@ -339,12 +351,12 @@
     const int cw = wg - 1;
     const int wq = warp & 3;
     float* st = stg + cw * STG_FLOATS;
-    float acc[128];
+    float acc[TBN / 2];
     EpiRow r;
     r.row_in_tile = cw * 64 + (wq & 1) * 32 + lane;
     r.lane = lane;
     r.is_val = (CH == 1) || ((lane & 3) == 0);
-    r.ds_ld = MUL ? (size_t)((a.n + BN - 1) / BN) * BN : (size_t)a.NT * BN;
+    r.ds_ld = (size_t)(((MUL ? a.n : a.n_gemm) + BN - 1) / BN) * BN;
     int slot = 0;
     uint32_t phase = 0;
     for (int j = 0; j < J; ++j) {
@@ -352,19 +364,18 @@
       r.row = r.mt * BM + r.row_in_tile;
       r.row_ok = r.row < Mrows;
       for (int nt = 0; nt < a.NT; ++nt) {
-        r.nt = nt;
         sr_mbar_wait(&full[slot], phase);
         wgmma_fence();
-        mma_chunk<true>(acc, sr_smem_u32(sA + (size_t)slot * A_STAGE) + cw * 8 * 128,
-                        sr_smem_u32(sW + (size_t)slot * W_STAGE));
+        mma_chunk<TBN, true>(acc, sr_smem_u32(sA + (size_t)slot * A_STAGE) + cw * 8 * 128,
+                             sr_smem_u32(sW + (size_t)slot * W_STAGE));
         wgmma_commit();
         int prev = slot;
         if (++slot == STAGES) { slot = 0; phase ^= 1u; }
         for (int kc = 1; kc < a.KC; ++kc) {
           sr_mbar_wait(&full[slot], phase);
           wgmma_fence();
-          mma_chunk<false>(acc, sr_smem_u32(sA + (size_t)slot * A_STAGE) + cw * 8 * 128,
-                           sr_smem_u32(sW + (size_t)slot * W_STAGE));
+          mma_chunk<TBN, false>(acc, sr_smem_u32(sA + (size_t)slot * A_STAGE) + cw * 8 * 128,
+                                sr_smem_u32(sW + (size_t)slot * W_STAGE));
           wgmma_commit();
           wgmma_wait<1>();
           if (lane == 0) sr_mbar_arrive(&empty[prev]);
@@ -373,20 +384,21 @@
         }
         wgmma_wait<0>();
         if (lane == 0) sr_mbar_arrive(&empty[prev]);
-#pragma unroll
-        for (int h = 0; h < 2; ++h) {
+        constexpr int PASS = TBN < 128 ? TBN : 128, FRAGS = PASS / 8, WCH = PASS / 64;
+#pragma unroll
+        for (int h = 0; h < TBN / PASS; ++h) {
           const int fr = 16 * wq + (lane >> 2), fc = 2 * (lane & 3);
 #pragma unroll
-          for (int i = 0; i < 16; ++i) {
+          for (int i = 0; i < FRAGS; ++i) {
             *reinterpret_cast<float2*>(st + fr * STG_LD + 8 * i + fc) =
-                make_float2(acc[4 * (16 * h + i)], acc[4 * (16 * h + i) + 1]);
+                make_float2(acc[4 * (FRAGS * h + i)], acc[4 * (FRAGS * h + i) + 1]);
             *reinterpret_cast<float2*>(st + (fr + 8) * STG_LD + 8 * i + fc) =
-                make_float2(acc[4 * (16 * h + i) + 2], acc[4 * (16 * h + i) + 3]);
+                make_float2(acc[4 * (FRAGS * h + i) + 2], acc[4 * (FRAGS * h + i) + 3]);
           }
           warpgroup_sync(1 + cw);
-          const float* srow = st + ((wq & 1) * 32 + lane) * STG_LD + (wq >> 1) * 64;
-          for (int i = 0; i < 2; ++i) {
-            const int chunk = 4 * h + 2 * (wq >> 1) + i;
+          const float* srow = st + ((wq & 1) * 32 + lane) * STG_LD + (wq >> 1) * (PASS / 2);
+          for (int i = 0; i < WCH; ++i) {
+            const int c0 = nt * TBN + h * PASS + (wq >> 1) * (PASS / 2) + 32 * i;
             uint32_t v[32];
 #pragma unroll
             for (int j4 = 0; j4 < 8; ++j4) {
@@ -394,7 +406,7 @@
               v[4 * j4] = __float_as_uint(t.x); v[4 * j4 + 1] = __float_as_uint(t.y);
               v[4 * j4 + 2] = __float_as_uint(t.z); v[4 * j4 + 3] = __float_as_uint(t.w);
             }
-            epi_chunk<ACT, CH, MUL>(a, r, v, chunk, nt * BN + chunk * 32 < a.n_gemm);
+            epi_chunk<ACT, CH, MUL>(a, r, v, c0, c0 < a.n_gemm);
           }
           warpgroup_sync(1 + cw);
         }
@@ -471,14 +483,15 @@
 
 __global__ void pack_weights_kernel(const float* __restrict__ w, int N, int K, int ld,
                                     __nv_bfloat16* __restrict__ dst, int NT, int KC) {
-  const long long total = (long long)NT * BN * KC * 4;
+  const int bn = tile_n(N);
+  const long long total = (long long)NT * bn * KC * 4;
   for (long long idx = (long long)blockIdx.x * blockDim.x + threadIdx.x; idx < total;
        idx += (long long)gridDim.x * blockDim.x) {
-    const int r = (int)(idx % BN);
-    const long long rest = idx / BN;
+    const int r = (int)(idx % bn);
+    const long long rest = idx / bn;
     const int g = (int)(rest % (KC * 4));
     const int nt = (int)(rest / (KC * 4));
-    const int n = nt * BN + r;
+    const int n = nt * bn + r;
     const int kc = g >> 2, k8 = g & 3;
     __align__(16) __nv_bfloat16 p1[8], p2[8], p3[8];
 #pragma unroll
@@ -487,11 +500,11 @@
       const float x = (n < N && k < K) ? w[(size_t)n * ld + k] : 0.f;
       split3(x, p1[e], p2[e], p3[e]);
     }
-    const size_t off = (size_t)k8 * (BN * 8) + (size_t)(r >> 3) * 64 + (r & 7) * 8;
-    *reinterpret_cast<uint4*>(dst + w_tile_off(nt, kc, KC, 0) + off) = *reinterpret_cast<uint4*>(p1);
-    *reinterpret_cast<uint4*>(dst + w_tile_off(nt, kc, KC, 1) + off) = *reinterpret_cast<uint4*>(p2);
+    const size_t off = (size_t)k8 * (bn * 8) + (size_t)(r >> 3) * 64 + (r & 7) * 8;
+    *reinterpret_cast<uint4*>(dst + w_tile_off(bn, nt, kc, KC, 0) + off) = *reinterpret_cast<uint4*>(p1);
+    *reinterpret_cast<uint4*>(dst + w_tile_off(bn, nt, kc, KC, 1) + off) = *reinterpret_cast<uint4*>(p2);
     if constexpr (kPlanes == 3)
-      *reinterpret_cast<uint4*>(dst + w_tile_off(nt, kc, KC, kPlanes - 1) + off) = *reinterpret_cast<uint4*>(p3);
+      *reinterpret_cast<uint4*>(dst + w_tile_off(bn, nt, kc, KC, kPlanes - 1) + off) = *reinterpret_cast<uint4*>(p3);
   }
 }
 
@@ -547,16 +560,17 @@
 }
 
 __global__ void embed_bwd_kernel(const float* __restrict__ pts, long long P, int multires, const float* __restrict__ gx,
-                                 int ld, int ch, float* __restrict__ gp, float pw0, float pw1, float pw2, float pw3,
-                                 float pw4, float pw5, float pw6, float pw7) {
+                                 int ld, int ch, const float* __restrict__ gk, int gk_ld, float* __restrict__ gp,
+                                 float pw0, float pw1, float pw2, float pw3, float pw4, float pw5, float pw6, float pw7) {
   const float pw[8] = {pw0, pw1, pw2, pw3, pw4, pw5, pw6, pw7};
   for (long long p = (long long)blockIdx.x * blockDim.x + threadIdx.x; p < P; p += (long long)gridDim.x * blockDim.x) {
     const float* gv = gx + (size_t)p * ch * ld;
+    const float* gs = gk != nullptr ? gk + (size_t)p * gk_ld : nullptr;
     float out[3];
 #pragma unroll
     for (int j = 0; j < 3; ++j) {
       const float x = pts[p * 3 + j];
-      float acc = gv[j];
+      float acc = gv[j] + (gs ? gs[j] : 0.f);
       const float* gt = ch == 4 ? gv + (size_t)(1 + j) * ld : nullptr;
       float freq = 1.0f;
       for (int b = 0; b < multires; ++b, freq *= 2.0f) {
@@ -564,7 +578,8 @@
         sincosf(x * freq, &sn, &cs);
         const float w = pw[b] * freq;
         const int ks = 3 + 6 * b + j, kc = ks + 3;
-        acc += w * (cs * gv[ks] - sn * gv[kc]);
+        const float gsn = gv[ks] + (gs ? gs[ks] : 0.f), gcs = gv[kc] + (gs ? gs[kc] : 0.f);
+        acc += w * (cs * gsn - sn * gcs);
         if (gt) acc -= w * freq * (sn * gt[ks] + cs * gt[kc]);
       }
       out[j] = acc;
@@ -578,14 +593,14 @@
 extern "C" {
 
 int sr_tc_embed_backward(const float* pts, int64_t P, int multires, const float* pe_w, int ch, const float* gx, int ld,
-                         float* gp, cudaStream_t s) {
+                         const float* gk, int gk_ld, float* gp, cudaStream_t s) {
   if (!pts || !gx || !gp || !pe_w || P <= 0 || (ch != 1 && ch != 4) || multires < 0 || multires > 8 ||
-      ld < 3 + 6 * multires)
+      ld < 3 + 6 * multires || (gk && (ch != 1 || gk_ld < 3 + 6 * multires)))
     return SR_EINVAL;
   float w[8];
   for (int i = 0; i < 8; ++i) w[i] = i < multires ? pe_w[i] : 0.f;
-  sr_tc::embed_bwd_kernel<<<sr_grid_for(P, 256, 8), 256, 0, s>>>(pts, P, multires, gx, ld, ch, gp, w[0], w[1], w[2], w[3],
-                                                                  w[4], w[5], w[6], w[7]);
+  sr_tc::embed_bwd_kernel<<<sr_grid_for(P, 256, 8), 256, 0, s>>>(pts, P, multires, gx, ld, ch, gk, gk_ld, gp, w[0], w[1],
+                                                                  w[2], w[3], w[4], w[5], w[6], w[7]);
   return sr_launch_status();
 }
 
@@ -609,8 +624,8 @@
   return MT * KC * sr_tc::kPlanes * sr_tc::A_PLANE * 2;
 }
 int64_t sr_tc_weight_bytes(int N, int K) {
-  const int64_t NT = (N + sr_tc::BN - 1) / sr_tc::BN, KC = (K + 31) / 32;
-  return NT * KC * sr_tc::kPlanes * sr_tc::W_PLANE * 2;
+  const int64_t bn = sr_tc::tile_n(N), NT = (N + bn - 1) / bn, KC = (K + 31) / 32;
+  return NT * KC * sr_tc::kPlanes * bn * sr_tc::BK * 2;
 }
 
 int sr_tc_pack_rows(const float* src, int64_t M, int K, int ld, void* dst, const int32_t* m_dev,
@@ -625,8 +640,8 @@
 
 int sr_tc_pack_weights(const float* w, int N, int K, int ld, void* dst, cudaStream_t s) {
   if (!w || !dst || N <= 0 || K <= 0 || ld < K) return SR_EINVAL;
-  const int NT = (N + sr_tc::BN - 1) / sr_tc::BN, KC = (K + 31) / 32;
-  const long long total = (long long)NT * sr_tc::BN * KC * 4;
+  const int bn = sr_tc::tile_n(N), NT = (N + bn - 1) / bn, KC = (K + 31) / 32;
+  const long long total = (long long)NT * bn * KC * 4;
   sr_tc::pack_weights_kernel<<<sr_grid_for(total, 256, 8), 256, 0, s>>>(w, N, K, ld, (__nv_bfloat16*)dst, NT, KC);
   return sr_launch_status();
 }
@@ -643,8 +658,9 @@
                 : (act < SR_ACT_NONE || act > SR_ACT_TANH))
     return SR_EINVAL;
   LayerArgs a;
+  const int bn = tile_n(N);
   a.A = (const __nv_bfloat16*)A; a.W = (const __nv_bfloat16*)W; a.bias = bias; a.M = M;
-  a.MT = (int)((M + BM - 1) / BM); a.NT = (N + BN - 1) / BN; a.KC = (K + 31) / 32;
+  a.MT = (int)((M + BM - 1) / BM); a.NT = (N + bn - 1) / bn; a.KC = (K + 31) / 32;
   a.n_gemm = N; a.n = n_valid; a.ch = ch;
   a.A_next = (__nv_bfloat16*)A_next; a.KCn = A_next ? (K_next + 31) / 32 : 0;
   a.scale = scale; a.skip_src = skip_src; a.skip_n = skip_n; a.skip_ld = skip_ld;
@@ -654,7 +670,9 @@
 
   using Kern = void (*)(const LayerArgs);
   Kern kern = nullptr;
-#define SR_SW(ACT_, CH_, MUL_) kern = (Kern)tc_sweep_kernel<ACT_, CH_, MUL_>
+  const bool narrow = bn == BN_NARROW;
+#define SR_SW(ACT_, CH_, MUL_)                                                                    \
+  kern = narrow ? (Kern)tc_sweep_kernel<ACT_, CH_, MUL_, BN_NARROW> : (Kern)tc_sweep_kernel<ACT_, CH_, MUL_, BN>
   const int key = (ch == 4 ? 10 : 0) + (mul_tiles ? 5 + mul_act : act);
   switch (key) {
     case 0: SR_SW(SR_ACT_NONE, 1, false); break;
@@ -674,18 +692,19 @@
   }
 #undef SR_SW
   if (!kern) return SR_EINVAL;
-  static bool attr_set_dev[64][20] = {};
+  static bool attr_set_dev[64][2][20] = {};
   int cur_dev = 0;
   cudaGetDevice(&cur_dev);
-  bool& attr_set = attr_set_dev[cur_dev & 63][key];
+  bool& attr_set = attr_set_dev[cur_dev & 63][narrow][key];
+  const size_t smem = narrow ? smem_bytes<BN_NARROW>() : smem_bytes<BN>();
   if (!attr_set) {
-    cudaError_t e = cudaFuncSetAttribute(kern, cudaFuncAttributeMaxDynamicSharedMemorySize, (int)kSmem);
+    cudaError_t e = cudaFuncSetAttribute(kern, cudaFuncAttributeMaxDynamicSharedMemorySize, (int)smem);
     if (e != cudaSuccess) return (int)e;
     attr_set = true;
   }
   const int grid = a.MT < SR_NUM_SMS ? a.MT : SR_NUM_SMS;
-  kern<<<grid, kThreads, kSmem, s>>>(a);
-  const int kc0 = a.NT * (BN / 32);
+  kern<<<grid, kThreads, smem, s>>>(a);
+  const int kc0 = a.NT * (bn / 32);
   if (a.A_next != nullptr && a.KCn > kc0) {
     const int rc = sr_launch_status();
     if (rc) return rc;
diff --git a/selfreconcode_b200/csrc/trace_tc.cu b/selfreconcode_b200/csrc/trace_tc.cu
--- a/selfreconcode_b200/csrc/trace_tc.cu
+++ b/selfreconcode_b200/csrc/trace_tc.cu
@@ -166,8 +166,7 @@
   const float* pts;
   const float* rays;
   const long long* batch_inds;
-  const float* sdf4;
-  int ld_s;
+  const float* grad;
   const float* off4;
   sr_lbs_params lbs;
   int has_lbs;
@@ -208,7 +207,7 @@
       for (int r = 0; r < 3; ++r)
 #pragma unroll
         for (int c = 0; c < 3; ++c) m[3 * r + c] = Mm[3 * r] * Q[c] + Mm[3 * r + 1] * Q[3 + c] + Mm[3 * r + 2] * Q[6 + c];
-      const float gx = a.sdf4[(i * 4 + 1) * a.ld_s], gy = a.sdf4[(i * 4 + 2) * a.ld_s], gz = a.sdf4[(i * 4 + 3) * a.ld_s];
+      const float gx = a.grad[i * 3], gy = a.grad[i * 3 + 1], gz = a.grad[i * 3 + 2];
       const float gn = sqrtf(gx * gx + gy * gy + gz * gz);
       a.normals[i * 3] = gx / gn; a.normals[i * 3 + 1] = gy / gn; a.normals[i * 3 + 2] = gz / gn;
       const float c00 = m[4] * m[8] - m[5] * m[7], c01 = -m[3] * m[8] + m[5] * m[6], c02 = m[3] * m[7] - m[4] * m[6];
@@ -273,12 +272,12 @@
 extern "C" {
 
 int sr_tc_shade_point(int64_t P, const float* pts, const float* rays, const int64_t* batch_inds,
-                      const float* sdf4, int ld_s, const float* off4, const sr_lbs_params* lbs,
+                      const float* grad, const float* off4, const sr_lbs_params* lbs,
                       float* normals, float* crays, float* dpos, uint8_t* inv_ok, cudaStream_t s) {
-  if (P <= 0 || !pts || !rays || !sdf4 || !normals || !crays) return SR_EINVAL;
+  if (P <= 0 || !pts || !rays || !grad || !normals || !crays) return SR_EINVAL;
   ShadePtArgs a;
-  a.P = P; a.pts = pts; a.rays = rays; a.batch_inds = (const long long*)batch_inds; a.sdf4 = sdf4;
-  a.ld_s = ld_s; a.off4 = off4; a.has_lbs = lbs ? 1 : 0;
+  a.P = P; a.pts = pts; a.rays = rays; a.batch_inds = (const long long*)batch_inds; a.grad = grad;
+  a.off4 = off4; a.has_lbs = lbs ? 1 : 0;
   if (lbs) a.lbs = *lbs;
   a.normals = normals; a.crays = crays; a.dpos = dpos; a.inv_ok = inv_ok;
   shade_point_kernel<<<sr_grid_for(P * 32, 256, 8), 256, 0, s>>>(a);
diff --git a/selfreconcode_b200/ops.py b/selfreconcode_b200/ops.py
--- a/selfreconcode_b200/ops.py
+++ b/selfreconcode_b200/ops.py
@@ -384,6 +384,9 @@
             self.desc.pe_w[i] = float(pe_w[i]) if i < len(pe_w) else 0.0
 
     def truncated_last(self, n_out):
+        for c in self._children:
+            if c.desc.layer[c.desc.n_layers - 1].n == n_out:
+                return c
         t = FusedMLP(self.d_in, self.multires, self.device)
         C.memmove(C.byref(t.desc), C.byref(self.desc), C.sizeof(MlpDesc))
         last = t.desc.layer[t.desc.n_layers - 1]
@@ -774,6 +777,7 @@
             self.layers.append(dict(W=W, Wb=Wb, bias=torch.zeros((_pad(n, 256),), dtype=torch.float32, device=dev),
                                     n=n, k=k, act=ly.act, skip=bool(ly.skip), _e=e,
                                     zero_bias=torch.zeros((_pad(k, 256),), dtype=torch.float32, device=dev)))
+        self._wb_head = {}
         self.c_layers = (_lib.TcLayer * len(self.layers))()
         for c, L in zip(self.c_layers, self.layers):
             c.W, c.Wb, c.bias, c.zero_bias = (L[t].data_ptr() for t in ("W", "Wb", "bias", "zero_bias"))
@@ -790,6 +794,25 @@
                 check(lib.sr_tc_pack_weights(_p(e["wt"]), k, n, e["wt"].shape[1], _p(L["Wb"]), _stream()),
                       "tc_pack_weights")
                 L["bias"][:n].copy_(e["bias"][:n])
+            for n_keep, buf in self._wb_head.items():
+                self._pack_head(n_keep, buf)
+
+    def _pack_head(self, n_keep, buf):
+        L = self.layers[0]
+        e = L["_e"]
+        check(_lib.load().sr_tc_pack_weights(_p(e["wt"]), n_keep, L["n"], e["wt"].shape[1], _p(buf), _stream()),
+              "tc_pack_weights")
+
+    def wb_head(self, n_keep):
+        buf = self._wb_head.get(n_keep)
+        if buf is None:
+            lib = _lib.load()
+            buf = torch.empty((lib.sr_tc_weight_bytes(n_keep, self.layers[0]["n"]),), dtype=torch.uint8,
+                              device=self.fused.device)
+            with torch.cuda.device(self.fused.device):
+                self._pack_head(n_keep, buf)
+            self._wb_head[n_keep] = buf
+        return buf
 
 
 def tc_net(fused):
@@ -888,7 +911,8 @@
                                    tcn.layers[l - 1]["act"], scale, _p(m_dev), _stream()), "tc_linear")
             cur, nxt, K = nxt, cur, Kn
         else:
-            check(lib.sr_tc_linear(_p(cur), _p(ly["Wb"]), _p(ly["zero_bias"]), P, ly["k"], K, ly["k"], 0, 1, None, 0,
+            Wb, N = (tcn.wb_head(n_keep), n_keep) if n_keep < ly["k"] else (ly["Wb"], ly["k"])
+            check(lib.sr_tc_linear(_p(cur), _p(Wb), _p(ly["zero_bias"]), P, N, K, N, 0, 1, None, 0,
                                    scale, None, 0, 0, _p(g_out), g_out.shape[1], 0, n_keep, None, None, 0, 0, 1.0,
                                    _p(m_dev), _stream()), "tc_linear")
 
@@ -1076,6 +1100,54 @@
     return st
 
 
+class _TcShadeBuffers:
+
+    def __init__(self, dev, cap, sdf_full):
+        lib = _lib.load()
+        d = sdf_full.desc
+        f32 = lambda *shape: torch.empty(shape, dtype=torch.float32, device=dev)
+        u8 = lambda n: torch.empty((n,), dtype=torch.uint8, device=dev)
+        self.cap = cap
+        self.ld = _pad(d.d_in, 32)
+        self.emb = f32(cap, self.ld)
+        self.A_in = u8(lib.sr_tc_act_bytes(cap, self.ld))
+        self.acts = [u8(lib.sr_tc_act_bytes(cap, _pad(d.layer[i + 1].k, 32))) for i in range(d.n_layers - 1)]
+        self.out = f32(cap, d.layer[d.n_layers - 1].n)
+        widest = max([32] + [_pad(d.layer[l].n, 32) for l in range(d.n_layers - 1)])
+        self.A = [u8(lib.sr_tc_act_bytes(cap, widest)) for _ in range(2)]
+        self.cot = torch.zeros((cap, 32), dtype=torch.float32, device=dev)
+        self.cot[:, 0] = 1.0
+        self.g_out = f32(cap, self.ld)
+        self.g_skip = f32(cap, self.ld)
+        self.grad = f32(cap, 3)
+
+
+_tc_shade_bufs = {}
+
+
+def _sdf_grad_tc(lib, sdf_full, pts, P):
+    dev = pts.device
+    d = sdf_full.desc
+    key = (dev.index, tuple(d.layer[i].n for i in range(d.n_layers)), d.d_in)
+    B = _tc_shade_bufs.get(key)
+    if B is None or B.cap < P:
+        cap = _pad(max(P, B.cap + B.cap // 4 if B is not None else 0), 4096)
+        _tc_shade_bufs.pop(key, None)
+        B = None
+        B = _tc_shade_bufs[key] = _TcShadeBuffers(dev, cap, sdf_full)
+    ts, tv = tc_net(sdf_full), tc_net(sdf_full.truncated_last(1))
+    pw = (C.c_float * 16)(*[d.pe_w[i] for i in range(16)])
+    emb, out, grad, g_out = B.emb[:P], B.out[:P], B.grad[:P], B.g_out[:P]
+    check(lib.sr_tc_embed(_p(pts), P, d.multires, pw, 1, None, None, 0, 0, _p(emb), B.ld, None, None, _stream()),
+          "tc_embed")
+    _tc_mlp(lib, ts, emb, 1, out, B.A_in, B.acts)
+    _tc_backward_sweep(lib, tv, B.cot, B.A, B.acts, P, None, g_out, B.g_skip, d.d_in)
+    has_skip = any(l["skip"] for l in ts.layers)
+    check(lib.sr_tc_embed_backward(_p(pts), P, d.multires, pw, 1, _p(g_out), B.ld, _p(B.g_skip) if has_skip else None,
+                                   B.ld, _p(grad), _stream()), "tc_embed_backward")
+    return out, grad, g_out
+
+
 def shade_and_render_tc(sdf_full, def_net, lbs, render_net, pts, rays, batch_inds, conds, nfeat=256):
     _need_cuda(pts, rays)
     dev = pts.device
@@ -1091,23 +1163,23 @@
             side.wait_stream(main)
             with torch.cuda.stream(side):
                 o4 = tc_mlp_forward(def_net, pts, ch=4, conds=conds, batch_inds=bi)
-            s4 = tc_mlp_forward(sdf_full, pts, ch=4)
+            f_feat, grad, _ = _sdf_grad_tc(lib, sdf_full, pts, P)
             main.wait_stream(side)
             o4.record_stream(main)
         else:
-            s4 = tc_mlp_forward(sdf_full, pts, ch=4)
+            f_feat, grad, _ = _sdf_grad_tc(lib, sdf_full, pts, P)
             o4 = tc_mlp_forward(def_net, pts, ch=4, conds=conds, batch_inds=bi) if def_net is not None else None
         normals = torch.empty((P, 3), dtype=torch.float32, device=dev)
         crays = torch.empty((P, 3), dtype=torch.float32, device=dev)
         dpos = torch.empty((P, 3), dtype=torch.float32, device=dev)
         ok = torch.empty((P,), dtype=torch.bool, device=dev)
-        check(lib.sr_tc_shade_point(P, _p(pts), _p(rays), _p(bi), _p(s4), s4.shape[1], _p(o4), _lbs_ref(lbs),
+        check(lib.sr_tc_shade_point(P, _p(pts), _p(rays), _p(bi), _p(grad), _p(o4), _lbs_ref(lbs),
                                     _p(normals), _p(crays), _p(dpos), _p(ok), _stream()), "tc_shade_point")
         rd = render_net.desc
         ld = _pad(rd.d_in, 32)
         emb = torch.empty((P, ld), dtype=torch.float32, device=dev)
         pw = (C.c_float * 16)(*[rd.pe_w[i] for i in range(16)])
-        check(lib.sr_tc_render_embed(P, _p(pts), _p(crays), _p(normals), _p(s4), s4.shape[1], 1, nfeat, 4,
+        check(lib.sr_tc_render_embed(P, _p(pts), _p(crays), _p(normals), _p(f_feat), f_feat.shape[1], 1, nfeat, 1,
                                      rd.multires, pw, _p(emb), ld, _stream()), "tc_render_embed")
         rn = tc_net(render_net)
         rgb = torch.empty((P, rn.layers[-1]["n"]), dtype=torch.float32, device=dev)
diff --git a/selfreconcode_b200/train_ops.py b/selfreconcode_b200/train_ops.py
--- a/selfreconcode_b200/train_ops.py
+++ b/selfreconcode_b200/train_ops.py
@@ -224,8 +224,8 @@
             gp = torch.empty((P, 3), dtype=torch.float32, device=pts.device)
             pw = (C.c_float * 16)(*[pe_w[i] if i < multires else 0.0 for i in range(16)])
             with torch.cuda.device(pts.device):
-                check(lib.sr_tc_embed_backward(_p(pts), P, multires, pw, ch, _p(gx), width, _p(gp), _stream()),
-                      "tc_embed_backward")
+                check(lib.sr_tc_embed_backward(_p(pts), P, multires, pw, ch, _p(gx), width, None, 0, _p(gp),
+                                               _stream()), "tc_embed_backward")
         if E and ctx.needs_input_grad[1]:
             pe = 3 + 6 * multires
             ge = gx.view(P, ch, width)[:, 0, pe:pe + E]
```

Result: faster. 1.114 million, median of 6 (+9.5%).
